# blackle/Megalania

Measured on AMD Instinct MI355X. Metric: SA neighbour-cost evals/s, higher is better.
Workload: dtype u64

## Files before the change

### megalania_amd/csrc/mgl_api.hip

```cpp
#include "mgl_kernels.hip"
#include "mgl_kernels2.hip"
#include "mgl_kernels3.hip"
#include "mgl_kernels4.hip"
#include "mgl_kernels5.hip"
#include "mgl_pbuild.hip"
#include "mgl_index.hip"
#include "mgl_matchfinder.hip"
#include "mgl_optimal.hip"
#include "mgl_adaptive.hip"
#include "mgl_props.hip"
#include "../../include/megalania_hip.h"

#include <math.h>
#include <stdio.h>
#include <stdlib.h>
#include <string.h>
#include <string>
#include <vector>

static const uint16_t k_cost_table[2048] = {
#include "mgl_cost_table.inc"
};

#define MGL_MAX_INPUT 176000000ull
static thread_local std::string g_err;
static int fail(int code, const std::string& msg)
{
	g_err = msg;
	return code;
}
#define HIPCHK(expr)                                                                         \
	do {                                                                                     \
		hipError_t e_ = (expr);                                                              \
		if (e_ != hipSuccess)                                                                \
			return fail(MGL_EDEVICE, std::string(#expr) + ": " + hipGetErrorString(e_));     \
	} while (0)

extern "C" const char* mgl_version(void) { return "megalania-hip 0.1 (gfx950)"; }
extern "C" const char* mgl_last_error(void) { return g_err.c_str(); }
extern "C" int mgl_device_count(void)
{
	int n = 0;
	if (hipGetDeviceCount(&n) != hipSuccess) return 0;
	return n;
}
extern "C" uint32_t mgl_rng_draw_at(uint64_t seed, uint64_t step, uint32_t j, uint32_t n)
{
	return mgl_rng_draw(mgl_rng_key(seed, step, j), n);
}

struct BaseMem {
	BaseView v;
	Control* ctl;
};

struct mgl_sa {
	int device;
	hipStream_t stream;
	hipStream_t stream2;
	hipEvent_t ev_fork, ev_join;
	hipEvent_t ev_tgt = nullptr, ev_tgt_go = nullptr;
	int tgt_ahead = 0;
	hipStream_t stream3 = nullptr;
	hipEvent_t ev_rest[8] = { nullptr, nullptr, nullptr, nullptr, nullptr, nullptr, nullptr, nullptr }, ev_sim = nullptr;
	uint32_t halves;
	uint32_t n;
	mgl_properties props;
	mgl_sa_config cfg;
	uint64_t temperature = 0;
	DevCtx ctx;
	uint8_t* d_data;
	uint32_t* d_bucket_off;
	uint32_t* d_bucket_pos;
	uint16_t* d_bucket_nx;
	uint32_t* d_quad_pos;
	uint16_t* d_quad_nx;
	uint32_t *d_quad_rank = nullptr, *d_quad_run = nullptr;
	uint32_t* d_xpos[6] = { nullptr, nullptr, nullptr, nullptr, nullptr, nullptr };
	uint32_t* d_xrank[6] = { nullptr, nullptr, nullptr, nullptr, nullptr, nullptr };
	uint32_t* d_xrun[6] = { nullptr, nullptr, nullptr, nullptr, nullptr, nullptr };
	uint8_t* d_xnxb[6] = { nullptr, nullptr, nullptr, nullptr, nullptr, nullptr };
	uint32_t *d_oct_pos = nullptr, *d_oct_rank = nullptr, *d_oct_run = nullptr;
	uint32_t *d_hex_pos = nullptr, *d_hex_rank = nullptr, *d_hex_run = nullptr;
	uint64_t *d_oct_nx8 = nullptr, *d_hex_nx8 = nullptr;
	uint16_t* d_cost_tbl;
	BaseMem base, scratch;
	mgl_pk* d_best;
	NbrOut nbr;
	uint32_t* d_aos;
	uint64_t* d_cum;
	uint16_t* d_final_probs;
	mgl_pk* d_topk_pk;
	uint64_t* d_topk_cost;
	uint32_t* d_small;
	uint32_t* d_sub_offs;
	uint32_t* d_sub_lens;
	uint32_t sub_cap;
	uint64_t sqrt_thresh;
	uint32_t per_wave_bytes, waves_per_block, nbr_lds, walk_lds;
	bool incremental;
	Base2 b2;
	unsigned long long* d_prof;
	uint32_t* d_todo;
	uint32_t per_wave2, waves_per_block2, nbr2_lds, build_lds;
	uint32_t chg_cap = MGL_CHG_CAP;
	uint32_t per_wave_pick, per_wave_rest, pick_waves;
	size_t b2_bytes;
	BigScratch big;
	uint32_t* d_todo2;
	uint32_t* d_todo3 = nullptr;
	uint4* d_pickstate;
	uint4* d_pickrec;
	bool split_nbr, adaptive;
	bool form_single = false;
	uint32_t* d_counts;
	ApplyBuf ab;
	uint32_t apply_blocks;
	bool incremental_apply;
	bool snapshots;
	Base2 snap_lit, snap_best;
	SnapMeta* d_snap_meta;
	bool parallel_build;
	PBuild pb;
	hipEvent_t ev_begin, ev_end;
	std::vector<hipEvent_t> ev_pool;
	int accept_mode = MGL_ACCEPT_AUTO;
	uint32_t bulk_threshold = 0;
	bool bulk_now = true;
	uint64_t bulk_hold = 0;
	uint64_t blk_done = 0;
	uint64_t blk_imp0 = 0, blk_acc0 = 0;
	BulkBuf bulk;
	BatchBuf batch;
	bool batch_ok = false;
	uint32_t* d_strat_tgt = nullptr;
	uint32_t* d_strat_pre = nullptr;
	bool select_small = false;
	uint32_t* h_bstat = nullptr;
	hipEvent_t ev_bstat = nullptr;
	uint32_t force_batch_fail = 0;
	uint32_t force_batch_late = 0;
	AcceptLimits lim, lim_max;
	uint64_t batch_early_giveups = 0;
	uint64_t batch_accepts = 0, batch_fallbacks = 0;
	std::vector<uint8_t> mode_log;
	uint32_t force_rollbacks = 0;
	uint64_t bulk_rollbacks = 0;
	bool best_unverified = false;
	uint32_t sim_waves = MGL_SIM_WAVES;
	std::vector<hipEvent_t> ev_sim_pool;
	int64_t time_sim_step = -1;
	bool count_traffic = false;
	unsigned long long* d_traffic = nullptr;
	uint32_t short_looks = 0;
	hipEvent_t ev_val = nullptr;
	int mf_finder = MGL_MF_NEAREST;
	uint32_t mf_depth = MGL_MF_DEF_DEPTH;
	uint32_t mf_built = 0;
	uint32_t* d_mf_off = nullptr;
	uint32_t* d_mf_src = nullptr;
	uint16_t* d_mf_len = nullptr;
	size_t mf_total = 0;
	double mf_ms = 0;
};

static uint64_t ceil_sqrt_u64(uint64_t x)
{
	uint64_t r = (uint64_t)sqrt((double)x);
	while (r * r > x) r--;
	while ((r + 1) * (r + 1) <= x) r++;
	return r * r == x ? r : r + 1;
}

static void dfree(void* p) { if (p) (void)hipFree(p); }
static void free_base(BaseMem& b)
{
	dfree(b.v.slab); dfree(b.v.onwalk); dfree(b.v.ckpt_probs); dfree(b.v.ckpt_hdr); dfree(b.ctl);
	memset(&b, 0, sizeof b);
}
static hipError_t alloc_base(BaseMem& b, uint32_t n, uint32_t ckpt_elems)
{
	memset(&b, 0, sizeof b);
	hipError_t e;
	b.v.nckpt = (n + (1u << MGL_CKPT_SHIFT) - 1u) >> MGL_CKPT_SHIFT;
	b.v.ckpt_elems = ckpt_elems;
	if ((e = hipMalloc(&b.v.slab, sizeof(mgl_pk) * (size_t)n)) != hipSuccess) return e;
	if ((e = hipMalloc(&b.v.onwalk, sizeof(uint64_t) * (((size_t)n + 63) / 64 + 1))) != hipSuccess) return e;
	if ((e = hipMalloc(&b.v.ckpt_probs, sizeof(uint16_t) * (size_t)b.v.nckpt * ckpt_elems)) != hipSuccess) return e;
	if ((e = hipMalloc(&b.v.ckpt_hdr, sizeof(CkptHdr) * (size_t)b.v.nckpt)) != hipSuccess) return e;
	if ((e = hipMalloc(&b.ctl, sizeof(Control))) != hipSuccess) return e;
	if ((e = hipMemset(b.v.onwalk, 0, sizeof(uint64_t) * (((size_t)n + 63) / 64 + 1))) != hipSuccess) return e;
	return hipMemset(b.ctl, 0, sizeof(Control));
}

static size_t b2_pool_entries(const Base2& b) { return (size_t)b.pool_cap + 256; }
static int alloc_b2(Base2& b, size_t n, bool own_slab, bool init, size_t* bytes_out)
{
	size_t bytes = 0;
	if (own_slab) {
		HIPCHK(hipMalloc(&b.slab, sizeof(mgl_pk) * n)); bytes += sizeof(mgl_pk) * n;
		HIPCHK(hipMalloc(&b.onwalk, sizeof(uint64_t) * ((n + 63) / 64 + 1)));
	}
	HIPCHK(hipMalloc(&b.sp0, sizeof(uint64_t) * (b.nw0 + 64))); bytes += sizeof(uint64_t) * (b.nw0 + 64);
	HIPCHK(hipMalloc(&b.sp1, sizeof(uint64_t) * (b.nw1 + 64)));
	HIPCHK(hipMalloc(&b.sp2, sizeof(uint64_t) * (b.nw2 + 64)));
	HIPCHK(hipMalloc(&b.sp_state, sizeof(uint32_t) * 8 * n)); bytes += sizeof(uint32_t) * 8 * n;
	HIPCHK(hipMalloc(&b.ck_probs, sizeof(uint16_t) * (size_t)b.nck * b.ck_elems)); bytes += sizeof(uint16_t) * (size_t)b.nck * b.ck_elems;
	HIPCHK(hipMalloc(&b.ch_off, sizeof(uint32_t) * b.ck_elems));
	HIPCHK(hipMalloc(&b.ch_len, sizeof(uint32_t) * b.ck_elems));
	HIPCHK(hipMalloc(&b.ch_cap, sizeof(uint32_t) * b.ck_elems));
	HIPCHK(hipMalloc(&b.ch_pos, sizeof(uint32_t) * b2_pool_entries(b))); bytes += sizeof(uint32_t) * (size_t)b.pool_cap;
	HIPCHK(hipMalloc(&b.ch_ev, sizeof(uint16_t) * b2_pool_entries(b))); bytes += sizeof(uint16_t) * (size_t)b.pool_cap;
	HIPCHK(hipMalloc(&b.pool_top, sizeof(uint32_t)));
	HIPCHK(hipMalloc(&b.ch_sb, sizeof(uint32_t) * (size_t)b.ck_elems * b.sb_stride)); bytes += sizeof(uint32_t) * (size_t)b.ck_elems * b.sb_stride;
	if (init) {
		HIPCHK(hipMemset(b.ch_sb, 0, sizeof(uint32_t) * (size_t)b.ck_elems * b.sb_stride));
		HIPCHK(hipMemset(b.sp0, 0, sizeof(uint64_t) * (b.nw0 + 64)));
		HIPCHK(hipMemset(b.sp1, 0, sizeof(uint64_t) * (b.nw1 + 64)));
		HIPCHK(hipMemset(b.sp2, 0, sizeof(uint64_t) * (b.nw2 + 64)));
		HIPCHK(hipMemset(b.ch_pos, 0xFF, sizeof(uint32_t) * b2_pool_entries(b)));
		HIPCHK(hipMemset(b.ch_ev, 0, sizeof(uint16_t) * b2_pool_entries(b)));
	}
	if (bytes_out) *bytes_out = bytes;
	return MGL_OK;
}
static void free_b2(Base2& b, bool own_slab)
{
	if (own_slab) { dfree(b.slab); dfree(b.onwalk); }
	dfree(b.sp0); dfree(b.sp1); dfree(b.sp2); dfree(b.sp_state); dfree(b.ck_probs);
	dfree(b.ch_off); dfree(b.ch_len); dfree(b.ch_cap); dfree(b.ch_pos); dfree(b.ch_ev); dfree(b.pool_top); dfree(b.ch_sb);
	memset(&b, 0, sizeof b);
}
static int launch_snapshot(mgl_sa* sa, Base2& snap, uint32_t which, int dir, int cond)
{
	const Base2& from = dir == 0 ? sa->b2 : snap;
	const Base2& to = dir == 0 ? snap : sa->b2;
	const size_t n = sa->n;
	SnapPlan p;
	memset(&p, 0, sizeof p);
	uint32_t k = 0;
	auto seg = [&](const void* s, void* d, size_t bytes, uint32_t pool_elem) {
		p.seg[k].src = s; p.seg[k].dst = d; p.seg[k].bytes = bytes; p.seg[k].pool_elem = pool_elem; k++;
	};
	seg(from.slab, to.slab, sizeof(mgl_pk) * n, 0);
	seg(from.onwalk, to.onwalk, sizeof(uint64_t) * ((n + 63) / 64 + 1), 0);
	seg(from.sp0, to.sp0, sizeof(uint64_t) * (from.nw0 + 64), 0);
	seg(from.sp1, to.sp1, sizeof(uint64_t) * (from.nw1 + 64), 0);
	seg(from.sp2, to.sp2, sizeof(uint64_t) * (from.nw2 + 64), 0);
	seg(from.sp_state, to.sp_state, sizeof(uint32_t) * 8 * n, 0);
	seg(from.ck_probs, to.ck_probs, sizeof(uint16_t) * (size_t)from.nck * from.ck_elems, 0);
	seg(from.ch_off, to.ch_off, sizeof(uint32_t) * from.ck_elems, 0);
	seg(from.ch_len, to.ch_len, sizeof(uint32_t) * from.ck_elems, 0);
	seg(from.ch_cap, to.ch_cap, sizeof(uint32_t) * from.ck_elems, 0);
	seg(from.ch_pos, to.ch_pos, sizeof(uint32_t) * b2_pool_entries(from), 4);
	seg(from.ch_ev, to.ch_ev, sizeof(uint16_t) * b2_pool_entries(from), 2);
	seg(from.pool_top, to.pool_top, sizeof(uint32_t), 0);
	seg(from.ch_sb, to.ch_sb, sizeof(uint32_t) * (size_t)from.ck_elems * from.sb_stride, 0);
	p.nseg = k;
	p.src_pool_top = from.pool_top;
	hipLaunchKernelGGL(k_snapshot, dim3(2048), dim3(256), 0, sa->stream, p, sa->base.ctl, sa->d_snap_meta + which, dir, cond);
	HIPCHK(hipGetLastError());
	return MGL_OK;
}

static int launch_rebuild(mgl_sa* sa, BaseMem& b, int from_dirty, uint64_t* cum, uint16_t* final_probs)
{
	hipLaunchKernelGGL(k_rebuild, dim3(1), dim3(64), sa->walk_lds, sa->stream, sa->ctx, b.v, b.ctl, from_dirty, cum, final_probs);
	HIPCHK(hipGetLastError());
	return MGL_OK;
}
static int launch_pbuild(mgl_sa* sa, bool validate_beside = false)
{
	const DevCtx& c = sa->ctx;
	Base2& b = sa->b2;
	PBuild& pb = sa->pb;
	Control* ctl = sa->base.ctl;
	hipStream_t st = sa->stream;
	const uint32_t total = c.L.total;
	hipLaunchKernelGGL(pb_exits, dim3(pb.nblk), dim3(320), 0, st, c, b, pb);
	hipLaunchKernelGGL(pb_entries_group, dim3(pb.ngrp), dim3(320), MGL_PB_GROUP * MGL_PB_ENTRIES * 2u, st, pb);
	hipLaunchKernelGGL(pb_entries, dim3(1), dim3(64), 0, st, c, pb);
	hipLaunchKernelGGL(pb_entries_fill, dim3(pb.ngrp), dim3(64), 0, st, pb);
	hipLaunchKernelGGL(pb_mark, dim3(pb.nblk), dim3(64), 0, st, c, b, pb, ctl);
	{
		const uint32_t nch = (pb.nblk + MGL_PB_SCAN_CHUNK - 1u) / MGL_PB_SCAN_CHUNK;
		hipLaunchKernelGGL(pb_scan_chunks, dim3((nch + 255u) / 256u), dim3(256), 0, st, pb);
		hipLaunchKernelGGL(pb_scan, dim3(1), dim3(64), 0, st, pb);
		hipLaunchKernelGGL(pb_scan_fill, dim3((nch + 255u) / 256u), dim3(256), 0, st, pb);
	}
	hipLaunchKernelGGL(pb_levels, dim3((b.nw0 + 255) / 256), dim3(256), 0, st, (const uint64_t*)b.sp0, b.sp1, b.nw0, b.nw1);
	hipLaunchKernelGGL(pb_levels, dim3((b.nw1 + 255) / 256), dim3(256), 0, st, (const uint64_t*)b.sp1, b.sp2, b.nw1, b.nw2);
	hipLaunchKernelGGL(pb_walk, dim3(pb.nblk), dim3(64), b.ck_elems * 4u, st, c, b, pb);
	if (validate_beside) {
		HIPCHK(hipEventRecord(sa->ev_fork, st));
		HIPCHK(hipStreamWaitEvent(sa->stream2, sa->ev_fork, 0));
		hipLaunchKernelGGL(k_validate, dim3((sa->ctx.n + 255u) / 256u), dim3(256), 0, sa->stream2, sa->ctx, sa->b2, sa->base.ctl);
		HIPCHK(hipEventRecord(sa->ev_val, sa->stream2));
	}
	{
		const uint32_t og = (pb.nblk + MGL_PB_OFF_ROWS - 1u) / MGL_PB_OFF_ROWS;
		hipLaunchKernelGGL(pb_offsets_sum, dim3((b.ck_elems + 255) / 256, og), dim3(256), 0, st, b, pb);
		hipLaunchKernelGGL(pb_offsets_top, dim3((b.ck_elems + 255) / 256), dim3(256), 0, st, b, pb, total, og);
		hipLaunchKernelGGL(pb_offsets, dim3((b.ck_elems + 255) / 256, og), dim3(256), 0, st, b, pb, total);
		hipLaunchKernelGGL(pb_index, dim3((total + 31u) / 32u, (pb.nblk + 1u + 31u) / 32u), dim3(256), 0, st, b, pb, total);
	}
	hipLaunchKernelGGL(pb_layout, dim3(1), dim3(64), 0, st, b, pb, ctl, total);
	hipLaunchKernelGGL(pb_scatter, dim3(pb.nblk), dim3(256), b.ck_elems * 4u, st, b, pb, total);
	hipLaunchKernelGGL(pb_sim, dim3((pb.seg_cap + 63) / 64), dim3(64), 0, st, c, b, pb);
	hipLaunchKernelGGL(pb_sim_fix, dim3((total + 63) / 64), dim3(64), 0, st, c, b, pb);
	hipLaunchKernelGGL(pb_ckpt, dim3((b.ck_elems + 63) / 64, (b.nck + MGL_PB_CK_ROWS - 1) / MGL_PB_CK_ROWS), dim3(64), 0, st, c, b);
	hipLaunchKernelGGL(pb_finish, dim3(1), dim3(64), 0, st, pb, ctl);
	if (validate_beside) HIPCHK(hipStreamWaitEvent(st, sa->ev_val, 0));
	HIPCHK(hipGetLastError());
	return MGL_OK;
}
static int rebuild_base(mgl_sa* sa, int after_accept)
{
	if (!sa->incremental) return launch_rebuild(sa, sa->base, after_accept, nullptr, nullptr);
	if (sa->parallel_build && !after_accept) return launch_pbuild(sa);
	hipLaunchKernelGGL(k_build, dim3(1), dim3(64), sa->build_lds, sa->stream, sa->ctx, sa->b2, sa->base.ctl, after_accept);
	HIPCHK(hipGetLastError());
	return MGL_OK;
}
static int launch_validate(mgl_sa* sa)
{
	if (!sa->incremental) return MGL_OK;
	hipLaunchKernelGGL(k_validate, dim3((sa->ctx.n + 255u) / 256u), dim3(256), 0, sa->stream, sa->ctx, sa->b2, sa->base.ctl);
	HIPCHK(hipGetLastError());
	return MGL_OK;
}
static Base2 accept_b2(const mgl_sa* sa) { Base2 b = sa->b2; b.pool_cap = sa->lim.v[MGL_LIM_POOL]; return b; }
static ApplyBuf accept_ab(const mgl_sa* sa)
{
	ApplyBuf ab = sa->ab;
	ab.job_cap = sa->lim.v[MGL_LIM_JOBS]; ab.span_cap = sa->lim.v[MGL_LIM_SPAN_AREA]; ab.scratch_cap = sa->lim.v[MGL_LIM_SCRATCH];
	return ab;
}
static BatchBuf accept_bt(const mgl_sa* sa) { BatchBuf bt = sa->batch; bt.runs_cap = sa->lim.v[MGL_LIM_BATCH_RUNS]; return bt; }
static void accept_limits_init(mgl_sa* sa, uint32_t* why)
{
	AcceptLimits& m = sa->lim_max;
	memset(&m, 0, sizeof m);
	m.v[MGL_LIM_APPLY_EVENTS] = MGL_APPLY_CAP; m.v[MGL_LIM_APPLY_GUARD] = 1u << 20; m.v[MGL_LIM_APPLY_SUB] = MGL_SUB_CAP;
	m.v[MGL_LIM_APPLY_SPAN] = MGL_SPAN_CAP; m.v[MGL_LIM_APPLY_PIECES] = MGL_PIECE_CAP; m.v[MGL_LIM_APPLY_SHIFT] = MGL_SUB_CAP;
	m.v[MGL_LIM_POOL] = sa->b2.pool_cap; m.v[MGL_LIM_JOBS] = sa->ab.job_cap; m.v[MGL_LIM_SPAN_AREA] = sa->ab.span_cap;
	m.v[MGL_LIM_SCRATCH] = sa->ab.scratch_cap;
	m.v[MGL_LIM_BATCH_JOURNAL] = MGL_BATCH_JCAP; m.v[MGL_LIM_BATCH_EVENTS] = MGL_BATCH_EVCAP; m.v[MGL_LIM_BATCH_OPS] = MGL_BATCH_OPCAP;
	m.v[MGL_LIM_BATCH_GUARD] = 1u << 18; m.v[MGL_LIM_BATCH_SUB] = MGL_BATCH_SUB; m.v[MGL_LIM_BATCH_SHIFT] = 2047u;
	m.v[MGL_LIM_BATCH_RUNS] = sa->batch.runs_cap; m.v[MGL_LIM_SOFT_REACH] = 1u;
	m.why = why;
	sa->lim = m;
	sa->lim.v[MGL_LIM_SOFT_REACH] = 0u;
}
static int launch_targets_ahead(mgl_sa* sa, uint64_t next_gstep);
static int launch_apply(mgl_sa* sa, uint64_t next_gstep = ~0ull)
{
	if (sa->snapshots) {
		int rc = launch_snapshot(sa, sa->snap_best, 1, 0, 2);
		if (rc) return rc;
	}
	hipLaunchKernelGGL(k_apply_walk, dim3(1), dim3(64), 0, sa->stream, sa->ctx, sa->b2, sa->base.ctl, sa->nbr, sa->ab, sa->lim);
	if (next_gstep != ~0ull) { int rc = launch_targets_ahead(sa, next_gstep); if (rc) return rc; }
	if (!sa->snapshots)
		hipLaunchKernelGGL(k_copy_best, dim3(256), dim3(256), 0, sa->stream, (const Control*)sa->base.ctl,
		                   (const mgl_pk*)sa->base.v.slab, sa->d_best, sa->ctx.n);
	hipLaunchKernelGGL(k_apply_chains, dim3(sa->apply_blocks), dim3(MGL_APPLY_THREADS), 0, sa->stream, sa->ctx, accept_b2(sa), sa->base.ctl, accept_ab(sa), sa->lim);
	hipLaunchKernelGGL(k_apply_jobs, dim3(1024), dim3(256), 0, sa->stream, sa->b2, (const Control*)sa->base.ctl, sa->ab, 0, (const uint32_t*)nullptr);
	hipLaunchKernelGGL(k_apply_jobs, dim3(1024), dim3(256), 0, sa->stream, sa->b2, (const Control*)sa->base.ctl, sa->ab, 1, (const uint32_t*)nullptr);
	hipLaunchKernelGGL(k_build_end, dim3(1), dim3(64), sa->build_lds, sa->stream, sa->ctx, sa->b2, sa->base.ctl, sa->snapshots ? 1 : 0, sa->d_counts, sa->adaptive ? 1 : 0, sa->form_single ? 1 : 0);
	HIPCHK(hipGetLastError());
	return MGL_OK;
}
static const bool g_trace = getenv("MGL_TRACE") != nullptr, g_prof_big = getenv("MGL_PROF_BIG") != nullptr, g_big_inline_sim = getenv("MGL_BIG_INLINE_SIM") != nullptr;
#define NBR_TRACE(name) do { if (g_trace) { fprintf(stderr, "[mgl] %s\n", name); hipError_t e_ = hipDeviceSynchronize(); if (e_ != hipSuccess) fprintf(stderr, "[mgl] %s -> %s\n", name, hipGetErrorString(e_)); } } while (0)
static hipEvent_t sim_event(mgl_sa* sa, size_t i)
{
	while (sa->ev_sim_pool.size() <= i) {
		hipEvent_t e = nullptr;
		if (hipEventCreate(&e) != hipSuccess) return nullptr;
		sa->ev_sim_pool.push_back(e);
	}
	return sa->ev_sim_pool[i];
}
static uint32_t nbr_slices(const mgl_sa* sa)
{
	const uint32_t K = sa->cfg.neighbours_per_step;
	return (sa->halves >= 2 && K >= 1024) ? sa->halves : 1u;
}
static void launch_targets(mgl_sa* sa, hipStream_t st, uint64_t step_override)
{
	const uint32_t K = sa->cfg.neighbours_per_step;
	const uint64_t* onwalk = sa->incremental ? sa->b2.onwalk : sa->base.v.onwalk;
	const uint32_t nw0 = sa->incremental ? sa->b2.nw0 : (sa->ctx.n + 63u) >> 6;
	hipLaunchKernelGGL(k_rank_blocks, dim3(sa->ctx.strat_nblk), dim3(64), 0, st, onwalk, nw0, sa->d_strat_pre, sa->ctx.strat_nblk);
	hipLaunchKernelGGL(k_rank_scan, dim3(1), dim3(1024), 0, st, sa->d_strat_pre, sa->ctx.strat_nblk);
	hipLaunchKernelGGL(k_targets, dim3((K + 3u) / 4u), dim3(256), 0, st, sa->ctx, onwalk, nw0, (const Control*)sa->base.ctl, sa->cfg.seed, step_override, K, sa->d_strat_tgt);
}
static int launch_targets_ahead(mgl_sa* sa, uint64_t next_gstep)
{
	if (!sa->d_strat_pre || !sa->incremental) return MGL_OK;
	HIPCHK(hipEventRecord(sa->ev_tgt_go, sa->stream));
	HIPCHK(hipStreamWaitEvent(sa->stream2, sa->ev_tgt_go, 0));
	launch_targets(sa, sa->stream2, next_gstep);
	HIPCHK(hipEventRecord(sa->ev_tgt, sa->stream2));
	HIPCHK(hipGetLastError());
	sa->tgt_ahead = 1;
	return MGL_OK;
}
static int launch_neighbours(mgl_sa* sa, uint64_t step_override, bool zero_counts = true)
{
	const uint32_t K = sa->cfg.neighbours_per_step;
	if (sa->d_strat_pre) {
		if (sa->tgt_ahead) HIPCHK(hipStreamWaitEvent(sa->stream, sa->ev_tgt, 0));
		if (sa->tgt_ahead != 1) launch_targets(sa, sa->stream, step_override);
		sa->tgt_ahead = 0;
	}
	if (!sa->incremental) {
		const uint32_t blocks = (K + sa->waves_per_block - 1) / sa->waves_per_block;
		hipLaunchKernelGGL(k_neighbours, dim3(blocks), dim3(64 * sa->waves_per_block), sa->nbr_lds, sa->stream, sa->ctx, sa->base.v,
		                   (const Control*)sa->base.ctl, sa->cfg.seed, step_override, K, sa->nbr, sa->per_wave_bytes,
		                   (const uint32_t*)nullptr, (const uint32_t*)nullptr); NBR_TRACE("k_neighbours");
		HIPCHK(hipGetLastError());
		return MGL_OK;
	}
	if (zero_counts) HIPCHK(hipMemsetAsync(sa->d_counts, 0, 8 * sizeof(uint32_t), sa->stream));
	const uint32_t blocks2 = (K + sa->waves_per_block2 - 1) / sa->waves_per_block2;
	const bool split_now = sa->split_nbr && !sa->form_single;
	const uint32_t sim_lds_regular = ((((sa->ctx.L.total + 31u) >> 5) + 3u) & ~3u) * 4u + sa->chg_cap * 16u;
	if (split_now) {
		const uint32_t slices = nbr_slices(sa);
		HIPCHK(hipEventRecord(sa->ev_fork, sa->stream));
		if (slices >= 2) HIPCHK(hipStreamWaitEvent(sa->stream2, sa->ev_fork, 0));
		HIPCHK(hipStreamWaitEvent(sa->stream3, sa->ev_fork, 0));
		for (uint32_t h = 0; h < slices; h++) {
			const uint32_t j0 = (uint32_t)((uint64_t)K * h / slices), j1 = (uint32_t)((uint64_t)K * (h + 1) / slices);
			hipStream_t st = (h & 1u) ? sa->stream2 : sa->stream;
			hipLaunchKernelGGL((k_neighbours2<false, MGL_NBR_PICK>), dim3((j1 - j0 + sa->pick_waves - 1) / sa->pick_waves), dim3(64 * sa->pick_waves),
			                   (MGL_PICK_T_GLOBAL ? 0u : 4096u) + sa->pick_waves * sa->per_wave_pick, st, sa->ctx,
			                   sa->b2, sa->base.ctl, sa->cfg.seed, step_override, K, sa->nbr, sa->per_wave_pick, sa->d_todo, sa->d_counts,
			                   (unsigned long long*)nullptr, sa->big, sa->d_pickrec, j0, j1, sa->d_pickstate); NBR_TRACE("k_neighbours2<false, MGL_NBR_PICK>");
			hipLaunchKernelGGL((k_neighbours2<false, MGL_NBR_REST>), dim3(j1 - j0), dim3(64), sa->per_wave_rest, st, sa->ctx,
			                   sa->b2, sa->base.ctl, sa->cfg.seed, step_override, K, sa->nbr, sa->per_wave_rest, sa->d_todo, sa->d_counts,
			                   g_prof_big ? (unsigned long long*)nullptr : sa->d_prof, sa->big, sa->d_pickrec, j0, j1, sa->d_pickstate); NBR_TRACE("k_neighbours2<false, MGL_NBR_REST>");
			HIPCHK(hipEventRecord(sa->ev_rest[h], st));
		}
		HIPCHK(hipGetLastError());
		for (uint32_t h = 0; h < slices; h++) {
			const uint32_t j0 = (uint32_t)((uint64_t)K * h / slices), j1 = (uint32_t)((uint64_t)K * (h + 1) / slices);
			HIPCHK(hipStreamWaitEvent(sa->stream3, sa->ev_rest[h], 0));
			if (sa->time_sim_step >= 0 && h < 2) HIPCHK(hipEventRecord(sim_event(sa, 6 * (size_t)sa->time_sim_step + 2 * h), sa->stream3));
			if (sa->count_traffic)
				hipLaunchKernelGGL(k_sim<true>, dim3(j1 - j0), dim3(64 * sa->sim_waves), sim_lds_regular, sa->stream3, sa->ctx, sa->b2, sa->base.ctl,
				                   sa->nbr, sa->big, j0, j1, sa->d_todo3, sa->d_counts + 4, (const uint32_t*)nullptr, (const uint32_t*)nullptr, sa->d_traffic);
			else
				hipLaunchKernelGGL(k_sim<false>, dim3(j1 - j0), dim3(64 * sa->sim_waves), sim_lds_regular, sa->stream3, sa->ctx, sa->b2, sa->base.ctl,
				                   sa->nbr, sa->big, j0, j1, sa->d_todo3, sa->d_counts + 4, (const uint32_t*)nullptr, (const uint32_t*)nullptr, (unsigned long long*)nullptr);
			NBR_TRACE("k_sim");
			if (sa->time_sim_step >= 0 && h < 2) HIPCHK(hipEventRecord(sim_event(sa, 6 * (size_t)sa->time_sim_step + 2 * h + 1), sa->stream3));
		}
		HIPCHK(hipEventRecord(sa->ev_sim, sa->stream3));
		for (uint32_t h = 1; h < slices; h += 2) HIPCHK(hipStreamWaitEvent(sa->stream, sa->ev_rest[h], 0));
	}
	if (!sa->split_nbr || sa->form_single) {
		hipLaunchKernelGGL((k_neighbours2<false, MGL_NBR_FULL>), dim3(blocks2), dim3(64 * sa->waves_per_block2), sa->nbr2_lds, sa->stream, sa->ctx,
		                   sa->b2, sa->base.ctl, sa->cfg.seed, step_override, K, sa->nbr, sa->per_wave2, sa->d_todo, sa->d_counts,
		                   sa->d_prof, sa->big, sa->d_pickrec, 0u, K, sa->d_pickstate); NBR_TRACE("k_neighbours2<false, MGL_NBR_FULL>");
	}
	const uint32_t bigneed = (sa->big.slots + sa->waves_per_block2 - 1) / sa->waves_per_block2;
	const uint32_t bigblocks = bigneed < 1024u ? bigneed : 1024u;
	BigScratch big_now = sa->big;
	big_now.lds_cache = 1u;
	const uint32_t big_lds = sa->nbr2_lds + 12u * MGL_BIG_CAP;
	if (!split_now || g_big_inline_sim) big_now.sim_hdr2 = nullptr;
	hipLaunchKernelGGL((k_neighbours2<true, MGL_NBR_FULL>), dim3(bigblocks), dim3(64 * sa->waves_per_block2), big_lds, sa->stream, sa->ctx,
	                   sa->b2, sa->base.ctl, sa->cfg.seed, step_override, K, sa->nbr, sa->per_wave2, sa->d_todo2, sa->d_counts + 1,
	                   g_prof_big ? sa->d_prof : (unsigned long long*)nullptr, big_now, (sa->split_nbr && !sa->form_single) ? sa->d_pickrec : (uint4*)nullptr, 0u, K, sa->d_pickstate); NBR_TRACE("k_neighbours2<true, MGL_NBR_FULL>");
	if (split_now) {
		const uint32_t sim_lds = ((((sa->ctx.L.total + 31u) >> 5) + 3u) & ~3u) * 4u + MGL_SIM2_CAP * 16u;
		if (sa->time_sim_step >= 0) HIPCHK(hipEventRecord(sim_event(sa, 6 * (size_t)sa->time_sim_step + 4), sa->stream));
		if (sa->count_traffic)
			hipLaunchKernelGGL(k_sim<true>, dim3(256), dim3(64 * MGL_SIM_WAVES_LIST), sim_lds, sa->stream, sa->ctx, sa->b2, sa->base.ctl, sa->nbr, big_now, 0u, K,
			                   sa->d_todo3, sa->d_counts + 4, (const uint32_t*)sa->d_todo, (const uint32_t*)sa->d_counts, sa->d_traffic);
		else
			hipLaunchKernelGGL(k_sim<false>, dim3(256), dim3(64 * MGL_SIM_WAVES_LIST), sim_lds, sa->stream, sa->ctx, sa->b2, sa->base.ctl, sa->nbr, big_now, 0u, K,
			                   sa->d_todo3, sa->d_counts + 4, (const uint32_t*)sa->d_todo, (const uint32_t*)sa->d_counts, (unsigned long long*)nullptr);
		NBR_TRACE("k_sim");
		if (sa->time_sim_step >= 0) HIPCHK(hipEventRecord(sim_event(sa, 6 * (size_t)sa->time_sim_step + 5), sa->stream));
		HIPCHK(hipStreamWaitEvent(sa->stream, sa->ev_sim, 0));
		BigScratch late = sa->big;
		late.todo_in = sa->d_todo3; late.todo_in_count = sa->d_counts + 4; late.sim_hdr2 = nullptr; late.lds_cache = 1u;
		late.cont = nullptr;
		hipLaunchKernelGGL((k_neighbours2<true, MGL_NBR_FULL>), dim3(bigblocks < 64u ? bigblocks : 64u), dim3(64 * sa->waves_per_block2), big_lds, sa->stream, sa->ctx,
		                   sa->b2, sa->base.ctl, sa->cfg.seed, step_override, K, sa->nbr, sa->per_wave2, sa->d_todo2, sa->d_counts + 1,
		                   (unsigned long long*)nullptr, late, sa->d_pickrec, 0u, K, sa->d_pickstate); NBR_TRACE("k_neighbours2<true, MGL_NBR_FULL>");
	}
	const uint32_t blocks = (K + sa->waves_per_block - 1) / sa->waves_per_block;
	hipLaunchKernelGGL(k_neighbours, dim3(blocks < 256u ? blocks : 256u), dim3(64 * sa->waves_per_block), sa->nbr_lds, sa->stream, sa->ctx, sa->base.v,
	                   (const Control*)sa->base.ctl, sa->cfg.seed, step_override, K, sa->nbr, sa->per_wave_bytes,
	                   (const uint32_t*)sa->d_todo2, (const uint32_t*)(sa->d_counts + 1)); NBR_TRACE("k_neighbours");
	HIPCHK(hipGetLastError());
	return MGL_OK;
}

static int import_slab(mgl_sa* sa, const mgl_packet* packets, mgl_pk* d_slab)
{
	HIPCHK(hipMemcpyAsync(sa->d_aos, packets, sizeof(mgl_packet) * (size_t)sa->n, hipMemcpyHostToDevice, sa->stream));
	hipLaunchKernelGGL(k_import, dim3(1024), dim3(256), 0, sa->stream, (const uint32_t*)sa->d_aos, d_slab, sa->n);
	HIPCHK(hipGetLastError());
	return MGL_OK;
}
static int export_slab(mgl_sa* sa, const mgl_pk* d_slab, mgl_packet* packets)
{
	hipLaunchKernelGGL(k_export, dim3(1024), dim3(256), 0, sa->stream, d_slab, sa->d_aos, sa->n);
	HIPCHK(hipGetLastError());
	HIPCHK(hipMemcpyAsync(packets, sa->d_aos, sizeof(mgl_packet) * (size_t)sa->n, hipMemcpyDeviceToHost, sa->stream));
	HIPCHK(hipStreamSynchronize(sa->stream));
	return MGL_OK;
}

extern "C" void mgl_sa_destroy(mgl_sa* sa)
{
	if (!sa) return;
	(void)hipSetDevice(sa->device);
	if (sa->stream) (void)hipStreamSynchronize(sa->stream);
	dfree(sa->d_data); dfree(sa->d_bucket_off); dfree(sa->d_bucket_pos); dfree(sa->d_bucket_nx); dfree(sa->d_quad_pos); dfree(sa->d_quad_nx); dfree(sa->d_cost_tbl);
	dfree(sa->d_quad_rank); dfree(sa->d_quad_run); dfree(sa->d_oct_pos);
	for (int i = 0; i < 6; i++) { if (i != 0 && i != 2) { dfree(sa->d_xpos[i]); dfree(sa->d_xrank[i]); dfree(sa->d_xrun[i]); } dfree(sa->d_xnxb[i]); } dfree(sa->d_oct_rank); dfree(sa->d_oct_run);
	dfree(sa->d_hex_pos); dfree(sa->d_hex_rank); dfree(sa->d_hex_run); dfree(sa->d_oct_nx8); dfree(sa->d_hex_nx8);
	free_base(sa->base); free_base(sa->scratch);
	if (!sa->snapshots) dfree(sa->d_best);
	dfree(sa->nbr.cost); dfree(sa->nbr.ndiffs); dfree(sa->nbr.walked); dfree(sa->nbr.win); dfree(sa->nbr.win2); dfree(sa->nbr.dpos);
	dfree(sa->bulk.ckey); dfree(sa->bulk.cwin); dfree(sa->bulk.taken); dfree(sa->bulk.cstate); dfree(sa->bulk.cflags); dfree(sa->bulk.hdr);
	dfree(sa->nbr.dold); dfree(sa->nbr.dnew);
	dfree(sa->d_aos); dfree(sa->d_cum); dfree(sa->d_final_probs);
	free_b2(sa->b2, false);
	free_b2(sa->snap_lit, true); free_b2(sa->snap_best, true); dfree(sa->d_snap_meta);
	dfree(sa->pb.exits); dfree(sa->pb.entry); dfree(sa->pb.gexits); dfree(sa->pb.gentry); dfree(sa->pb.gsum); dfree(sa->pb.ch_map); dfree(sa->pb.ch_vs); dfree(sa->pb.ch_pk); dfree(sa->pb.ch_state); dfree(sa->pb.tf_ctx); dfree(sa->pb.tf_dist); dfree(sa->pb.tf_pk);
	dfree(sa->pb.st_in); dfree(sa->pb.hist); dfree(sa->pb.stage); dfree(sa->pb.stage_n); dfree(sa->pb.stage_over); dfree(sa->pb.acc); dfree(sa->pb.seg_off); dfree(sa->pb.unres);
	dfree(sa->d_todo); dfree(sa->d_prof);
	dfree(sa->big.sim_hdr); dfree(sa->big.sim_keys); dfree(sa->big.sim_pos);
	dfree(sa->big.ins_key); dfree(sa->big.rem_key); dfree(sa->big.ins_pos); dfree(sa->big.rem_pos); dfree(sa->big.uctx);
	if (sa->h_bstat) (void)hipHostFree(sa->h_bstat);
	if (sa->ev_bstat) (void)hipEventDestroy(sa->ev_bstat);
	dfree(sa->big.cont); dfree(sa->d_traffic); dfree(sa->d_strat_pre); dfree(sa->d_strat_tgt);
	{
		BatchBuf& bt = sa->batch;
		dfree(bt.hdr); dfree(bt.cl); dfree(bt.jpos); dfree(bt.jnew); dfree(bt.jold); dfree(bt.st_ikey); dfree(bt.st_rkey); dfree(bt.st_ipos);
		dfree(bt.st_rpos); dfree(bt.ops); dfree(bt.ins_cl); dfree(bt.rem_cl); dfree(bt.acc); dfree(bt.runs);
		dfree(bt.cnt_i); dfree(bt.cnt_r); dfree(bt.off_i); dfree(bt.off_r); dfree(bt.cur_i); dfree(bt.cur_r); dfree(bt.touched);
		dfree(bt.bk_ipos); dfree(bt.bk_rpos); dfree(bt.bk_ibit); dfree(bt.bk_icl); dfree(bt.bk_rcl);
	}
	for (hipEvent_t e : sa->ev_sim_pool) if (e) (void)hipEventDestroy(e);
	dfree(sa->d_todo2); dfree(sa->d_todo3); dfree(sa->d_counts); dfree(sa->big.sim_hdr2); dfree(sa->big.sim_slot2); dfree(sa->d_pickrec); dfree(sa->d_pickstate);
	dfree(sa->lim.why); dfree(sa->ab.hdr); dfree(sa->ab.ins_key); dfree(sa->ab.rem_key); dfree(sa->ab.ins_pos); dfree(sa->ab.rem_pos);
	dfree(sa->ab.tctx); dfree(sa->ab.scratch_pos); dfree(sa->ab.scratch_ev);
	dfree(sa->ab.span_pos); dfree(sa->ab.span_ev); dfree(sa->ab.jobs_b); dfree(sa->ab.jobs_c);
	dfree(sa->d_mf_off); dfree(sa->d_mf_src); dfree(sa->d_mf_len);
	dfree(sa->d_topk_pk); dfree(sa->d_topk_cost); dfree(sa->d_small); dfree(sa->d_sub_offs); dfree(sa->d_sub_lens);
	for (hipEvent_t e : sa->ev_pool) (void)hipEventDestroy(e);
	if (sa->ev_begin) (void)hipEventDestroy(sa->ev_begin);
	if (sa->ev_end) (void)hipEventDestroy(sa->ev_end);
	if (sa->stream2) (void)hipStreamDestroy(sa->stream2);
	if (sa->stream3) (void)hipStreamDestroy(sa->stream3);
	for (auto& e : sa->ev_rest) if (e) (void)hipEventDestroy(e);
	if (sa->ev_sim) (void)hipEventDestroy(sa->ev_sim);
	if (sa->ev_val) (void)hipEventDestroy(sa->ev_val);
	if (sa->ev_fork) (void)hipEventDestroy(sa->ev_fork);
	if (sa->ev_tgt) (void)hipEventDestroy(sa->ev_tgt);
	if (sa->ev_tgt_go) (void)hipEventDestroy(sa->ev_tgt_go);
	if (sa->ev_join) (void)hipEventDestroy(sa->ev_join);
	if (sa->stream) (void)hipStreamDestroy(sa->stream);
	delete sa;
}

static int create_impl(mgl_sa* sa, const uint8_t* data, size_t n)
{
	HIPCHK(hipSetDevice(sa->device));
	HIPCHK(hipStreamCreate(&sa->stream));
	HIPCHK(hipStreamCreate(&sa->stream2));
	HIPCHK(hipEventCreateWithFlags(&sa->ev_fork, hipEventDisableTiming));
	HIPCHK(hipEventCreateWithFlags(&sa->ev_join, hipEventDisableTiming));
	HIPCHK(hipEventCreateWithFlags(&sa->ev_tgt, hipEventDisableTiming));
	HIPCHK(hipEventCreateWithFlags(&sa->ev_tgt_go, hipEventDisableTiming));
	HIPCHK(hipStreamCreate(&sa->stream3));
	for (auto& e : sa->ev_rest) HIPCHK(hipEventCreateWithFlags(&e, hipEventDisableTiming));
	HIPCHK(hipEventCreateWithFlags(&sa->ev_sim, hipEventDisableTiming));
	HIPCHK(hipEventCreateWithFlags(&sa->ev_val, hipEventDisableTiming));
	sa->halves = getenv("MGL_HALVES") ? (uint32_t)atoi(getenv("MGL_HALVES")) : (n > (1u << 20) ? 2u : 1u);
	if (sa->halves < 1 || sa->halves > 8) sa->halves = 1;
	HIPCHK(hipEventCreate(&sa->ev_begin));
	HIPCHK(hipEventCreate(&sa->ev_end));
	const mgl_layout L = mgl_make_layout(sa->props.lc, sa->props.lp, sa->props.pb);
	const uint32_t ckpt_elems = (L.total + 7u) & ~7u;

	HIPCHK(hipMalloc(&sa->d_data, n + 128));
	HIPCHK(hipMemset(sa->d_data, 0, n + 128));
	HIPCHK(hipMemcpy(sa->d_data, data, n, hipMemcpyHostToDevice));

	{
		const uint32_t m = (uint32_t)(n - 1);
		HIPCHK(hipMalloc(&sa->d_bucket_off, sizeof(uint32_t) * 65537));
		HIPCHK(hipMalloc(&sa->d_bucket_pos, sizeof(uint32_t) * (n ? n : 1)));
		HIPCHK(hipMalloc(&sa->d_bucket_nx, sizeof(uint16_t) * (n ? n : 1)));
		HIPCHK(hipMalloc(&sa->d_quad_pos, sizeof(uint32_t) * (n ? n : 1)));
		HIPCHK(hipMalloc(&sa->d_quad_nx, sizeof(uint16_t) * (n ? n : 1)));
		for (int i = 0; i < 6; i++) {
			HIPCHK(hipMalloc(&sa->d_xnxb[i], n + 1));
			HIPCHK(hipMemset(sa->d_xnxb[i], 0, n + 1));
			if (i == 0 || i == 2) continue;
			for (uint32_t** a : { &sa->d_xpos[i], &sa->d_xrank[i], &sa->d_xrun[i] }) {
				HIPCHK(hipMalloc(a, sizeof(uint32_t) * (n + 1)));
				HIPCHK(hipMemset(*a, 0, sizeof(uint32_t) * (n + 1)));
			}
		}
		for (uint32_t** a : { &sa->d_quad_rank, &sa->d_quad_run, &sa->d_oct_pos, &sa->d_oct_rank, &sa->d_oct_run, &sa->d_hex_pos, &sa->d_hex_rank, &sa->d_hex_run }) {
			HIPCHK(hipMalloc(a, sizeof(uint32_t) * (n + 1)));
			HIPCHK(hipMemset(*a, 0, sizeof(uint32_t) * (n + 1)));
		}
		HIPCHK(hipMalloc(&sa->d_oct_nx8, sizeof(uint64_t) * (n + 1)));
		HIPCHK(hipMalloc(&sa->d_hex_nx8, sizeof(uint64_t) * (n + 1)));
		if (m == 0) HIPCHK(hipMemset(sa->d_bucket_off, 0, sizeof(uint32_t) * 65537));
		else {
			const uint32_t nblk = (m + MGL_IX_ITEMS - 1) / MGL_IX_ITEMS;
			uint32_t *tmp = nullptr, *matrix = nullptr;
			HIPCHK(hipMalloc(&tmp, sizeof(uint32_t) * m));
			HIPCHK(hipMalloc(&matrix, sizeof(uint32_t) * 256 * (size_t)nblk));
			for (int pass = 1; pass >= 0; pass--) {
				const uint32_t* in = pass == 1 ? nullptr : tmp;
				uint32_t* out = pass == 1 ? tmp : sa->d_bucket_pos;
				hipLaunchKernelGGL(ix_count, dim3(nblk), dim3(64), 0, sa->stream, (const uint8_t*)sa->d_data, in, m, pass, matrix, nblk);
				hipLaunchKernelGGL(ix_scan, dim3(1), dim3(1024), 0, sa->stream, matrix, 256u * nblk);
				hipLaunchKernelGGL(ix_scatter, dim3(nblk), dim3(64), 0, sa->stream, (const uint8_t*)sa->d_data, in, out, m, pass,
				                   (const uint32_t*)matrix, nblk);
			}
			hipLaunchKernelGGL(ix_offsets, dim3(m / 256 + 1), dim3(256), 0, sa->stream, (const uint8_t*)sa->d_data,
			                   (const uint32_t*)sa->d_bucket_pos, m, sa->d_bucket_off);
			hipLaunchKernelGGL(ix_next2, dim3(m / 256 + 1), dim3(256), 0, sa->stream, (const uint8_t*)sa->d_data,
			                   (const uint32_t*)sa->d_bucket_pos, m, sa->d_bucket_nx, 0);
			for (int pass = 3; pass >= 0; pass--) {
				const uint32_t* in = pass == 3 ? nullptr : ((pass & 1) ? (const uint32_t*)sa->d_quad_pos : (const uint32_t*)tmp);
				uint32_t* out = (pass & 1) ? tmp : sa->d_quad_pos;
				hipLaunchKernelGGL(ix_count, dim3(nblk), dim3(64), 0, sa->stream, (const uint8_t*)sa->d_data, in, m, pass, matrix, nblk);
				hipLaunchKernelGGL(ix_scan, dim3(1), dim3(1024), 0, sa->stream, matrix, 256u * nblk);
				hipLaunchKernelGGL(ix_scatter, dim3(nblk), dim3(64), 0, sa->stream, (const uint8_t*)sa->d_data, in, out, m, pass,
				                   (const uint32_t*)matrix, nblk);
			}
			hipLaunchKernelGGL(ix_next2, dim3(m / 256 + 1), dim3(256), 0, sa->stream, (const uint8_t*)sa->d_data,
			                   (const uint32_t*)sa->d_quad_pos, m, sa->d_quad_nx, 1);
			sa->d_xpos[0] = sa->d_bucket_pos; sa->d_xpos[2] = sa->d_quad_pos;
			sa->d_xrank[2] = sa->d_quad_rank; sa->d_xrun[2] = sa->d_quad_run;
			for (uint32_t D : { 3u, 5u, 6u, 7u, 8u, 16u }) {
				uint32_t* dst = D == 8 ? sa->d_oct_pos : D == 16 ? sa->d_hex_pos : sa->d_xpos[D - 2];
				for (int pass = (int)D - 1; pass >= 0; pass--) {
					const uint32_t* in = pass == (int)D - 1 ? nullptr : ((pass & 1) ? (const uint32_t*)dst : (const uint32_t*)tmp);
					uint32_t* out = (pass & 1) ? tmp : dst;
					hipLaunchKernelGGL(ix_count, dim3(nblk), dim3(64), 0, sa->stream, (const uint8_t*)sa->d_data, in, m, pass, matrix, nblk);
					hipLaunchKernelGGL(ix_scan, dim3(1), dim3(1024), 0, sa->stream, matrix, 256u * nblk);
					hipLaunchKernelGGL(ix_scatter, dim3(nblk), dim3(64), 0, sa->stream, (const uint8_t*)sa->d_data, in, out, m, pass,
					                   (const uint32_t*)matrix, nblk);
				}
			}
			struct { const uint32_t* pos; uint32_t* rank; uint32_t* run; void* nx; uint32_t D, nxbytes; } lv[7] = {
				{ sa->d_xpos[1], sa->d_xrank[1], sa->d_xrun[1], sa->d_xnxb[1], 3u, 1u },
				{ sa->d_quad_pos, sa->d_quad_rank, sa->d_quad_run, sa->d_xnxb[2], 4u, 1u },
				{ sa->d_xpos[3], sa->d_xrank[3], sa->d_xrun[3], sa->d_xnxb[3], 5u, 1u },
				{ sa->d_xpos[4], sa->d_xrank[4], sa->d_xrun[4], sa->d_xnxb[4], 6u, 1u },
				{ sa->d_xpos[5], sa->d_xrank[5], sa->d_xrun[5], sa->d_xnxb[5], 7u, 1u },
				{ sa->d_oct_pos, sa->d_oct_rank, sa->d_oct_run, sa->d_oct_nx8, 8u, 8u },
				{ sa->d_hex_pos, sa->d_hex_rank, sa->d_hex_run, sa->d_hex_nx8, 16u, 8u } };
			hipLaunchKernelGGL(ix_next_byte, dim3(m / 256 + 1), dim3(256), 0, sa->stream, (const uint8_t*)sa->d_data, (const uint32_t*)sa->d_bucket_pos, m, sa->d_xnxb[0], 2u);
			for (auto& l : lv) {
				hipLaunchKernelGGL(ix_rank, dim3(m / 256 + 1), dim3(256), 0, sa->stream, l.pos, m, l.rank);
				if (l.nxbytes == 1) hipLaunchKernelGGL(ix_next_byte, dim3(m / 256 + 1), dim3(256), 0, sa->stream, (const uint8_t*)sa->d_data, l.pos, m, (uint8_t*)l.nx, l.D);
				else hipLaunchKernelGGL(ix_next_bytes, dim3(m / 256 + 1), dim3(256), 0, sa->stream, (const uint8_t*)sa->d_data, l.pos, m, l.nx, l.D, l.nxbytes);
				hipLaunchKernelGGL(ix_heads, dim3(m / 256 + 1), dim3(256), 0, sa->stream, (const uint8_t*)sa->d_data, l.pos, m, l.D, l.run);
				hipLaunchKernelGGL(ix_maxscan, dim3(1), dim3(1024), 0, sa->stream, l.run, m);
			}
			hipError_t e1 = hipGetLastError(), e2 = hipStreamSynchronize(sa->stream);
			(void)hipFree(tmp); (void)hipFree(matrix);
			HIPCHK(e1); HIPCHK(e2);
		}
	}
	HIPCHK(hipMalloc(&sa->d_cost_tbl, sizeof(k_cost_table)));
	HIPCHK(hipMemcpy(sa->d_cost_tbl, k_cost_table, sizeof(k_cost_table), hipMemcpyHostToDevice));

	sa->ctx.data = sa->d_data; sa->ctx.n = (uint32_t)n;
	sa->ctx.bucket_off = sa->d_bucket_off; sa->ctx.bucket_pos = sa->d_bucket_pos; sa->ctx.bucket_nx = sa->d_bucket_nx; sa->ctx.quad_pos = sa->d_quad_pos; sa->ctx.quad_nx = sa->d_quad_nx;
	for (int i = 0; i < 6; i++) { sa->ctx.xpos[i] = sa->d_xpos[i]; sa->ctx.xrank[i] = sa->d_xrank[i]; sa->ctx.xrun[i] = sa->d_xrun[i]; sa->ctx.xnxb[i] = sa->d_xnxb[i]; }
	sa->ctx.oct_pos = sa->d_oct_pos; sa->ctx.oct_rank = sa->d_oct_rank; sa->ctx.oct_run = sa->d_oct_run; sa->ctx.oct_nx8 = sa->d_oct_nx8;
	sa->ctx.hex_pos = sa->d_hex_pos; sa->ctx.hex_rank = sa->d_hex_rank; sa->ctx.hex_run = sa->d_hex_run; sa->ctx.hex_nx8 = sa->d_hex_nx8;
	sa->ctx.cost_tbl = sa->d_cost_tbl; sa->ctx.L = L;
	sa->ctx.dict_limit = sa->cfg.dict_limit; sa->ctx.max_scan = sa->cfg.max_bucket_scan; sa->ctx.top_k = sa->cfg.top_k;

	HIPCHK(alloc_base(sa->base, (uint32_t)n, ckpt_elems));
	HIPCHK(alloc_base(sa->scratch, (uint32_t)n, ckpt_elems));

	const size_t K = sa->cfg.neighbours_per_step;
	HIPCHK(hipMalloc(&sa->nbr.cost, sizeof(uint64_t) * K));
	HIPCHK(hipMalloc(&sa->nbr.ndiffs, sizeof(uint32_t) * K));
	HIPCHK(hipMalloc(&sa->nbr.walked, sizeof(uint32_t) * K));
	HIPCHK(hipMalloc(&sa->nbr.win, sizeof(uint32_t) * 2 * K));
	HIPCHK(hipMemset(sa->nbr.win, 0xFF, sizeof(uint32_t) * 2 * K));
	HIPCHK(hipMalloc(&sa->nbr.win2, sizeof(uint32_t) * K));
	HIPCHK(hipMemset(sa->nbr.win2, 0xFF, sizeof(uint32_t) * K));
	memset(&sa->bulk, 0, sizeof sa->bulk);
	HIPCHK(hipMalloc(&sa->bulk.ckey, sizeof(uint64_t) * K));
// ... 56 lines not shown
			pb.shift = b.sb_shift;
			pb.nblk = (uint32_t)((n + (1u << pb.shift) - 1) >> pb.shift);
			HIPCHK(hipMalloc(&pb.exits, sizeof(uint16_t) * (size_t)pb.nblk * MGL_PB_ENTRIES));
			HIPCHK(hipMalloc(&pb.entry, sizeof(uint32_t) * ((size_t)pb.nblk + 1)));
			pb.ngrp = (pb.nblk + MGL_PB_GROUP - 1u) / MGL_PB_GROUP;
			HIPCHK(hipMalloc(&pb.gexits, sizeof(uint16_t) * (size_t)pb.ngrp * MGL_PB_ENTRIES));
			HIPCHK(hipMalloc(&pb.gentry, sizeof(uint16_t) * (size_t)pb.ngrp));
			{
				const size_t nch = ((size_t)pb.nblk + MGL_PB_SCAN_CHUNK - 1u) / MGL_PB_SCAN_CHUNK;
				HIPCHK(hipMalloc(&pb.ch_map, sizeof(uint64_t) * nch));
				HIPCHK(hipMalloc(&pb.ch_vs, sizeof(uint32_t) * 8 * nch));
				HIPCHK(hipMalloc(&pb.ch_pk, sizeof(uint32_t) * nch));
				HIPCHK(hipMalloc(&pb.ch_state, sizeof(uint32_t) * 8 * nch));
			}
			HIPCHK(hipMalloc(&pb.gsum, sizeof(uint32_t) * (size_t)((pb.nblk + MGL_PB_OFF_ROWS - 1u) / MGL_PB_OFF_ROWS) * ckpt_elems));
			HIPCHK(hipMalloc(&pb.tf_ctx, sizeof(uint64_t) * pb.nblk));
			HIPCHK(hipMalloc(&pb.tf_dist, sizeof(uint32_t) * 8 * (size_t)pb.nblk));
			HIPCHK(hipMalloc(&pb.tf_pk, sizeof(uint32_t) * pb.nblk));
			HIPCHK(hipMalloc(&pb.st_in, sizeof(uint32_t) * 8 * (size_t)pb.nblk));
			HIPCHK(hipMalloc(&pb.hist, sizeof(uint32_t) * (size_t)pb.nblk * ckpt_elems));
			HIPCHK(hipMalloc(&pb.stage, sizeof(uint64_t) * (size_t)pb.nblk * ((MGL_PB_STAGE_PER_POS << pb.shift) + 32u)));
			HIPCHK(hipMalloc(&pb.stage_n, sizeof(uint32_t) * (size_t)pb.nblk));
			HIPCHK(hipMalloc(&pb.stage_over, sizeof(uint32_t)));
			HIPCHK(hipMemset(pb.stage_over, 0, sizeof(uint32_t)));
			HIPCHK(hipMalloc(&pb.acc, sizeof(unsigned long long) * 16));
			HIPCHK(hipMemset(pb.acc, 0, sizeof(unsigned long long) * 16));
			pb.seg_cap = b.pool_cap / MGL_PB_SEG + ckpt_elems + 64u;
			HIPCHK(hipMalloc(&pb.seg_off, sizeof(uint32_t) * (ckpt_elems + 1)));
			HIPCHK(hipMalloc(&pb.unres, pb.seg_cap));
		}
		sa->snapshots = !(sa->cfg.flags & MGL_F_NO_SNAPSHOTS);
		if (sa->snapshots) {
			for (Base2* s : { &sa->snap_lit, &sa->snap_best }) {
				*s = b;
				s->slab = nullptr; s->onwalk = nullptr; s->sp0 = s->sp1 = s->sp2 = nullptr; s->sp_state = nullptr;
				s->ck_probs = nullptr; s->ch_off = s->ch_len = s->ch_cap = s->ch_pos = nullptr; s->ch_ev = nullptr;
				s->pool_top = nullptr;
				int rc = alloc_b2(*s, n, true, false, nullptr);
				if (rc) return rc;
			}
			HIPCHK(hipMalloc(&sa->d_snap_meta, sizeof(SnapMeta) * 2));
			HIPCHK(hipMemset(sa->d_snap_meta, 0, sizeof(SnapMeta) * 2));
			sa->d_best = sa->snap_best.slab;
		}
		if (sa->cfg.flags & MGL_F_PROFILE) {
			HIPCHK(hipMalloc(&sa->d_prof, sizeof(unsigned long long) * (32 + K)));
			HIPCHK(hipMemset(sa->d_prof, 0, sizeof(unsigned long long) * (32 + K)));
		}
		HIPCHK(hipMalloc(&sa->d_todo, sizeof(uint32_t) * (K + 1)));
		HIPCHK(hipMemset(sa->d_todo, 0, sizeof(uint32_t) * (K + 1)));
		sa->b2_bytes = bytes;
		sa->incremental_apply = getenv("MGL_NO_INCREMENTAL_APPLY") == nullptr;
		{
			ApplyBuf& ab = sa->ab;
			memset(&ab, 0, sizeof ab);
			sa->apply_blocks = 256;
			ab.scratch_cap = b.pool_cap + 256u;
			ab.span_cap = 1u << 22;
			ab.job_cap = 1u << 20;
			HIPCHK(hipMalloc(&ab.hdr, sizeof(uint32_t) * 16));
			HIPCHK(hipMemset(ab.hdr, 0, sizeof(uint32_t) * 16));
			HIPCHK(hipMalloc(&ab.ins_key, sizeof(uint16_t) * MGL_BATCH_ALLOC));
			HIPCHK(hipMalloc(&ab.rem_key, sizeof(uint16_t) * MGL_BATCH_ALLOC));
			HIPCHK(hipMalloc(&ab.ins_pos, sizeof(uint32_t) * MGL_BATCH_ALLOC));
			HIPCHK(hipMalloc(&ab.rem_pos, sizeof(uint32_t) * MGL_BATCH_ALLOC));
			HIPCHK(hipMalloc(&ab.tctx, sizeof(uint16_t) * 16384));
			HIPCHK(hipMalloc(&ab.scratch_pos, sizeof(uint32_t) * (size_t)ab.scratch_cap));
			HIPCHK(hipMalloc(&ab.scratch_ev, sizeof(uint16_t) * (size_t)ab.scratch_cap));
			HIPCHK(hipMalloc(&ab.span_pos, sizeof(uint32_t) * (size_t)ab.span_cap));
			HIPCHK(hipMalloc(&ab.span_ev, sizeof(uint16_t) * (size_t)ab.span_cap));
			HIPCHK(hipMalloc(&ab.jobs_b, sizeof(uint4) * (size_t)ab.job_cap));
			HIPCHK(hipMalloc(&ab.jobs_c, sizeof(uint4) * (size_t)ab.job_cap));
			BatchBuf& bt = sa->batch;
			memset(&bt, 0, sizeof bt);
			HIPCHK(hipMalloc(&bt.hdr, sizeof(uint32_t) * 16));
			HIPCHK(hipMemset(bt.hdr, 0, sizeof(uint32_t) * 16));
			HIPCHK(hipMalloc(&bt.cl, sizeof(uint32_t) * 8 * MGL_BATCH_MAX));
			HIPCHK(hipMalloc(&bt.jpos, sizeof(uint32_t) * MGL_BATCH_MAX * MGL_MAX_DIFFS));
			HIPCHK(hipMalloc(&bt.jnew, sizeof(mgl_pk) * MGL_BATCH_MAX * MGL_MAX_DIFFS));
			HIPCHK(hipMalloc(&bt.jold, sizeof(mgl_pk) * MGL_BATCH_MAX * MGL_MAX_DIFFS));
			HIPCHK(hipMalloc(&bt.st_ikey, sizeof(uint16_t) * MGL_BATCH_ALLOC));
			HIPCHK(hipMalloc(&bt.st_rkey, sizeof(uint16_t) * MGL_BATCH_ALLOC));
			HIPCHK(hipMalloc(&bt.st_ipos, sizeof(uint32_t) * MGL_BATCH_ALLOC));
			HIPCHK(hipMalloc(&bt.st_rpos, sizeof(uint32_t) * MGL_BATCH_ALLOC));
			HIPCHK(hipMalloc(&bt.ops, sizeof(uint4) * 2 * (size_t)MGL_BATCH_MAX * MGL_BATCH_OPCAP));
			HIPCHK(hipMalloc(&bt.ins_cl, MGL_BATCH_ALLOC));
			HIPCHK(hipMalloc(&bt.rem_cl, MGL_BATCH_ALLOC));
			bt.nctx = L.total;
			bt.runs_cap = 1u << 17;
			HIPCHK(hipMalloc(&bt.runs, sizeof(uint4) * 2 * (size_t)bt.runs_cap));
			for (uint32_t** p : { &bt.cnt_i, &bt.cnt_r, &bt.off_i, &bt.off_r, &bt.cur_i, &bt.cur_r, &bt.touched }) {
				HIPCHK(hipMalloc(p, sizeof(uint32_t) * (bt.nctx + 64u)));
				HIPCHK(hipMemset(*p, 0, sizeof(uint32_t) * (bt.nctx + 64u)));
			}
			HIPCHK(hipMalloc(&bt.bk_ipos, sizeof(uint32_t) * MGL_BATCH_ALLOC));
			HIPCHK(hipMalloc(&bt.bk_rpos, sizeof(uint32_t) * MGL_BATCH_ALLOC));
			HIPCHK(hipMalloc(&bt.bk_ibit, sizeof(uint16_t) * MGL_BATCH_ALLOC));
			HIPCHK(hipMalloc(&bt.bk_icl, MGL_BATCH_ALLOC));
			HIPCHK(hipMalloc(&bt.bk_rcl, MGL_BATCH_ALLOC));
			HIPCHK(hipMalloc(&bt.acc, sizeof(long long) * 4));
			HIPCHK(hipMemset(bt.acc, 0, sizeof(long long) * 4));
			HIPCHK(hipHostMalloc((void**)&sa->h_bstat, sizeof(uint32_t) * 16, hipHostMallocDefault));
			HIPCHK(hipEventCreateWithFlags(&sa->ev_bstat, hipEventDisableTiming));
			sa->batch_ok = sa->incremental_apply && getenv("MGL_NO_BATCH") == nullptr;
			uint32_t* why = nullptr;
			HIPCHK(hipMalloc(&why, sizeof(uint32_t)));
			HIPCHK(hipMemset(why, 0, sizeof(uint32_t)));
			accept_limits_init(sa, why);

		}
		{
			const uint32_t fixed = MGL_MAX_DIFFS * (8u + 8u + 4u) + (((((L.total + 31u) >> 5) + 3u) & ~3u) * 4u) ;
			const uint32_t model = ckpt_elems * 2u + MGL_PRICE_WORDS * 4u;
			sa->chg_cap = K <= 1024u ? 4u * MGL_CHG_CAP : (K <= 2048u ? 2u * MGL_CHG_CAP : MGL_CHG_CAP);
			const uint32_t lists = sa->chg_cap * (4u + 4u + 2u + 2u) + 2u * sa->chg_cap * 2u;
			sa->per_wave2 = (fixed + (model > lists ? model : lists) + 15u) & ~15u;
			sa->per_wave_pick = (model + 15u) & ~15u;
			sa->per_wave_rest = (fixed + lists + 15u) & ~15u;
		}
		{
			BigScratch& g = sa->big;
			memset(&g, 0, sizeof g);
			g.chg_cap = sa->chg_cap;
			g.cap = MGL_BIG_CAP; g.uctx_cap = ckpt_elems; g.slots = (uint32_t)(K > 512 ? K : 512);
			HIPCHK(hipMalloc(&g.ins_key, sizeof(uint16_t) * (size_t)g.cap * g.slots));
			HIPCHK(hipMalloc(&g.rem_key, sizeof(uint16_t) * (size_t)g.cap * g.slots));
			HIPCHK(hipMalloc(&g.ins_pos, sizeof(uint32_t) * (size_t)g.cap * g.slots));
			HIPCHK(hipMalloc(&g.rem_pos, sizeof(uint32_t) * (size_t)g.cap * g.slots));
			HIPCHK(hipMalloc(&g.uctx, sizeof(uint16_t) * (size_t)g.uctx_cap * g.slots));
			HIPCHK(hipMalloc(&sa->d_todo2, sizeof(uint32_t) * (K + 1)));
			HIPCHK(hipMemset(sa->d_todo2, 0, sizeof(uint32_t) * (K + 1)));
		}
		{
			uint32_t best_w = 1, best_total = 0;
			for (uint32_t w = 1; w <= 8; w++) {
				const uint32_t bytes = 4096u + w * sa->per_wave2;
				if (bytes > 160u * 1024u) break;
				const uint32_t tot = (160u * 1024u / bytes) * w;
				if (tot > best_total) { best_total = tot; best_w = w; }
			}
			(void)best_w;
			sa->waves_per_block2 = 1;
		}
		sa->nbr2_lds = 4096u + sa->waves_per_block2 * sa->per_wave2;
		sa->build_lds = 4096u + ckpt_elems * 2u + ckpt_elems * 8u;
		HIPCHK(hipMalloc(&sa->d_counts, sizeof(uint32_t) * 16));
		HIPCHK(hipMemset(sa->d_counts, 0, sizeof(uint32_t) * 16));
		HIPCHK(hipMalloc(&sa->d_todo3, sizeof(uint32_t) * (K + 1)));
		HIPCHK(hipMemset(sa->d_todo3, 0, sizeof(uint32_t) * (K + 1)));
		sa->big.todo_in = sa->d_todo; sa->big.todo_in_count = sa->d_counts; sa->big.spill_ctr = sa->d_counts + 2;
		HIPCHK(hipFuncSetAttribute((const void*)k_neighbours2<false, MGL_NBR_FULL>, hipFuncAttributeMaxDynamicSharedMemorySize, (int)sa->nbr2_lds));
		HIPCHK(hipFuncSetAttribute((const void*)k_neighbours2<false, MGL_NBR_PICK>, hipFuncAttributeMaxDynamicSharedMemorySize, 160 * 1024));
		HIPCHK(hipFuncSetAttribute((const void*)k_neighbours2<false, MGL_NBR_REST>, hipFuncAttributeMaxDynamicSharedMemorySize, (int)sa->nbr2_lds));
		HIPCHK(hipFuncSetAttribute((const void*)k_neighbours2<true, MGL_NBR_FULL>, hipFuncAttributeMaxDynamicSharedMemorySize, (int)(sa->nbr2_lds + 12u * MGL_BIG_CAP)));
		HIPCHK(hipMalloc(&sa->d_pickrec, sizeof(uint4) * K));
		HIPCHK(hipMalloc(&sa->d_pickstate, sizeof(uint4) * 2 * K));
		sa->split_nbr = getenv("MGL_NO_SPLIT") == nullptr;
		if (sa->split_nbr) {
			BigScratch& g = sa->big;
			HIPCHK(hipMalloc(&g.sim_hdr, sizeof(uint4) * (size_t)K));
			HIPCHK(hipMalloc(&g.sim_keys, sizeof(uint16_t) * 2u * sa->chg_cap * (size_t)K));
			HIPCHK(hipMalloc(&g.sim_pos, sizeof(uint32_t) * 2u * sa->chg_cap * (size_t)K));
			HIPCHK(hipMemset(g.sim_hdr, 0xFF, sizeof(uint4) * (size_t)K));
			HIPCHK(hipMalloc(&g.sim_hdr2, sizeof(uint4) * (size_t)K));
			HIPCHK(hipMalloc(&g.sim_slot2, sizeof(uint32_t) * (size_t)K));
			HIPCHK(hipMemset(g.sim_hdr2, 0xFF, sizeof(uint4) * (size_t)K));
			if (getenv("MGL_NO_CONT") == nullptr) {
				HIPCHK(hipMalloc(&g.cont, sizeof(uint32_t) * MGL_CONT_WORDS * (size_t)g.slots));
				HIPCHK(hipMemset(g.cont, 0, sizeof(uint32_t) * MGL_CONT_WORDS * (size_t)g.slots));
			}
		}
		if (getenv("MGL_SIMW")) { const int w = atoi(getenv("MGL_SIMW")); if (w == 1 || w == 2 || w == 4 || w == 8) sa->sim_waves = (uint32_t)w; }
		sa->adaptive = sa->split_nbr && getenv("MGL_NO_ADAPT") == nullptr;
		sa->form_single = !sa->split_nbr;
		sa->pick_waves = getenv("MGL_PICK_WAVES") ? (uint32_t)atoi(getenv("MGL_PICK_WAVES")) : 0u;
		if (sa->pick_waves != 1 && sa->pick_waves != 2 && sa->pick_waves != 4 && sa->pick_waves != 8) sa->pick_waves = 0;
		{
			uint32_t best_w = 1, best_resident = 0;
			for (uint32_t w = 1; w <= 8; w *= 2) {
				const uint32_t bytes = (MGL_PICK_T_GLOBAL ? 0u : 4096u) + w * sa->per_wave_pick;
				if (bytes > 160u * 1024u) break;
				const uint32_t resident = (160u * 1024u / ((bytes + 1279u) / 1280u * 1280u)) * w;
				if (resident > best_resident) { best_resident = resident; best_w = w; }
			}
			if (n > (1u << 20)) best_w = 1;
			if (sa->pick_waves == 0 || (MGL_PICK_T_GLOBAL ? 0u : 4096u) + sa->pick_waves * sa->per_wave_pick > 160u * 1024u) sa->pick_waves = best_w;
		}
		HIPCHK(hipFuncSetAttribute((const void*)k_sim<false>, hipFuncAttributeMaxDynamicSharedMemorySize, 96 * 1024));
		HIPCHK(hipFuncSetAttribute((const void*)k_sim<true>, hipFuncAttributeMaxDynamicSharedMemorySize, 96 * 1024));
		HIPCHK(hipMalloc(&sa->d_traffic, sizeof(unsigned long long) * 2));
		HIPCHK(hipMemset(sa->d_traffic, 0, sizeof(unsigned long long) * 2));
		HIPCHK(hipFuncSetAttribute((const void*)k_build, hipFuncAttributeMaxDynamicSharedMemorySize, (int)sa->build_lds));
		HIPCHK(hipFuncSetAttribute((const void*)k_build_end, hipFuncAttributeMaxDynamicSharedMemorySize, (int)sa->build_lds));
	}

	if (!(sa->cfg.flags & MGL_F_POSITION_TARGETS)) {
		sa->ctx.strat_nblk = (uint32_t)((n + 4095u) / 4096u);
		HIPCHK(hipMalloc(&sa->d_strat_pre, sizeof(uint32_t) * (sa->ctx.strat_nblk + 2u)));
		HIPCHK(hipMemset(sa->d_strat_pre, 0, sizeof(uint32_t) * (sa->ctx.strat_nblk + 2u)));
		sa->ctx.strat_pre = sa->d_strat_pre;
		HIPCHK(hipMalloc(&sa->d_strat_tgt, sizeof(uint32_t) * sa->cfg.neighbours_per_step));
		sa->ctx.strat_tgt = sa->d_strat_tgt;
	}
	sa->sqrt_thresh = ceil_sqrt_u64(sa->cfg.iters_per_epoch);
	sa->bulk_threshold = getenv("MGL_BULK_THRESHOLD") ? (uint32_t)atoi(getenv("MGL_BULK_THRESHOLD"))
	                     : sa->batch_ok ? 2u : (n <= (1u << 20) ? 16u : n <= (1u << 24) ? 32u : 128u);
	if (sa->bulk_threshold == 0) sa->bulk_threshold = 1;

	hipLaunchKernelGGL(k_fill_literal, dim3(1024), dim3(256), 0, sa->stream, sa->base.v.slab, sa->ctx.n);
	if (!sa->d_best) HIPCHK(hipMalloc(&sa->d_best, sizeof(mgl_pk) * n));
	hipLaunchKernelGGL(k_fill_literal, dim3(1024), dim3(256), 0, sa->stream, sa->d_best, sa->ctx.n);
	HIPCHK(hipGetLastError());
	int rc = rebuild_base(sa, 0);
	if (rc) return rc;
	if (sa->incremental && sa->snapshots && (rc = launch_snapshot(sa, sa->snap_lit, 0, 0, 0))) return rc;
	HIPCHK(hipStreamSynchronize(sa->stream));
	{
		Control c0;
		HIPCHK(hipMemcpy(&c0, sa->base.ctl, sizeof c0, hipMemcpyDeviceToHost));
		if (c0.error_flags) return fail(MGL_EDEVICE, "mgl_sa_create: building the base structures of the all-literal slab failed");
	}
	return MGL_OK;
}

extern "C" mgl_sa* mgl_sa_create(const uint8_t* data, size_t n, mgl_properties props, const mgl_sa_config* cfg)
{
	if (!data || n == 0 || !cfg) { fail(MGL_EINVAL, "mgl_sa_create: bad data/size/config"); return nullptr; }
	if (n > MGL_MAX_INPUT) { fail(MGL_EINVAL, "mgl_sa_create: input larger than 176 000 000 bytes is not supported"); return nullptr; }
	if (props.lc + props.lp > 4 || props.pb > 4 || props.lc > 8) { fail(MGL_EINVAL, "mgl_sa_create: unsupported lc/lp/pb"); return nullptr; }
	mgl_sa* sa = new (std::nothrow) mgl_sa();
	if (!sa) { fail(MGL_ENOMEM, "mgl_sa_create: out of host memory"); return nullptr; }
	sa->cfg = *cfg;
	sa->props = props;
	sa->n = (uint32_t)n;
	sa->device = cfg->device;
	if (sa->cfg.neighbours_per_step == 0) sa->cfg.neighbours_per_step = 1;
	if (sa->cfg.neighbours_per_step > (1u << 20)) { delete sa; fail(MGL_EINVAL, "neighbours_per_step > 2^20"); return nullptr; }
	if (sa->cfg.top_k == 0) sa->cfg.top_k = 20;
	if (sa->cfg.top_k > MGL_MAX_TOPK) { delete sa; fail(MGL_EINVAL, "top_k > 32"); return nullptr; }
	if (sa->cfg.dict_limit == 0) sa->cfg.dict_limit = 0x400000u;
	if (sa->cfg.iters_per_epoch == 0) sa->cfg.iters_per_epoch = n;
	int rc = create_impl(sa, data, n);
	if (rc != MGL_OK) {
		std::string keep = g_err;
		mgl_sa_destroy(sa);
		g_err = keep;
		return nullptr;
	}
	return sa;
}

static int read_ctl(mgl_sa* sa, BaseMem& b, Control* out)
{
	HIPCHK(hipMemcpyAsync(out, b.ctl, sizeof(Control), hipMemcpyDeviceToHost, sa->stream));
	HIPCHK(hipStreamSynchronize(sa->stream));
	return MGL_OK;
}
static int write_ctl(mgl_sa* sa, BaseMem& b, const Control* in)
{
	HIPCHK(hipMemcpyAsync(b.ctl, in, sizeof(Control), hipMemcpyHostToDevice, sa->stream));
	HIPCHK(hipStreamSynchronize(sa->stream));
	return MGL_OK;
}

static int keep_best_before_overwrite(mgl_sa* sa, Control& c)
{
	if (!(sa->incremental && sa->snapshots) || !c.best_is_current) return MGL_OK;
	int rc = launch_snapshot(sa, sa->snap_best, 1, 0, 0);
	if (rc) return rc;
	c.best_is_current = 0;
	return MGL_OK;
}

extern "C" int mgl_sa_begin_epoch(mgl_sa* sa, unsigned phase, int from_best)
{
	if (!sa) return fail(MGL_EINVAL, "null handle");
	HIPCHK(hipSetDevice(sa->device));
	Control c;
	int rc = read_ctl(sa, sa->base, &c);
	if (rc) return rc;
	if (from_best && c.best_cost == 0) from_best = 0;
	const bool snaps = sa->incremental && sa->snapshots;
	const bool base_is_best = snaps && c.best_is_current;
	if (!from_best && (rc = keep_best_before_overwrite(sa, c))) return rc;
	c.iter = 0; c.cur_cost = 0; c.phase = phase; c.accepted_flag = 0; c.copy_best_flag = 0;
	if ((rc = write_ctl(sa, sa->base, &c))) return rc;
	sa->bulk_now = !from_best; sa->bulk_hold = 0; sa->blk_done = 0; sa->select_small = false;
	if (from_best && base_is_best) return MGL_OK;
	if (snaps) {
		SnapMeta meta[2];
		HIPCHK(hipMemcpyAsync(meta, sa->d_snap_meta, sizeof meta, hipMemcpyDeviceToHost, sa->stream));
		HIPCHK(hipStreamSynchronize(sa->stream));
		const uint32_t which = from_best ? 1u : 0u;
		if (meta[which].valid) {
			if ((rc = launch_snapshot(sa, which ? sa->snap_best : sa->snap_lit, which, 1, 0))) return rc;
			HIPCHK(hipStreamSynchronize(sa->stream));
			return MGL_OK;
		}
	}
	if (from_best) HIPCHK(hipMemcpyAsync(sa->base.v.slab, sa->d_best, sizeof(mgl_pk) * (size_t)sa->n, hipMemcpyDeviceToDevice, sa->stream));
	else {
		hipLaunchKernelGGL(k_fill_literal, dim3(1024), dim3(256), 0, sa->stream, sa->base.v.slab, sa->ctx.n);
		HIPCHK(hipGetLastError());
	}
	if ((rc = rebuild_base(sa, 0))) return rc;
	if (from_best && sa->best_unverified) {
		if ((rc = launch_validate(sa))) return rc;
		Control v;
		if ((rc = read_ctl(sa, sa->base, &v))) return rc;
		if (v.error_flags || v.rebuild_cost != v.best_cost) {
			v.error_flags = 0;
			(void)write_ctl(sa, sa->base, &v);
			return fail(MGL_EINVAL, "mgl_sa_begin_epoch: the adopted best slab is not a valid parse of the input at the cost it came with");
		}
		sa->best_unverified = false;
	}
	if (snaps && (rc = launch_snapshot(sa, from_best ? sa->snap_best : sa->snap_lit, from_best ? 1u : 0u, 0, 0))) return rc;
	HIPCHK(hipStreamSynchronize(sa->stream));
	return MGL_OK;
// ... 739 lines not shown
		hipLaunchKernelGGL(k_batch_chains, dim3(MGL_BATCH_GRID), dim3(MGL_BATCH_THREADS), 0, sa->stream, sa->ctx, accept_b2(sa), sa->base.ctl, bt, ab, sa->lim);
		hipLaunchKernelGGL(k_batch_ckpt, dim3(1024, 8), dim3(256), 0, sa->stream, b, (const Control*)sa->base.ctl, bt, ab);
		hipLaunchKernelGGL(k_apply_jobs, dim3(1024), dim3(256), 0, sa->stream, b, (const Control*)sa->base.ctl, sa->ab, 0, (const uint32_t*)sa->batch.hdr);
		hipLaunchKernelGGL(k_apply_jobs, dim3(1024), dim3(256), 0, sa->stream, b, (const Control*)sa->base.ctl, sa->ab, 1, (const uint32_t*)sa->batch.hdr);
		hipLaunchKernelGGL(k_batch_end, dim3(1), dim3(64), 0, sa->stream, sa->base.ctl, sa->batch);
		HIPCHK(hipGetLastError());
		HIPCHK(hipMemcpyAsync(sa->h_bstat, sa->batch.hdr, sizeof bstat, hipMemcpyDeviceToHost, sa->stream));
		HIPCHK(hipEventRecord(sa->ev_bstat, sa->stream));
		launch_bulk_close(sa, (const uint32_t*)sa->batch.hdr);
		HIPCHK(hipGetLastError());
		HIPCHK(hipEventSynchronize(sa->ev_bstat));
		memcpy(bstat, sa->h_bstat, sizeof bstat);
		closed = bstat[0] == 3u || bstat[0] == 0u;
		if (!closed && sa->tgt_ahead) sa->tgt_ahead = 2;
		if (sa->force_batch_fail) {
			const uint32_t zero = 0u;
			HIPCHK(hipMemcpy(sa->batch.hdr + 9, &zero, sizeof zero, hipMemcpyHostToDevice));
			HIPCHK(hipMemcpy(sa->batch.hdr + 13, &zero, sizeof zero, hipMemcpyHostToDevice));
			if ((bstat[0] == 1u || bstat[0] == 3u) && --sa->force_batch_fail == 0) sa->force_batch_late = 0;
		}
	}
	if (sa->batch_ok) sa->select_small = bstat[7] <= 512u;
	if (bstat[0] == 3u) sa->batch_accepts++;
	else if (bstat[0] != 0u) {
		if (sa->batch_ok && bstat[0] == 1u) sa->batch_fallbacks++;
		if (sa->batch_ok && bstat[0] == 2u && bstat[4]) sa->batch_early_giveups++;
		if (bstat[0] != 1u)
			hipLaunchKernelGGL(k_bulk_write, dim3(64), dim3(256), 0, sa->stream, sa->base.ctl, sa->nbr, sa->bulk, sa->base.v.slab);
		HIPCHK(hipGetLastError());
		Control now;
		if (sa->batch_ok && bstat[0] == 1u) {
			if ((rc = read_ctl(sa, sa->base, &now))) return rc;
			now.apply_failed = 0;
			if ((rc = write_ctl(sa, sa->base, &now))) return rc;
		}
		if ((rc = launch_pbuild(sa, sa->incremental))) return rc;
		if ((rc = read_ctl(sa, sa->base, &now))) return rc;
		if (sa->force_rollbacks && now.taken) { sa->force_rollbacks--; now.error_flags |= MGL_ERR_BAD_PACKET; }
		if (now.error_flags & MGL_ERR_BAD_PACKET) {
			hipLaunchKernelGGL(k_bulk_rollback, dim3(64), dim3(256), 0, sa->stream, sa->nbr, sa->bulk, sa->base.v.slab);
			HIPCHK(hipGetLastError());
			now.error_flags &= ~MGL_ERR_BAD_PACKET;
			now.accepted -= now.taken;
			now.taken = 0;
			sa->bulk_rollbacks++;
			if ((rc = write_ctl(sa, sa->base, &now))) return rc;
			if ((rc = launch_pbuild(sa))) return rc;
		}
	}
	if (!closed) launch_bulk_close(sa, nullptr);
	HIPCHK(hipGetLastError());
	return MGL_OK;
}

extern "C" int mgl_sa_run(mgl_sa* sa, uint64_t steps, mgl_sa_stats* stats)
{
	if (!sa) return fail(MGL_EINVAL, "null handle");
	HIPCHK(hipSetDevice(sa->device));
	Control before, after;
	int rc = read_ctl(sa, sa->base, &before);
	if (rc) return rc;
	const bool timing = (sa->cfg.flags & MGL_F_TIMING) != 0;
	const uint64_t t_stride = steps > 16 ? 4u : 1u;
	const uint64_t timed_steps = timing ? ((steps + t_stride - 1) / t_stride < 512 ? (steps + t_stride - 1) / t_stride : 512) : 0;
	const bool inc_apply = sa->incremental && sa->incremental_apply;
	const DecideArgs dargs = decide_args(sa);
	const int mode = (sa->incremental && sa->parallel_build) ? sa->accept_mode : MGL_ACCEPT_SINGLE;
	sa->mode_log.clear();
	if (sa->tgt_ahead) sa->tgt_ahead = 2;
	const uint64_t rollbacks_before = sa->bulk_rollbacks;
	std::vector<uint8_t> sim_timed;
	unsigned long long traffic_before[2] = { 0, 0 };
	if (sa->count_traffic) HIPCHK(hipMemcpy(traffic_before, sa->d_traffic, sizeof traffic_before, hipMemcpyDeviceToHost));
	if (sa->blk_done == 0) { sa->blk_imp0 = before.imp_cands; sa->blk_acc0 = before.accepted; }
	HIPCHK(hipEventRecord(sa->ev_begin, sa->stream));
	for (uint64_t s = 0; s < steps;) {
		const bool bulk = mode == MGL_ACCEPT_BULK || (mode == MGL_ACCEPT_AUTO && sa->bulk_now);
		const uint64_t full = mode == MGL_ACCEPT_AUTO ? (bulk ? 4u : 16u) : 64u;
		uint64_t block = mode == MGL_ACCEPT_AUTO ? full - sa->blk_done : full;
		if (sa->short_looks && block > 4u) block = 4u;
		if (block > steps - s) block = steps - s;
		for (uint64_t e = s + block; s < e; s++) {
			const bool t = s % t_stride == 0 && s / t_stride < timed_steps;
			const uint64_t ti = s / t_stride;
			if (sa->mode_log.size() < (1u << 20)) sa->mode_log.push_back(bulk ? 1 : 0);
			if (t) HIPCHK(hipEventRecord(pool_event(sa, 4 * ti + 0), sa->stream));
			sa->time_sim_step = (t && sa->split_nbr && !sa->form_single) ? (int64_t)ti : -1;
			if (t) sim_timed.push_back(sa->time_sim_step >= 0 ? (nbr_slices(sa) < 2u ? 1 : 2) : 0);
			rc = launch_neighbours(sa, ~0ull, s == 0 || !inc_apply);
			sa->time_sim_step = -1;
			if (rc) return rc;
			if (t) HIPCHK(hipEventRecord(pool_event(sa, 4 * ti + 1), sa->stream));
			if (bulk) {
				if (t) HIPCHK(hipEventRecord(pool_event(sa, 4 * ti + 2), sa->stream));
				if ((rc = launch_bulk_tail(sa, s + 1 < steps ? before.gstep + s + 1 : ~0ull))) return rc;
				if (t) HIPCHK(hipEventRecord(pool_event(sa, 4 * ti + 3), sa->stream));
				continue;
			}
			hipLaunchKernelGGL(k_decide, dim3(1), dim3(1024), 0, sa->stream, sa->ctx, sa->base.v, sa->base.ctl, sa->nbr, dargs, inc_apply ? 0 : 1);
			HIPCHK(hipGetLastError());
			if (t) HIPCHK(hipEventRecord(pool_event(sa, 4 * ti + 2), sa->stream));
			if (inc_apply) {
				if ((rc = launch_apply(sa, s + 1 < steps ? before.gstep + s + 1 : ~0ull))) return rc;
			} else {
				hipLaunchKernelGGL(k_copy_best, dim3(256), dim3(256), 0, sa->stream, (const Control*)sa->base.ctl,
				                   (const mgl_pk*)sa->base.v.slab, sa->d_best, sa->ctx.n);
				HIPCHK(hipGetLastError());
				if ((rc = rebuild_base(sa, 1))) return rc;
				if (sa->incremental && sa->snapshots && (rc = launch_snapshot(sa, sa->snap_best, 1, 0, 1))) return rc;
			}
			if (t) HIPCHK(hipEventRecord(pool_event(sa, 4 * ti + 3), sa->stream));
		}
		if (mode == MGL_ACCEPT_AUTO) sa->blk_done += block;
		const bool block_over = mode == MGL_ACCEPT_AUTO && sa->blk_done == full;
		if (block_over || (s < steps && sa->adaptive)) {
			Control now;
			if ((rc = read_ctl(sa, sa->base, &now))) return rc;
			if (now.error_flags) break;
			if (sa->short_looks) sa->short_looks--;
			if (sa->adaptive && sa->form_single != (now.nbr_single != 0)) { sa->form_single = now.nbr_single != 0; sa->short_looks = 3; }
			if (block_over) {
				auto_decide(sa, bulk, full, now.imp_cands - sa->blk_imp0, now.accepted - sa->blk_acc0);
				sa->blk_done = 0; sa->blk_imp0 = now.imp_cands; sa->blk_acc0 = now.accepted;
			}
		}
	}
	HIPCHK(hipEventRecord(sa->ev_end, sa->stream));
	HIPCHK(hipStreamSynchronize(sa->stream));
	if ((rc = read_ctl(sa, sa->base, &after))) return rc;
	if (sa->adaptive && sa->form_single != (after.nbr_single != 0)) { sa->form_single = after.nbr_single != 0; sa->short_looks = 3; }
	if (stats) {
		memset(stats, 0, sizeof *stats);
		stats->steps = after.gstep - before.gstep;
		stats->evaluations = after.evals - before.evals;
		stats->failed = after.failed - before.failed;
		stats->accepted = after.accepted - before.accepted;
		stats->improved = after.improved - before.improved;
		stats->packets_evaluated = after.packets_eval - before.packets_eval;
		stats->current_cost = after.cur_cost;
		stats->best_cost = after.best_cost;
		stats->packets = after.packets;
		float ms = 0;
		HIPCHK(hipEventElapsedTime(&ms, sa->ev_begin, sa->ev_end));
		stats->gpu_ms_total = ms;
		for (uint64_t s = 0; s < timed_steps; s++) {
			HIPCHK(hipEventElapsedTime(&ms, sa->ev_pool[4 * s + 0], sa->ev_pool[4 * s + 1]));
			stats->gpu_ms_neighbours += ms;
			HIPCHK(hipEventElapsedTime(&ms, sa->ev_pool[4 * s + 2], sa->ev_pool[4 * s + 3]));
			stats->gpu_ms_rebuild += ms;
		}
		stats->neighbour_launches = timed_steps;
		for (uint64_t s = 0; s < timed_steps && s < sim_timed.size(); s++) {
			if (!sim_timed[s]) continue;
			for (uint32_t h = 0; h < 3; h++) {
				if (h < 2 && h >= sim_timed[s]) continue;
				HIPCHK(hipEventElapsedTime(&ms, sa->ev_sim_pool[6 * s + 2 * h], sa->ev_sim_pool[6 * s + 2 * h + 1]));
				stats->gpu_ms_sim += ms;
				stats->sim_launches++;
			}
		}
		if (sa->count_traffic) {
			unsigned long long now[2] = { 0, 0 };
			HIPCHK(hipMemcpy(now, sa->d_traffic, sizeof now, hipMemcpyDeviceToHost));
			stats->sim_bytes_counted = now[0] - traffic_before[0];
		}
		stats->full_rebuilds = after.full_rebuilds - before.full_rebuilds;
		stats->fallback_neighbours = after.fallback_nbrs - before.fallback_nbrs;
		stats->second_pass_neighbours = after.big_nbrs - before.big_nbrs;
		stats->bulk_steps = after.bulk_steps - before.bulk_steps;
		stats->dropped_neighbours = after.dropped - before.dropped;
		stats->improving_neighbours = after.imp_cands - before.imp_cands;
		stats->bulk_rollbacks = sa->bulk_rollbacks - rollbacks_before;
		stats->bulk_double_writes = after.bulk_overlaps - before.bulk_overlaps;
	}
	if (after.error_flags) {
		char buf[96];
		snprintf(buf, sizeof buf, "mgl_sa_run: device consistency check failed (flags 0x%x)", after.error_flags);
		return fail(MGL_EDEVICE, buf);
	}
	return MGL_OK;
}

extern "C" int mgl_sa_current(mgl_sa* sa, mgl_packet* packets_out, uint64_t* perplexity_out)
{
	if (!sa) return fail(MGL_EINVAL, "null handle");
	HIPCHK(hipSetDevice(sa->device));
	Control c;
	int rc = read_ctl(sa, sa->base, &c);
	if (rc) return rc;
	if (perplexity_out) *perplexity_out = c.rebuild_cost;
	if (packets_out) return export_slab(sa, sa->base.v.slab, packets_out);
	return MGL_OK;
}
extern "C" int mgl_sa_best(mgl_sa* sa, mgl_packet* packets_out, uint64_t* perplexity_out)
{
	if (!sa) return fail(MGL_EINVAL, "null handle");
	HIPCHK(hipSetDevice(sa->device));
	Control c;
	int rc = read_ctl(sa, sa->base, &c);
	if (rc) return rc;
	if (perplexity_out) *perplexity_out = c.best_cost;
	if (packets_out) return export_slab(sa, (sa->incremental && sa->snapshots && c.best_is_current) ? sa->base.v.slab : sa->d_best, packets_out);
	return MGL_OK;
}

static int scratch_walk(mgl_sa* sa, const mgl_packet* packets, bool want_cum, bool want_probs, Control* out)
{
	int rc = import_slab(sa, packets, sa->scratch.v.slab);
	if (rc) return rc;
	HIPCHK(hipMemsetAsync(sa->scratch.ctl, 0, sizeof(Control), sa->stream));
	if ((rc = launch_rebuild(sa, sa->scratch, 0, want_cum ? sa->d_cum : nullptr, want_probs ? sa->d_final_probs : nullptr))) return rc;
	if ((rc = read_ctl(sa, sa->scratch, out))) return rc;
	if (out->error_flags) return fail(MGL_EINVAL, "slab is not a valid parse of the input");
	return MGL_OK;
}

extern "C" int mgl_sa_set_best(mgl_sa* sa, const mgl_packet* packets, uint64_t perplexity)
{
	if (!sa || !packets) return fail(MGL_EINVAL, "null argument");
	HIPCHK(hipSetDevice(sa->device));
	Control c;
	int rc = scratch_walk(sa, packets, false, false, &c);
	if (rc) return rc;
	if (c.rebuild_cost != perplexity) return fail(MGL_EINVAL, "mgl_sa_set_best: perplexity does not match the slab");
	HIPCHK(hipMemcpyAsync(sa->d_best, sa->scratch.v.slab, sizeof(mgl_pk) * (size_t)sa->n, hipMemcpyDeviceToDevice, sa->stream));
	if (sa->d_snap_meta) HIPCHK(hipMemsetAsync(sa->d_snap_meta + 1, 0, sizeof(SnapMeta), sa->stream));
	if ((rc = read_ctl(sa, sa->base, &c))) return rc;
	c.best_cost = perplexity;
	c.best_is_current = 0;
	return write_ctl(sa, sa->base, &c);
}

extern "C" int mgl_cost_slab(mgl_sa* sa, const mgl_packet* packets, uint64_t* total, uint64_t* per_packet_cumulative,
                             size_t* npackets)
{
	if (!sa || !packets) return fail(MGL_EINVAL, "null argument");
	HIPCHK(hipSetDevice(sa->device));
	Control c;
	int rc = scratch_walk(sa, packets, per_packet_cumulative != nullptr, false, &c);
	if (rc) return rc;
	if (total) *total = c.rebuild_cost;
	if (npackets) *npackets = (size_t)c.packets;
	if (per_packet_cumulative)
		HIPCHK(hipMemcpy(per_packet_cumulative, sa->d_cum, sizeof(uint64_t) * (size_t)c.packets, hipMemcpyDeviceToHost));
	return MGL_OK;
}

extern "C" int mgl_props_sweep(mgl_sa* sa, const mgl_packet* packets, mgl_props_cost* out, size_t cap, size_t* count, double* gpu_ms)
{
	static_assert(MGL_PROPS_TRIPLES == MGL_PROPS_NTRIPLES, "header and kernel disagree on the number of triples");
	if (!sa || !out) return fail(MGL_EINVAL, "null argument");
	if (count) *count = MGL_PROPS_TRIPLES;
	if (cap < MGL_PROPS_TRIPLES) return fail(MGL_ERANGE, "mgl_props_sweep: out holds fewer than 75 entries");
	HIPCHK(hipSetDevice(sa->device));
	const mgl_pk* slab = sa->base.v.slab;
	if (packets) {
		Control c;
		int rc = scratch_walk(sa, packets, false, false, &c);
		if (rc) return rc;
		slab = sa->scratch.v.slab;
	}
	struct Tmp {
		uint64_t* d = nullptr;
		hipEvent_t t0 = nullptr, t1 = nullptr;
		~Tmp() { dfree(d); if (t0) (void)hipEventDestroy(t0); if (t1) (void)hipEventDestroy(t1); }
	} tmp;
	HIPCHK(hipMalloc(&tmp.d, sizeof(uint64_t) * MGL_PROPS_TRIPLES));
	HIPCHK(hipEventCreate(&tmp.t0));
	HIPCHK(hipEventCreate(&tmp.t1));
	HIPCHK(hipEventRecord(tmp.t0, sa->stream));
	hipLaunchKernelGGL(k_props_sweep, dim3(MGL_PROPS_TRIPLES), dim3(64), 0, sa->stream, sa->ctx, slab, tmp.d);
	HIPCHK(hipGetLastError());
	HIPCHK(hipEventRecord(tmp.t1, sa->stream));
	uint64_t costs[MGL_PROPS_TRIPLES];
	HIPCHK(hipMemcpyAsync(costs, tmp.d, sizeof costs, hipMemcpyDeviceToHost, sa->stream));
	HIPCHK(hipStreamSynchronize(sa->stream));
	float ms = 0;
	HIPCHK(hipEventElapsedTime(&ms, tmp.t0, tmp.t1));
	if (gpu_ms) *gpu_ms = ms;
	for (uint32_t t = 0; t < MGL_PROPS_TRIPLES; t++) {
		const mgl_layout L = mgl_props_triple(t);
		out[t].props.lc = (uint8_t)L.lc; out[t].props.lp = (uint8_t)L.lp; out[t].props.pb = (uint8_t)L.pb;
		out[t].cost = costs[t];
	}
	return MGL_OK;
}

extern "C" int mgl_final_state(mgl_sa* sa, const mgl_packet* packets, uint16_t* probs_out, size_t probs_cap,
                               uint8_t* ctx_state_out, uint32_t dists_out[4])
{
	if (!sa || !packets) return fail(MGL_EINVAL, "null argument");
	HIPCHK(hipSetDevice(sa->device));
	Control c;
	int rc = scratch_walk(sa, packets, false, true, &c);
	if (rc) return rc;
	if (ctx_state_out) *ctx_state_out = (uint8_t)c.final_ctx_state;
	if (dists_out) memcpy(dists_out, c.final_dists, sizeof c.final_dists);
	if (probs_out) {
		const uint32_t total = sa->ctx.L.total, lit = total - MGL_OFF_LIT;
		if (probs_cap < total) return fail(MGL_ERANGE, "probs_out too small");
		std::vector<uint16_t> mine(total);
		HIPCHK(hipMemcpy(mine.data(), sa->d_final_probs, sizeof(uint16_t) * total, hipMemcpyDeviceToHost));
		uint16_t* o = probs_out;
		memcpy(o, &mine[MGL_OFF_LIT], 2 * lit); o += lit;
		memcpy(o, &mine[MGL_OFF_LEN], 2 * 514); o += 514;
		memcpy(o, &mine[MGL_OFF_REP_LEN], 2 * 514); o += 514;
		memcpy(o, &mine[MGL_OFF_DIST], 2 * 387); o += 387;
		memcpy(o, &mine[0], 2 * 432);
	}
// ... 33 lines not shown
	if (pos >= sa->n) return fail(MGL_ERANGE, "position outside the input");
	HIPCHK(hipSetDevice(sa->device));
	const uint32_t dcap = cap < sa->sub_cap ? (uint32_t)cap : sa->sub_cap;
	DevCtx c = sa->ctx;
	c.dict_limit = 0xFFFFFFFFu;
	hipLaunchKernelGGL(k_substrings, dim3(1), dim3(1), 0, sa->stream, c, (uint32_t)pos, (uint32_t)max_len, sa->d_sub_offs,
	                   sa->d_sub_lens, dcap, sa->d_small);
	HIPCHK(hipGetLastError());
	uint32_t cnt = 0;
	HIPCHK(hipMemcpyAsync(&cnt, sa->d_small, sizeof cnt, hipMemcpyDeviceToHost, sa->stream));
	HIPCHK(hipStreamSynchronize(sa->stream));
	const uint32_t take = cnt < dcap ? cnt : dcap;
	if (offsets && take) HIPCHK(hipMemcpy(offsets, sa->d_sub_offs, sizeof(uint32_t) * take, hipMemcpyDeviceToHost));
	if (lengths && take) HIPCHK(hipMemcpy(lengths, sa->d_sub_lens, sizeof(uint32_t) * take, hipMemcpyDeviceToHost));
	*count = cnt;
	return MGL_OK;
}

extern "C" int mgl_neighbours(mgl_sa* sa, uint64_t global_step, uint64_t* costs, mgl_diff* diffs, uint32_t* ndiffs, size_t diff_cap)
{
	if (!sa || !costs) return fail(MGL_EINVAL, "null argument");
	HIPCHK(hipSetDevice(sa->device));
	int rc = launch_neighbours(sa, global_step);
	if (rc == MGL_OK && sa->d_counts) HIPCHK(hipMemcpyAsync(sa->d_counts + 8, sa->d_counts, sizeof(uint32_t) * 8, hipMemcpyDeviceToDevice, sa->stream));
	if (rc) return rc;
	const size_t K = sa->cfg.neighbours_per_step;
	HIPCHK(hipMemcpyAsync(costs, sa->nbr.cost, sizeof(uint64_t) * K, hipMemcpyDeviceToHost, sa->stream));
	std::vector<uint32_t> nd(K), dpos;
	std::vector<mgl_pk> dold, dnew;
	HIPCHK(hipMemcpyAsync(nd.data(), sa->nbr.ndiffs, sizeof(uint32_t) * K, hipMemcpyDeviceToHost, sa->stream));
	if (diffs) {
		dpos.resize(K * MGL_MAX_DIFFS); dold.resize(K * MGL_MAX_DIFFS); dnew.resize(K * MGL_MAX_DIFFS);
		HIPCHK(hipMemcpyAsync(dpos.data(), sa->nbr.dpos, sizeof(uint32_t) * dpos.size(), hipMemcpyDeviceToHost, sa->stream));
		HIPCHK(hipMemcpyAsync(dold.data(), sa->nbr.dold, sizeof(mgl_pk) * dold.size(), hipMemcpyDeviceToHost, sa->stream));
		HIPCHK(hipMemcpyAsync(dnew.data(), sa->nbr.dnew, sizeof(mgl_pk) * dnew.size(), hipMemcpyDeviceToHost, sa->stream));
	}
	HIPCHK(hipStreamSynchronize(sa->stream));
	for (size_t j = 0; j < K; j++) {
		if (ndiffs) ndiffs[j] = nd[j];
		if (!diffs) continue;
		for (size_t e = 0; e < nd[j] && e < diff_cap; e++) {
			mgl_diff* d = &diffs[j * diff_cap + e];
			const mgl_pk o = dold[j * MGL_MAX_DIFFS + e], w = dnew[j * MGL_MAX_DIFFS + e];
			d->position = dpos[j * MGL_MAX_DIFFS + e];
			d->old_packet.type = (uint8_t)mgl_pk_type(o); d->old_packet.dist = mgl_pk_dist(o); d->old_packet.len = (uint16_t)mgl_pk_len(o);
			d->new_packet.type = (uint8_t)mgl_pk_type(w); d->new_packet.dist = mgl_pk_dist(w); d->new_packet.len = (uint16_t)mgl_pk_len(w);
		}
	}
	return MGL_OK;
}

extern "C" int mgl_debug_dump(mgl_sa* sa, uint32_t what, void* out, size_t cap_bytes, size_t* bytes)
{
	if (!sa || !out || !bytes) return fail(MGL_EINVAL, "null argument");
	if (!sa->incremental && what != 21 && what != 22) return fail(MGL_EINVAL, "mgl_debug_dump: handle runs the full-walk engine");
	HIPCHK(hipSetDevice(sa->device));
	HIPCHK(hipStreamSynchronize(sa->stream));
	const Base2& b = sa->b2;
	const void* src = nullptr;
	size_t sz = 0;
	uint32_t top = 0;
	if (sa->incremental) HIPCHK(hipMemcpy(&top, b.pool_top, sizeof top, hipMemcpyDeviceToHost));
	switch (what) {
	case 0: src = b.ch_off; sz = sizeof(uint32_t) * sa->ctx.L.total; break;
	case 1: src = b.ch_len; sz = sizeof(uint32_t) * sa->ctx.L.total; break;
	case 2: src = b.ch_pos; sz = sizeof(uint32_t) * (size_t)top; break;
	case 3: src = b.ch_ev; sz = sizeof(uint16_t) * (size_t)top; break;
	case 4: src = b.onwalk; sz = sizeof(uint64_t) * b.nw0; break;
	case 5: src = b.sp0; sz = sizeof(uint64_t) * b.nw0; break;
	case 6: src = b.sp_state; sz = sizeof(uint32_t) * 8 * (size_t)sa->n; break;
	case 7: src = b.ck_probs; sz = sizeof(uint16_t) * (size_t)b.nck * b.ck_elems; break;
	case 8: src = b.ch_cap; sz = sizeof(uint32_t) * sa->ctx.L.total; break;
	case 9: src = sa->d_prof; sz = sa->d_prof ? sizeof(unsigned long long) * (32 + sa->cfg.neighbours_per_step) : 0; break;
	case 80: {
		const uint64_t v[3] = { sa->batch_accepts, sa->batch_fallbacks, sa->batch_early_giveups };
		*bytes = sizeof v;
		if (cap_bytes >= sizeof v) memcpy(out, v, sizeof v);
		return MGL_OK;
	}
	case 84: src = sa->lim.why; sz = sizeof(uint32_t); break;
	case 85: src = b.pool_top; sz = sizeof(uint32_t); break;
	case 83: src = b.ch_sb; sz = sizeof(uint32_t) * (size_t)b.ck_elems * b.sb_stride; break;
	case 81: src = sa->batch.hdr; sz = sizeof(uint32_t) * 16; break;
	case 82: src = sa->batch.acc; sz = sizeof(long long) * 4; break;
	case 10: src = sa->d_counts + 8; sz = sizeof(uint32_t) * 4; break;
	case 14: src = sa->ab.hdr; sz = sa->ab.hdr ? sizeof(uint32_t) * 16 : 0; break;
	case 16: src = sa->base.ctl; sz = sizeof(Control); break;
	case 15: src = sa->d_pickrec; sz = sa->d_pickrec ? sizeof(uint4) * sa->cfg.neighbours_per_step : 0; break;
	case 18: src = sa->d_quad_pos; sz = sizeof(uint32_t) * (sa->n - 1); break;
	case 19: src = sa->d_quad_nx; sz = sizeof(uint16_t) * (sa->n - 1); break;
	case 12: src = sa->d_bucket_off; sz = sizeof(uint32_t) * 65537; break;
	case 13: src = sa->d_bucket_pos; sz = sizeof(uint32_t) * (sa->n - 1); break;
	case 30: case 31: case 32: case 33: case 34: case 35: src = sa->d_xpos[what - 30]; sz = sizeof(uint32_t) * (sa->n - 1); break;
	case 40: case 41: case 42: case 43: case 44: case 45: src = sa->d_xrank[what - 40]; sz = src ? sizeof(uint32_t) * (sa->n - 1) : 0; break;
	case 50: case 51: case 52: case 53: case 54: case 55: src = sa->d_xrun[what - 50]; sz = src ? sizeof(uint32_t) * (sa->n - 1) : 0; break;
	case 60: case 61: case 62: case 63: case 64: case 65: src = sa->d_xnxb[what - 60]; sz = sa->n - 1; break;
	case 70: src = sa->d_oct_pos; sz = sizeof(uint32_t) * (sa->n - 1); break;
	case 71: src = sa->d_oct_rank; sz = sizeof(uint32_t) * (sa->n - 1); break;
	case 72: src = sa->d_oct_run; sz = sizeof(uint32_t) * (sa->n - 1); break;
	case 73: src = sa->d_oct_nx8; sz = sizeof(uint64_t) * (sa->n - 1); break;
	case 74: src = sa->d_hex_pos; sz = sizeof(uint32_t) * (sa->n - 1); break;
	case 75: src = sa->d_hex_rank; sz = sizeof(uint32_t) * (sa->n - 1); break;
	case 76: src = sa->d_hex_run; sz = sizeof(uint32_t) * (sa->n - 1); break;
	case 77: src = sa->d_hex_nx8; sz = sizeof(uint64_t) * (sa->n - 1); break;
	case 22: src = sa->nbr.win2; sz = sizeof(uint32_t) * sa->cfg.neighbours_per_step; break;
	case 21: src = sa->nbr.win; sz = sizeof(uint32_t) * 2 * sa->cfg.neighbours_per_step; break;
	case 11: src = sa->pb.acc; sz = sa->pb.acc ? sizeof(unsigned long long) * 8 : 0; break;
	default: return fail(MGL_EINVAL, "mgl_debug_dump: unknown selector");
	}
	*bytes = sz;
	if (sz > cap_bytes) return fail(MGL_ERANGE, "mgl_debug_dump: buffer too small");
	HIPCHK(hipMemcpy(out, src, sz, hipMemcpyDeviceToHost));
	if (what == 84) HIPCHK(hipMemset(sa->lim.why, 0, sizeof(uint32_t)));
	return MGL_OK;
}

extern "C" int mgl_debug_set(mgl_sa* sa, uint32_t key, uint64_t value)
{
	if (sa && key == 5) {
		sa->force_batch_late = (uint32_t)(value >> 32);
		sa->force_batch_fail = (uint32_t)value;
		if (sa->force_batch_late && !sa->force_batch_fail) sa->force_batch_fail = 1;
		return MGL_OK;
	}
	if (sa && key == 6) {
		const uint32_t id = (uint32_t)(value & 0xFFu);
		const uint64_t v = value >> 8;
		if (!sa->incremental || !sa->lim.why) return fail(MGL_EINVAL, "mgl_debug_set: no in-place accept on this handle");
		HIPCHK(hipSetDevice(sa->device));
		HIPCHK(hipStreamSynchronize(sa->stream));
		if (id == 0) {
			if (v) return fail(MGL_EINVAL, "mgl_debug_set: limit id 0 takes value 0 (restore the defaults)");
			for (uint32_t i = 1; i < MGL_LIM_COUNT; i++) sa->lim.v[i] = i == MGL_LIM_SOFT_REACH ? 0u : sa->lim_max.v[i];
		} else {
			if (id >= MGL_LIM_COUNT || v > sa->lim_max.v[id]) return fail(MGL_EINVAL, "mgl_debug_set: unknown limit, or a value above the compiled / allocated one");
			sa->lim.v[id] = (uint32_t)v;
		}
		HIPCHK(hipMemset(sa->lim.why, 0, sizeof(uint32_t)));
		return MGL_OK;
	}
	if (sa && key == 4) {
		if (!sa->d_traffic) return fail(MGL_EINVAL, "mgl_debug_set: no split neighbour evaluation on this handle");
		sa->count_traffic = value != 0;
		return MGL_OK;
	}
	if (!sa) return fail(MGL_EINVAL, "null handle");
	if (key == 0) { sa->ctx.diag_stop = (uint32_t)value; return MGL_OK; }
	if (key == 1) { sa->pb.force_fix = (uint32_t)value; return MGL_OK; }
	if (key == 2) {
		if (value < 8 || value > sa->chg_cap || (value & 7u)) return fail(MGL_EINVAL, "mgl_debug_set: list capacity must be a multiple of 8 within the allocated one");
		sa->big.chg_cap = (uint32_t)value;
		return MGL_OK;
	}
	if (key == 3) { sa->force_rollbacks = (uint32_t)value; return MGL_OK; }
	return fail(MGL_EINVAL, "mgl_debug_set: unknown key");
}

#include "mgl_exchange.inc"
```

### megalania_amd/csrc/mgl_kernels2.hip

```cpp
#include "mgl_base2.h"


struct BitAcc {
	uint32_t word;
	uint64_t bits;
};
__device__ __forceinline__ void bitacc_move(BitAcc& a, uint64_t* arr, uint32_t new_word, uint32_t lane)
{
	if (new_word == a.word) return;
	if (lane == 0) arr[a.word] = a.bits;
	for (uint32_t z = a.word + 1 + lane; z < new_word; z += 64) arr[z] = 0;
	a.word = new_word; a.bits = 0;
}

__device__ void build_body(const DevCtx& c, const Base2& b, Control* ctl, int check_cost)
{
	extern __shared__ __attribute__((aligned(16))) unsigned char smem[];
	uint16_t* T = (uint16_t*)smem;
	uint16_t* probs = (uint16_t*)(smem + 4096);
	uint32_t* cnt = (uint32_t*)(smem + 4096 + (size_t)b.ck_elems * 2);
	uint32_t* off = cnt + b.ck_elems;
	const uint32_t lane = threadIdx.x;
	const uint32_t total = c.L.total;
	if (check_cost && !ctl->accepted_flag) return;
// ... 417 lines not shown
	if (!p.acc) return;
	const unsigned long long now = __builtin_readcyclecounter();
	if (lane == 0) { atomicAdd(&p.acc[phase], now - p.t); atomicAdd(&p.acc[8 + phase], 1ull); atomicMax(&p.acc[16 + phase], now - p.t); }
	p.t = __builtin_readcyclecounter();
}

struct Win {
	uint32_t base;
	mgl_pk pk;
	uint32_t byte;
};
__device__ __forceinline__ void win_cover(Win& w, const DevCtx& c, const mgl_pk* slab, uint32_t pos, uint32_t lane)
{
	const uint32_t base = pos & ~63u;
	if (base != w.base) {
		const uint32_t p = base + lane;
		w.pk = p < c.n ? slab[p] : 0;
		w.byte = c.data[p < c.n ? p : c.n];
		w.base = base;
	}
}
__device__ __forceinline__ mgl_pk win_pk(const Win& w, uint32_t pos) { return rdlane64(w.pk, pos - w.base); }
__device__ __forceinline__ uint32_t win_byte(const Win& w, uint32_t pos) { return rdlane(w.byte, pos - w.base); }

__device__ __forceinline__ void plan_at(const DevCtx& c, const mgl_wstate& st, uint32_t type, uint32_t dist, uint32_t len,
                                        uint32_t byte, mgl_plan& pl)
{
	uint32_t match_byte = 0, prev_byte = 0;
	if (type == MGL_LITERAL) {
		if (st.ctx_state >= 7 && st.dists[0] < st.pos) match_byte = c.data[st.pos - st.dists[0] - 1];
		if (c.L.lc > 0 && st.pos > 0) prev_byte = c.data[st.pos - 1];
	}
	mgl_plan_packet(&c.L, &st, type, dist, len, byte, match_byte, prev_byte, &pl);
}

template <bool INS>
__device__ __forceinline__ uint32_t literal_run_events(const DevCtx& c, Changes& ch, const Win& win, mgl_wstate& st, uint32_t limit, uint32_t lane)
{
	if (st.ctx_state >= 7u) return 0;
	const uint32_t o = st.pos - win.base;
	const unsigned long long lit = __ballot(mgl_pk_type(win.pk) == MGL_LITERAL) >> o;
	uint32_t run = (uint32_t)__ffsll((long long)~lit) - 1u;
	if (~lit == 0ull) run = 64u;
	run = run < 64u - o ? run : 64u - o;
	run = run < limit ? run : limit;
	if (run < 2u) return 0;
	const uint32_t take = run < 7u ? run : 7u;
	uint32_t& n = INS ? ch.n_ins : ch.n_rem;
	if (n + 9u * take > ch.cap) { ch.overflow = true; ch.list_full = true; return take; }
	const uint32_t i = lane / 9u, slot = lane - i * 9u;
	const uint32_t p = st.pos + i;
	const bool active = i < take;
	const uint32_t byte = (uint32_t)__shfl((int)win.byte, (int)((p - win.base) & 63u), 64);
	uint32_t prev_byte = 0;
	if (c.L.lc > 0) {
		const uint32_t wprev = (uint32_t)__shfl((int)win.byte, (int)((p - 1u - win.base) & 63u), 64);
		prev_byte = p == 0 ? 0u : (p - 1u >= win.base ? wprev : (uint32_t)c.data[p - 1u]);
	}
	mgl_wstate sv = st;
	sv.pos = p;
	sv.ctx_state = lit_steps(st.ctx_state, i);
	mgl_plan pl;
	mgl_plan_packet(&c.L, &sv, MGL_LITERAL, 0, 1, byte, 0, prev_byte, &pl);
	if (__ballot(active && pl.nev != 9u)) return 0;
	if (active) {
		uint32_t ctx, bit;
		mgl_plan_event(&pl, slot, &ctx, &bit);
		const uint32_t at = n + i * 9u + slot;
		if (INS) { ch.ins_key[at] = (uint16_t)(ctx | (bit << 15)); ch.ins_pos[at] = p; }
		else { ch.rem_key[at] = (uint16_t)ctx; ch.rem_pos[at] = p; }
	}
	n += 9u * take;
	st.pos += take;
	st.ctx_state = lit_steps(st.ctx_state, take);
	return take;
}

__device__ void model_load(const DevCtx& c, const Base2& b, uint16_t* probs, const uint16_t* T, uint32_t y, uint32_t lane)
{
	const uint32_t ck = y >> MGL_CK2_SHIFT;
	const uint4* src = (const uint4*)(b.ck_probs + (size_t)ck * b.ck_elems);
	uint4* dst = (uint4*)probs;
	const uint32_t n16 = b.ck_elems / 8u;
	for (uint32_t base = 0; base < n16; base += 256u) {
		uint4 r[4];
#pragma unroll
		for (uint32_t u = 0; u < 4; u++) { const uint32_t i = base + u * 64u + lane; if (i < n16) r[u] = src[i]; }
#pragma unroll
		for (uint32_t u = 0; u < 4; u++) { const uint32_t i = base + u * 64u + lane; if (i < n16) dst[i] = r[u]; }
	}
	const uint32_t first = ck << MGL_CK2_SHIFT;
	const uint64_t bits = b.onwalk[first >> 6] & ((y & 63u) ? ((1ull << (y & 63u)) - 1ull) : 0ull) & (~0ull << (first & 63u));
	wave_sync();
	if (bits) {
		const uint32_t start = uni(((first >> 6) << 6) + ctz64(bits));
		Walk w;
		walk_reset(w);
		w.st = uni_state(base_state_at(b, start));
		while (w.st.pos < y) {
			walk_window(w, c, b.slab, lane);
			if (w.st.ctx_state < 7u) {
				const uint32_t o = w.st.pos - w.wbase;
				const unsigned long long lit = __ballot(mgl_pk_type(w.wpk) == MGL_LITERAL) >> o;
				uint32_t run = ~lit == 0ull ? 64u : (uint32_t)__ffsll((long long)~lit) - 1u;
				run = run < 64u - o ? run : 64u - o;
				run = run < y - w.st.pos ? run : y - w.st.pos;
				if (run >= 2u) {
					const uint32_t take = run < 7u ? run : 7u;
					const uint32_t i = lane / 9u, slot = lane - i * 9u, p = w.st.pos + i;
					const bool active = i < take;
					const uint32_t byte = (uint32_t)__shfl((int)w.wbyte, (int)((p - w.wbase) & 63u), 64);
					uint32_t prev_byte = 0;
					if (c.L.lc > 0) {
						const uint32_t wprev = (uint32_t)__shfl((int)w.wbyte, (int)((p - 1u - w.wbase) & 63u), 64);
						prev_byte = p == 0 ? 0u : (p - 1u >= w.wbase ? wprev : (uint32_t)c.data[p - 1u]);
					}
					mgl_wstate sv = w.st;
					sv.pos = p; sv.ctx_state = lit_steps(w.st.ctx_state, i);
					mgl_plan pl;
					mgl_plan_packet(&c.L, &sv, MGL_LITERAL, 0, 1, byte, 0, prev_byte, &pl);
					if (!__ballot(active && pl.nev != 9u)) {
						uint32_t ctx = 0, bit = 0;
						if (active) mgl_plan_event(&pl, slot, &ctx, &bit);
						for (uint32_t r = 0; r < take; r++) {
							if (active && i == r) probs[ctx] = (uint16_t)mgl_prob_update(probs[ctx], bit);
							wave_sync();
						}
						w.st.pos += take; w.st.ctx_state = lit_steps(w.st.ctx_state, take);
						w.packets += take;
						continue;
					}
				}
			}
			const mgl_pk pk = walk_slab_at(w, w.st.pos);
			walk_packet<true>(w, c, probs, T, mgl_pk_type(pk), mgl_pk_dist(pk), mgl_pk_len(pk), lane);
		}
		wave_sync();
	}
}

__device__ __forceinline__ void walk_from_state(Walk& w, const mgl_wstate& st)
{
	walk_reset(w);
	w.st = st;
}

struct BigScratch {
	uint16_t* ins_key; uint32_t* ins_pos; uint16_t* rem_key; uint32_t* rem_pos; uint16_t* uctx;
	uint32_t cap, uctx_cap, slots;
	const uint32_t* todo_in; const uint32_t* todo_in_count;
	uint32_t* spill_ctr;
	uint32_t chg_cap;
	uint4* sim_hdr;
	uint4* sim_hdr2;
	uint32_t* sim_slot2;
	uint32_t lds_cache;
	uint16_t* sim_keys;
	uint32_t* sim_pos;
	uint32_t* cont;
};
#define MGL_CONT_WORDS 368u
#define MGL_CONT_MAGIC 0x434F4E54u
#ifndef MGL_PICK_T_GLOBAL
#define MGL_PICK_T_GLOBAL 1
#endif
#ifndef MGL_REST_WAVES_PER_SIMD
#define MGL_REST_WAVES_PER_SIMD 4
#endif
#define MGL_SIM2_CAP 4096u
#define MGL_NBR_FULL 0
#define MGL_NBR_PICK 1
#define MGL_NBR_REST 2
template <bool BIG, int MODE>
__device__ __forceinline__ void nbr2_one(const DevCtx& c, const Base2& b, Control* ctl, uint64_t seed,
                                         uint64_t step_override, uint32_t K, const NbrOut& out, uint32_t per_wave_bytes,
                                         uint32_t* todo, uint32_t* todo_count, unsigned long long* prof_acc,
                                         const BigScratch& big, uint4* pickrec, uint32_t j_base, uint32_t j_end, uint4* pickstate,
                                         unsigned char* smem, const uint16_t* T, uint32_t unit, uint32_t lane, uint32_t wid)
{
	uint32_t j = j_base + unit;
	uint32_t slot = 0;
	const unsigned long long t_begin = prof_acc ? __builtin_readcyclecounter() : 0ull;
	if (BIG) {
		slot = unit;
		const uint32_t nflag = *big.todo_in_count;
		if (slot >= nflag) return;
		j = uni(big.todo_in[slot]);
		if (lane == 0) atomicAdd((unsigned long long*)&ctl->big_nbrs, 1ull);
	}
	if (j >= K || (!BIG && j >= j_end)) return;
	unsigned char* mine = smem + ((MODE == MGL_NBR_REST || (MODE == MGL_NBR_PICK && MGL_PICK_T_GLOBAL)) ? 0u : 4096u) + (size_t)wid * per_wave_bytes;
	Journal jn;
	jn.old = (mgl_pk*)mine;
	jn.neu = jn.old + MGL_MAX_DIFFS;
	jn.pos = (uint32_t*)(jn.neu + MGL_MAX_DIFFS);
	jn.count = 0; jn.overflow = false;
	Changes ch;
	ch.nbitwords = (c.L.total + 31u) >> 5;
	ch.ctxbits = jn.pos + MGL_MAX_DIFFS;
	unsigned char* uni_base = MODE == MGL_NBR_PICK ? mine : (unsigned char*)(ch.ctxbits + ((ch.nbitwords + 3u) & ~3u));
	uint16_t* probs = (uint16_t*)uni_base;
	uint32_t* lencost = (uint32_t*)(uni_base + (size_t)b.ck_elems * 2);
	ch.ins_pos = (uint32_t*)uni_base;
	ch.rem_pos = ch.ins_pos + big.chg_cap;
	ch.ins_key = (uint16_t*)(ch.rem_pos + big.chg_cap);
	ch.rem_key = ch.ins_key + big.chg_cap;
	ch.uctx = ch.rem_key + big.chg_cap;
	ch.cap = big.chg_cap; ch.uctx_cap = 2 * big.chg_cap;
	if (BIG) {
		if (slot >= big.slots) {
			if (lane == 0) { const uint32_t s2 = atomicAdd(todo_count, 1u); todo[s2] = j; }
			return;
		}
		ch.ins_key = big.ins_key + (size_t)slot * big.cap; ch.ins_pos = big.ins_pos + (size_t)slot * big.cap;
		ch.rem_key = big.rem_key + (size_t)slot * big.cap; ch.rem_pos = big.rem_pos + (size_t)slot * big.cap;
		ch.uctx = big.uctx + (size_t)slot * big.uctx_cap;
		ch.cap = big.cap; ch.uctx_cap = big.uctx_cap;
	}
	ch.n_ins = ch.n_rem = 0; ch.direct = 0; ch.overflow = false; ch.list_full = false;
	bool too_many = false;
	bool spilled = BIG;
	const bool spilled_lds = false;

	const uint64_t gstep = step_override != ~0ull ? step_override : ctl->gstep;
	NbrRng rng; rng.key = mgl_rng_key(seed, gstep, j); rng.n = 0;
	uint32_t* const crec = (BIG && big.cont != nullptr) ? big.cont + (size_t)slot * MGL_CONT_WORDS : nullptr;
	bool resumed = false;
	if (BIG && crec != nullptr) resumed = uni(crec[0]) == MGL_CONT_MAGIC && uni(crec[1]) == j;

	uint32_t target;
	mgl_wstate nb;
	if (MODE == MGL_NBR_REST && lane == 0) big.sim_hdr[j] = make_uint4(0xFFFFFFFFu, 0u, 0u, 0u);
	if (BIG && big.sim_hdr2 != nullptr && lane == 0) big.sim_hdr2[j] = make_uint4(0xFFFFFFFFu, 0u, 0u, 0u);
	if (MODE == MGL_NBR_REST) {
		const uint4 s0 = pickstate[2u * j], s1 = pickstate[2u * j + 1u];
		target = s0.x; rng.n = s0.y;
		nb.pos = target; nb.ctx_state = s0.z;
		nb.dists[0] = s0.w; nb.dists[1] = s1.x; nb.dists[2] = s1.y; nb.dists[3] = s1.z;
	} else if (BIG && resumed) {
		target = uni(crec[2]);
		nb.pos = uni(crec[3]); nb.ctx_state = uni(crec[4]);
		nb.dists[0] = uni(crec[5]); nb.dists[1] = uni(crec[6]); nb.dists[2] = uni(crec[7]); nb.dists[3] = uni(crec[8]);
	} else if (c.strat_pre != nullptr) {
		target = uni(c.strat_tgt[j]);
		rng.n = 1;
		nb = uni_state(base_state_at(b, target));
		if (MODE == MGL_NBR_PICK && lane == 0) {
			pickstate[2u * j] = make_uint4(target, rng.n, nb.ctx_state, nb.dists[0]);
			pickstate[2u * j + 1u] = make_uint4(nb.dists[1], nb.dists[2], nb.dists[3], 0u);
		}
	} else {
		uint32_t mydraw = lane < 32 ? mgl_rng_draw(rng.key, lane) % c.n : 0;
		bool on = lane < 32 && ((b.onwalk[mydraw >> 6] >> (mydraw & 63u)) & 1ull);
		unsigned long long m = __ballot(on);
		if (m) {
			int f = __ffsll((long long)m) - 1;
			target = rdlane(mydraw, (uint32_t)f);
			rng.n = (uint32_t)f + 1;
		} else {
			rng.n = 32;
			uint32_t p = rdlane(mydraw, 31);
			uint32_t wd = p >> 6;
			uint64_t bits = b.onwalk[wd] & (~0ull << (p & 63u));
			while (!bits && ++wd < b.nw0) bits = b.onwalk[wd];
			target = uni(bits ? (wd << 6) + ctz64(bits) : 0u);
		}
		nb = uni_state(base_state_at(b, target));
		if (MODE == MGL_NBR_PICK && lane == 0) {
			pickstate[2u * j] = make_uint4(target, rng.n, nb.ctx_state, nb.dists[0]);
			pickstate[2u * j + 1u] = make_uint4(nb.dists[1], nb.dists[2], nb.dists[3], 0u);
		}
	}
	Prof prof;
	prof_start(prof, prof_acc);
	ch.dbg = prof_acc;
	ch.diag = c.diag_stop;
	const uint32_t pos = target;
	mgl_wstate bs = nb;
	Win win; win.base = 0xFFFFFFFFu; win.pk = 0; win.byte = 0;
	Walk tw;

	win_cover(win, c, b.slab, pos, lane);
	const mgl_pk first = win_pk(win, pos);
	mgl_pk m_first = first, m_second = 0;
	bool second_set = false, mutated = false;
	prof_mark(prof, 0, lane);
	if (c.diag_stop == 1) { if (lane == 0) { out.cost[j] = MGL_INVALID_COST; out.ndiffs[j] = 0; out.walked[j] = first; } return; }
	if (!(BIG && resumed) && pos + 1 < c.n && (nbr_draw(rng) % 2u) == 0) {
		const mgl_pk second = uni64(b.slab[pos + 1]);
		const uint32_t ft = mgl_pk_type(first), flen = mgl_pk_len(first);
		const uint32_t st = mgl_pk_type(second), slen = mgl_pk_len(second), sdist = mgl_pk_dist(second);
		if ((ft == MGL_LONG_REP || ft == MGL_MATCH) && flen > 2) {
			m_second = mgl_pack(ft, mgl_pk_dist(first), flen - 1);
			m_first = MGL_PK_LITERAL;
			if (MODE != MGL_NBR_PICK) { journal_set(jn, pos, first, m_first, lane); journal_set(jn, pos + 1, second, m_second, lane); }
			second_set = true; mutated = true;
		} else if ((ft == MGL_LITERAL || ft == MGL_SHORT_REP) && (st == MGL_MATCH || st == MGL_LONG_REP)) {
			uint32_t rep_start = pos - (st == MGL_LONG_REP ? mgl_dist_at(&nb, sdist) : sdist);
			if (slen < MGL_MAX_MATCH && rep_start > 0 && rep_start <= pos && win_byte(win, pos) == c.data[rep_start - 1]) {
				m_first = mgl_pack(st, sdist, slen + 1);
				if (MODE != MGL_NBR_PICK) journal_set(jn, pos, first, m_first, lane);
				mutated = true;
			}
		}
	}
	enum { P_MODEL, P_SIM, P_TOPK, P_WALK, P_OUT };
	uint32_t phase = mutated ? P_WALK : P_MODEL;
	if (MODE == MGL_NBR_PICK && mutated) return;
	if (MODE == MGL_NBR_REST && c.diag_stop != 0 && c.diag_stop != 4 && c.diag_stop < 40) return;
	bool pick_is_mutation = !mutated;
	uint32_t pick_pos = pos;
	mgl_pk pick_inc = first;
	bool pick_best = false;
	bool have_pick = false;
	mgl_pk picked_pk = 0, resume_old = 0;
	uint32_t sim_limit = MGL_POS_INF;
	bool sim_overlay = false;
	int64_t delta = 0;
	bool generate_failed = false, sim_deferred = false, walk_long = false;
	uint32_t npicks = 0;
	uint32_t count = 0;
	uint32_t walked = 0;
	uint32_t wend = 0;
	uint32_t wsoft = 0xFFFFFFFFu, taint = 0xFu, dep = 0u;
	bool first_packet = true;
	uint32_t guard = 0;
	if (BIG && resumed) {
		bs.pos = uni(crec[9]); bs.ctx_state = uni(crec[10]);
		bs.dists[0] = uni(crec[11]); bs.dists[1] = uni(crec[12]); bs.dists[2] = uni(crec[13]); bs.dists[3] = uni(crec[14]);
		count = uni(crec[15]); walked = uni(crec[16]); npicks = uni(crec[17]); wsoft = uni(crec[18]); taint = uni(crec[19]); dep = uni(crec[20]);
		rng.n = uni(crec[21]); guard = uni(crec[22]); jn.count = uni(crec[23]); ch.n_ins = uni(crec[24]); ch.n_rem = uni(crec[25]);
		const uint32_t fl = uni(crec[26]);
		pick_best = (fl & 1u) != 0; second_set = (fl & 2u) != 0;
		pick_inc = (mgl_pk)uni(crec[28]) | ((mgl_pk)uni(crec[29]) << 32);
		resume_old = (mgl_pk)uni(crec[30]) | ((mgl_pk)uni(crec[31]) << 32);
		m_second = (mgl_pk)uni(crec[32]) | ((mgl_pk)uni(crec[33]) << 32);
		ch.direct = (int64_t)((uint64_t)uni(crec[34]) | ((uint64_t)uni(crec[35]) << 32));
		if (lane < jn.count) {
			jn.pos[lane] = crec[48u + lane];
			jn.old[lane] = reinterpret_cast<const mgl_pk*>(crec + 112u)[lane];
			jn.neu[lane] = reinterpret_cast<const mgl_pk*>(crec + 240u)[lane];
		}
		wave_sync();
		if (lane == 0) crec[0] = 0u;
		pick_pos = nb.pos;
		mutated = true; pick_is_mutation = false; first_packet = false;
		phase = P_MODEL;
	}
	if ((MODE == MGL_NBR_REST || (BIG && pickrec != nullptr)) && !mutated) {
		const uint4 rec = pickrec[j];
		if (!(rec.w & 1u)) { generate_failed = true; phase = P_OUT; }
		else {
			m_first = (mgl_pk)rec.x | ((mgl_pk)rec.y << 32);
			journal_set(jn, pos, first, m_first, lane);
			rng.n = rec.z;
			pick_is_mutation = false;
			phase = P_WALK;
		}
	}

	for (;;) {
		if (MODE == MGL_NBR_REST && (phase == P_MODEL || phase == P_TOPK)) { ch.overflow = true; phase = P_OUT; continue; }
		if (MODE != MGL_NBR_REST && phase == P_MODEL) {
			if ((ch.n_ins + ch.n_rem) != 0 && !spilled) {
				uint32_t sl = 0;
				if (lane == 0) sl = atomicAdd(big.spill_ctr, 1u);
				sl = uni(sl);
				if (sl >= big.slots) { ch.overflow = true; phase = P_OUT; continue; }
				uint16_t* gik = big.ins_key + (size_t)sl * big.cap; uint32_t* gip = big.ins_pos + (size_t)sl * big.cap;
				uint16_t* grk = big.rem_key + (size_t)sl * big.cap; uint32_t* grp = big.rem_pos + (size_t)sl * big.cap;
				for (uint32_t i = lane; i < ch.n_ins; i += 64) { gik[i] = ch.ins_key[i]; gip[i] = ch.ins_pos[i]; }
				for (uint32_t i = lane; i < ch.n_rem; i += 64) { grk[i] = ch.rem_key[i]; grp[i] = ch.rem_pos[i]; }
				__threadfence_block();
				wave_sync();
				ch.ins_key = gik; ch.ins_pos = gip; ch.rem_key = grk; ch.rem_pos = grp;
				ch.uctx = big.uctx + (size_t)sl * big.uctx_cap;
				ch.cap = big.cap; ch.uctx_cap = big.uctx_cap;
				spilled = true;
			}
			model_load(c, b, probs, T, pick_pos, lane);
			if (!pick_is_mutation) prof_mark(prof, 5, lane);
			if (pick_is_mutation) {
				prof_mark(prof, 1, lane);
				if (c.diag_stop == 2) { if (lane == 0) { out.cost[j] = MGL_INVALID_COST; out.ndiffs[j] = 0; out.walked[j] = probs[lane]; } return; }
			}
			if ((ch.n_ins + ch.n_rem) != 0) { sim_limit = pick_pos; sim_overlay = true; phase = P_SIM; }
			else phase = P_TOPK;
		}
		if (BIG && big.sim_hdr2 != nullptr && !sim_overlay && !spilled_lds && ch.n_ins <= MGL_SIM2_CAP && ch.n_rem <= MGL_SIM2_CAP && phase == P_SIM) {
			if (lane == 0) {
				big.sim_slot2[j] = slot;
				big.sim_hdr2[j] = make_uint4(ch.n_ins, ch.n_rem, (uint32_t)(uint64_t)ch.direct, (uint32_t)((uint64_t)ch.direct >> 32));
			}
			sim_deferred = true;
			phase = P_OUT;
			continue;
		}
		if (MODE == MGL_NBR_REST && phase == P_SIM) {
			uint16_t* gk = big.sim_keys + (size_t)j * (2u * big.chg_cap);
			uint32_t* gp = big.sim_pos + (size_t)j * (2u * big.chg_cap);
			for (uint32_t e = lane; e < ch.n_ins; e += 64) { gk[e] = ch.ins_key[e]; gp[e] = ch.ins_pos[e]; }
			for (uint32_t e = lane; e < ch.n_rem; e += 64) { gk[big.chg_cap + e] = ch.rem_key[e]; gp[big.chg_cap + e] = ch.rem_pos[e]; }
			if (lane == 0) big.sim_hdr[j] = make_uint4(ch.n_ins, ch.n_rem, (uint32_t)(uint64_t)ch.direct, (uint32_t)((uint64_t)ch.direct >> 32));
			sim_deferred = true;
			phase = P_OUT;
			continue;
		}
		if (MODE == MGL_NBR_FULL && phase == P_SIM) {
			int64_t r;
			if (BIG && big.lds_cache && ch.n_ins <= MGL_BIG_CAP && ch.n_rem <= MGL_BIG_CAP) {
				uint32_t* cp = (uint32_t*)(mine + per_wave_bytes);
				Changes cl = ch;
				cl.ins_pos = cp; cl.rem_pos = cp + MGL_BIG_CAP;
				cl.ins_key = (uint16_t*)(cp + 2u * MGL_BIG_CAP); cl.rem_key = cl.ins_key + MGL_BIG_CAP;
				for (uint32_t e = lane; e < ch.n_ins; e += 64) { cl.ins_pos[e] = ch.ins_pos[e]; cl.ins_key[e] = ch.ins_key[e]; }
				for (uint32_t e = lane; e < ch.n_rem; e += 64) { cl.rem_pos[e] = ch.rem_pos[e]; cl.rem_key[e] = ch.rem_key[e]; }
				wave_sync();
				r = chain_sim(b, cl, T, sim_limit, sim_overlay ? probs : nullptr, lane, &too_many);
			} else {
				r = chain_sim(b, ch, T, sim_limit, (MODE != MGL_NBR_REST && sim_overlay) ? probs : nullptr, lane, &too_many);
			}
			wave_sync();
			if (too_many) { phase = P_OUT; continue; }
			if (sim_overlay) { prof_mark(prof, 6, lane); phase = P_TOPK; }
			else { delta = r; prof_mark(prof, 4, lane); phase = P_OUT; }
		}
		if (MODE != MGL_NBR_REST && phase == P_TOPK) {
			walk_from_state(tw, nb);
			walk_window(tw, c, b.slab, lane);
			mgl_pk picked;
			const bool ok = pick_from_top_k<(MODE == MGL_NBR_PICK ? 4 : 1)>(c, tw, probs, T, lencost, pick_inc, pick_best, rng, lane, &picked);
			if (MODE == MGL_NBR_PICK) {
				if (lane == 0) pickrec[j] = make_uint4((uint32_t)picked, (uint32_t)(picked >> 32), rng.n, ok ? 1u : 0u);
				return;
			}
			if (pick_is_mutation) {
				if (!ok) { generate_failed = true; phase = P_OUT; continue; }
				m_first = picked;
				journal_set(jn, pos, first, m_first, lane);
				pick_is_mutation = false;
				prof_mark(prof, 2, lane);
				if (c.diag_stop == 3 || (c.diag_stop >= 31 && c.diag_stop <= 39)) { if (lane == 0) { out.cost[j] = MGL_INVALID_COST; out.ndiffs[j] = 0; out.walked[j] = (uint32_t)m_first; } return; }
			} else {
				picked_pk = ok ? picked : pick_inc;
				have_pick = true;
				prof_mark(prof, 7, lane);
			}
			win.base = 0xFFFFFFFFu;
			phase = P_WALK;
		}
		if (MODE != MGL_NBR_PICK && phase == P_WALK) {
			bool request_pick = false;
			while (nb.pos < c.n || bs.pos < c.n) {
				if (ch.overflow || jn.overflow || too_many || ++guard > (BIG ? (1u << 20) : 4096u)) { ch.overflow = true; break; }
				if (!first_packet && !have_pick && nb.pos == bs.pos && count >= 3) {
					const bool same_ctx = nb.ctx_state == bs.ctx_state;
					const bool same_d = nb.dists[0] == bs.dists[0] && nb.dists[1] == bs.dists[1] && nb.dists[2] == bs.dists[2] &&
					                    nb.dists[3] == bs.dists[3];
					if (same_ctx && wsoft == 0xFFFFFFFFu) wsoft = nb.pos;
					if (same_ctx && same_d) break;
					if (same_ctx && nb.ctx_state < 7) {
						uint32_t sx = uni(sp_find_next(b, nb.pos));
						if (sx == MGL_POS_INF || sx > c.n) sx = c.n;
						if (sx > nb.pos) {
							const uint32_t cs = lit_steps(nb.ctx_state, sx - nb.pos);
							nb.pos = bs.pos = sx; nb.ctx_state = bs.ctx_state = cs;
							count = 8;
							continue;
						}
					}
				}
				if (walked > MGL_MAX_WALK && !have_pick) { walk_long = true; break; }
				if ((have_pick || nb.pos <= bs.pos) && nb.pos < c.n) {
					const uint32_t p = nb.pos;
					win_cover(win, c, b.slab, p, lane);
					mgl_pk pk, old = 0;
					if (have_pick) {
						pk = picked_pk; old = resume_old; have_pick = false;
					} else if (first_packet) {
						pk = m_first;
					} else {
						if (count < 8) count++;
						old = (second_set && p == pos + 1) ? m_second : win_pk(win, p);
						pk = old;
						uint32_t type = mgl_pk_type(pk);
						if (type == MGL_SHORT_REP || (type == MGL_LITERAL && count < 4)) {
							const bool same = nb.dists[0] < p && win_byte(win, p) == c.data[p - nb.dists[0] - 1];
							if (same) { if (count < 4) pk = MGL_PK_SHORT_REP; }
							else pk = MGL_PK_LITERAL;
						}
						type = mgl_pk_type(pk);
						if (type == MGL_LONG_REP) {
							const uint32_t len = mgl_pk_len(pk);
							uint32_t idx = mgl_pk_dist(pk);
							walk_from_state(tw, nb);
							bool ok = long_rep_ok(c, tw, idx, len, lane);
							for (uint32_t i = 0; i < 4 && !ok; i++) { idx = i; ok = long_rep_ok(c, tw, idx, len, lane); }
							pk = mgl_pack(MGL_LONG_REP, idx, len);
							if (!ok) {
								if (++npicks > MGL_MAX_REPAIR_PICKS) { walk_long = true; break; }
								pick_best = (nbr_draw(rng) % 4u) == 0;
								while (bs.pos < p && !ch.overflow) {
									win_cover(win, c, b.slab, bs.pos, lane);
									const mgl_pk bpk = win_pk(win, bs.pos);
									mgl_plan bpl;
									plan_at(c, bs, mgl_pk_type(bpk), mgl_pk_dist(bpk), mgl_pk_len(bpk), win_byte(win, bs.pos), bpl);
									changes_add<false>(ch, bpl, bs.pos, lane);
									mgl_advance(&bs, mgl_pk_type(bpk), mgl_pk_dist(bpk), mgl_pk_len(bpk));
								}
								if (ch.overflow) break;
								if (MODE == MGL_NBR_REST && big.cont != nullptr) {
									uint32_t slot2 = 0;
									if (lane == 0) {
										atomicAdd(big.spill_ctr + 1, 1u);
										slot2 = atomicAdd(todo_count, 1u);
										todo[slot2] = j;
										out.cost[j] = MGL_INVALID_COST; out.ndiffs[j] = 0; out.walked[j] = 0; out.win[2u * j] = pos; out.win[2u * j + 1u] = MGL_WIN_NONE;
									}
									slot2 = uni(slot2);
									if (slot2 < big.slots) {
										uint16_t* gik = big.ins_key + (size_t)slot2 * big.cap; uint32_t* gip = big.ins_pos + (size_t)slot2 * big.cap;
										uint16_t* grk = big.rem_key + (size_t)slot2 * big.cap; uint32_t* grp = big.rem_pos + (size_t)slot2 * big.cap;
										for (uint32_t i = lane; i < ch.n_ins; i += 64) { gik[i] = ch.ins_key[i]; gip[i] = ch.ins_pos[i]; }
										for (uint32_t i = lane; i < ch.n_rem; i += 64) { grk[i] = ch.rem_key[i]; grp[i] = ch.rem_pos[i]; }
										uint32_t* rec = big.cont + (size_t)slot2 * MGL_CONT_WORDS;
										if (lane < jn.count) {
											rec[48u + lane] = jn.pos[lane];
											reinterpret_cast<mgl_pk*>(rec + 112u)[lane] = jn.old[lane];
											reinterpret_cast<mgl_pk*>(rec + 240u)[lane] = jn.neu[lane];
										}
										if (lane == 0) {
											rec[1] = j; rec[2] = pos;
											rec[3] = nb.pos; rec[4] = nb.ctx_state; rec[5] = nb.dists[0]; rec[6] = nb.dists[1]; rec[7] = nb.dists[2]; rec[8] = nb.dists[3];
											rec[9] = bs.pos; rec[10] = bs.ctx_state; rec[11] = bs.dists[0]; rec[12] = bs.dists[1]; rec[13] = bs.dists[2]; rec[14] = bs.dists[3];
											rec[15] = count; rec[16] = walked; rec[17] = npicks; rec[18] = wsoft; rec[19] = taint; rec[20] = dep;
											rec[21] = rng.n; rec[22] = guard; rec[23] = jn.count; rec[24] = ch.n_ins; rec[25] = ch.n_rem;
											rec[26] = (pick_best ? 1u : 0u) | (second_set ? 2u : 0u);
											rec[28] = (uint32_t)pk; rec[29] = (uint32_t)(pk >> 32);
											rec[30] = (uint32_t)old; rec[31] = (uint32_t)(old >> 32);
											rec[32] = (uint32_t)m_second; rec[33] = (uint32_t)(m_second >> 32);
											rec[34] = (uint32_t)(uint64_t)ch.direct; rec[35] = (uint32_t)((uint64_t)ch.direct >> 32);
											rec[0] = MGL_CONT_MAGIC;
										}
									}
									return;
								}
								resume_old = old; pick_pos = p; pick_inc = pk;
								request_pick = true;
								if (!BIG && lane == 0) atomicAdd(big.spill_ctr + 1, 1u);
								break;
							}
						}
					}
					if (!first_packet && pk != old) {
						const mgl_pk base_old = (second_set && p == pos + 1) ? uni64(b.slab[p]) : old;
						journal_set(jn, p, base_old, pk, lane);
						wsoft = 0xFFFFFFFFu;
					}
					first_packet = false;
					walked++;
					const uint32_t ntype = mgl_pk_type(pk), ndist = mgl_pk_dist(pk), nlen = mgl_pk_len(pk);
					if (ntype == MGL_SHORT_REP || ntype == MGL_LONG_REP) {
						const uint32_t slot = ntype == MGL_SHORT_REP ? 0u : ndist;
						const bool same_read = bs.pos == p && win_pk(win, p) == pk && mgl_dist_at(&nb, slot) == mgl_dist_at(&bs, slot);
						if (!same_read) wsoft = 0xFFFFFFFFu;
						dep |= ntype == MGL_SHORT_REP ? (taint & 1u) : ((taint >> ndist) & 1u);
					}
					if (ntype == MGL_MATCH) taint = (taint << 1) & 0xFu;
					else if (ntype == MGL_LONG_REP) taint = (taint & ~((2u << ndist) - 1u)) | ((taint & ((1u << ndist) - 1u)) << 1) | ((taint >> ndist) & 1u);
					bool cancelled = false;
					if (bs.pos == p && win_pk(win, p) == pk && nb.ctx_state == bs.ctx_state) {
						cancelled = true;
						if (ntype == MGL_LITERAL && nb.ctx_state >= 7) {
							const uint32_t mn = nb.dists[0] < p ? c.data[p - nb.dists[0] - 1] : 0u;
							const uint32_t mb = bs.dists[0] < p ? c.data[p - bs.dists[0] - 1] : 0u;
							cancelled = mn == mb;
						}
					}
					if (cancelled) {
						mgl_advance(&bs, ntype, ndist, nlen);
					} else {
						if (bs.pos == p) {
							const mgl_pk bpk = win_pk(win, p);
							const uint32_t btype = mgl_pk_type(bpk), bdist = mgl_pk_dist(bpk), blen = mgl_pk_len(bpk);
							mgl_plan bpl;
							plan_at(c, bs, btype, bdist, blen, win_byte(win, p), bpl);
							changes_add<false>(ch, bpl, p, lane);
							mgl_advance(&bs, btype, bdist, blen);
						}
						mgl_plan npl;
						plan_at(c, nb, ntype, ndist, nlen, win_byte(win, p), npl);
						changes_add<true>(ch, npl, p, lane);
					}
					mgl_advance(&nb, ntype, ndist, nlen);
				} else {
					win_cover(win, c, b.slab, bs.pos, lane);
					if (literal_run_events<false>(c, ch, win, bs, (nb.pos < c.n ? nb.pos : c.n) - bs.pos, lane)) continue;
					const mgl_pk bpk = win_pk(win, bs.pos);
					mgl_plan bpl;
					plan_at(c, bs, mgl_pk_type(bpk), mgl_pk_dist(bpk), mgl_pk_len(bpk), win_byte(win, bs.pos), bpl);
					changes_add<false>(ch, bpl, bs.pos, lane);
					mgl_advance(&bs, mgl_pk_type(bpk), mgl_pk_dist(bpk), mgl_pk_len(bpk));
				}
			}
			if (walk_long) { phase = P_OUT; continue; }
			if (request_pick) { prof_mark(prof, 3, lane); phase = P_MODEL; continue; }
			prof_mark(prof, 3, lane);
			if (c.diag_stop == 4) { if (lane == 0) { out.cost[j] = MGL_INVALID_COST; out.ndiffs[j] = 0; out.walked[j] = ch.n_ins + ch.n_rem; } return; }
			if (ch.overflow || jn.overflow || too_many) { phase = P_OUT; continue; }
			wend = nb.pos;
			sim_limit = MGL_POS_INF; sim_overlay = false; phase = P_SIM;
			continue;
		}
		if (phase == P_OUT) break;
	}

	if (generate_failed) {
		if (lane == 0) { out.cost[j] = MGL_INVALID_COST; out.ndiffs[j] = 0; out.walked[j] = 0; out.win[2u * j] = pos; out.win[2u * j + 1u] = MGL_WIN_NONE; }
		return;
	}
	if (jn.overflow) {
		if (lane == 0) { out.cost[j] = MGL_INVALID_COST; out.ndiffs[j] = 0; out.walked[j] = walked; out.win[2u * j] = pos; out.win[2u * j + 1u] = MGL_WIN_DROPPED; }
		return;
	}
	if (walk_long || (ch.list_full && ch.cap == big.cap && !jn.overflow)) {
		if (lane == 0) { out.cost[j] = MGL_INVALID_COST; out.ndiffs[j] = 0; out.walked[j] = walked; out.win[2u * j] = pos; out.win[2u * j + 1u] = MGL_WIN_DROPPED; }
		return;
	}
	if (ch.overflow || too_many) {
		if (lane == 0) {
			const uint32_t slot2 = atomicAdd(todo_count, 1u);
			todo[slot2] = j;
			if (BIG) atomicAdd((unsigned long long*)&ctl->fallback_nbrs, 1ull);
			out.cost[j] = MGL_INVALID_COST; out.ndiffs[j] = 0; out.walked[j] = 0; out.win[2u * j] = pos; out.win[2u * j + 1u] = MGL_WIN_NONE;
		}
		return;
	}
	const uint64_t total = (uint64_t)((int64_t)ctl->rebuild_cost + delta + ch.direct);
	uint32_t nd = 0;
	for (uint32_t i = 0; i < jn.count; i++) {
		if (jn.old[i] == jn.neu[i]) continue;
		if (lane == 0) {
			out.dpos[(size_t)j * MGL_MAX_DIFFS + nd] = jn.pos[i];
			out.dold[(size_t)j * MGL_MAX_DIFFS + nd] = jn.old[i];
			out.dnew[(size_t)j * MGL_MAX_DIFFS + nd] = jn.neu[i];
		}
		nd++;
	}
	if (lane == 0) { if (!sim_deferred) out.cost[j] = total; out.ndiffs[j] = nd; out.walked[j] = walked; out.win[2u * j] = pos; out.win[2u * j + 1u] = wend; out.win2[j] = (wsoft < wend ? wsoft : wend) | (dep << 31); }
	if (prof_acc && lane == 0)
		prof_acc[32 + j] = ((__builtin_readcyclecounter() - t_begin) & 0xFFFFFFFFFFull) |
		                   ((unsigned long long)((ch.n_ins + ch.n_rem) & 0xFFFu) << 40) | ((unsigned long long)(walked & 0xFFFu) << 52);
}

template <bool BIG, int MODE>
__global__ void __launch_bounds__((MODE == MGL_NBR_PICK ? 512 : 64), (MODE == MGL_NBR_FULL ? (BIG ? 1 : MGL_NBR_WAVES_PER_SIMD) : (MODE == MGL_NBR_REST ? MGL_REST_WAVES_PER_SIMD : 4))) k_neighbours2(DevCtx c, Base2 b, Control* ctl, uint64_t seed,
                                                     uint64_t step_override, uint32_t K, NbrOut out, uint32_t per_wave_bytes,
                                                     uint32_t* todo, uint32_t* todo_count, unsigned long long* prof_acc,
                                                     BigScratch big, uint4* pickrec, uint32_t j_base, uint32_t j_end, uint4* pickstate)
{
	const uint32_t waves = blockDim.x >> 6;
	if (BIG && blockIdx.x * waves >= *big.todo_in_count) return;
	extern __shared__ __attribute__((aligned(16))) unsigned char smem[];
	uint16_t* T = (uint16_t*)smem;
	if (MODE == MGL_NBR_PICK && MGL_PICK_T_GLOBAL) {
		T = const_cast<uint16_t*>(c.cost_tbl);
	} else if (MODE != MGL_NBR_REST) {
		for (uint32_t i = threadIdx.x; i < 256; i += blockDim.x) reinterpret_cast<uint4*>(T)[i] = reinterpret_cast<const uint4*>(c.cost_tbl)[i];
		__syncthreads();
	}
	const uint32_t lane = threadIdx.x & 63u, wid = threadIdx.x >> 6;
	if (BIG) {
		const uint32_t n = *big.todo_in_count;
		for (uint32_t unit = blockIdx.x * waves + wid; unit < n; unit += gridDim.x * waves)
			nbr2_one<BIG, MODE>(c, b, ctl, seed, step_override, K, out, per_wave_bytes, todo, todo_count, prof_acc, big, pickrec, j_base, j_end, pickstate, smem, T, unit, lane, wid);
	} else {
		nbr2_one<BIG, MODE>(c, b, ctl, seed, step_override, K, out, per_wave_bytes, todo, todo_count, prof_acc, big, pickrec, j_base, j_end, pickstate, smem, T,
		                    blockIdx.x * waves + wid, lane, wid);
	}
}


#ifndef MGL_SIM_WAVES
#define MGL_SIM_WAVES 2u
#endif
#ifndef MGL_SIM_WAVES_LIST
#define MGL_SIM_WAVES_LIST 8u
#endif
#define MGL_SIM_WAVES_MAX 8u
struct SimShared {
	uint16_t* T;
	uint32_t* dyn;
	unsigned long long* sum;
	uint32_t* nu_many;
};
template <bool FROM_BIG, bool COUNT>
__device__ __forceinline__ void sim_one(const DevCtx& c, const Base2& b, Control* ctl, const NbrOut& out, const BigScratch& big, const uint4* hdrs,
                                        uint32_t j, uint32_t* todo, uint32_t* todo_count, const SimShared& sh, unsigned long long* traffic_ctr)
{
	const uint4 hdr = hdrs[j];
	if (hdr.x == 0xFFFFFFFFu) return;
	const uint32_t cap = FROM_BIG ? MGL_SIM2_CAP : big.chg_cap;
	const uint32_t slot = FROM_BIG ? big.sim_slot2[j] : 0u;
	uint32_t* s_bits = sh.dyn;
	uint32_t* s_pos = sh.dyn + ((((c.L.total + 31u) >> 5) + 3u) & ~3u);
	uint16_t* s_key = (uint16_t*)(s_pos + 2u * cap);
	uint16_t* s_uctx = s_key + 2u * cap;
	const uint32_t lane = threadIdx.x & 63u, wid = threadIdx.x >> 6;
	Changes ch;
	ch.n_ins = hdr.x; ch.n_rem = hdr.y;
	ch.ins_pos = s_pos; ch.rem_pos = s_pos + cap;
	ch.ins_key = s_key; ch.rem_key = s_key + cap;
	ch.uctx = s_uctx; ch.ctxbits = s_bits;
	ch.cap = cap; ch.uctx_cap = 2 * cap;
	ch.nbitwords = (c.L.total + 31u) >> 5;
	ch.direct = 0; ch.dbg = nullptr; ch.diag = c.diag_stop; ch.overflow = false; ch.list_full = false;
	__syncthreads();
	if (FROM_BIG) {
		const uint16_t* ik = big.ins_key + (size_t)slot * big.cap; const uint32_t* ip = big.ins_pos + (size_t)slot * big.cap;
		const uint16_t* rk = big.rem_key + (size_t)slot * big.cap; const uint32_t* rp = big.rem_pos + (size_t)slot * big.cap;
		for (uint32_t e = threadIdx.x; e < ch.n_ins; e += blockDim.x) { s_key[e] = ik[e]; s_pos[e] = ip[e]; }
		for (uint32_t e = threadIdx.x; e < ch.n_rem; e += blockDim.x) { s_key[cap + e] = rk[e]; s_pos[cap + e] = rp[e]; }
	} else {
		const uint16_t* gk = big.sim_keys + (size_t)j * (2u * cap);
		const uint32_t* gp = big.sim_pos + (size_t)j * (2u * cap);
		for (uint32_t e = threadIdx.x; e < ch.n_ins; e += blockDim.x) { s_key[e] = gk[e]; s_pos[e] = gp[e]; }
		for (uint32_t e = threadIdx.x; e < ch.n_rem; e += blockDim.x) { s_key[cap + e] = gk[cap + e]; s_pos[cap + e] = gp[cap + e]; }
	}
	__syncthreads();
	if (wid == 0) {
		bool too_many = false;
		const uint32_t nu = chain_list(ch, lane, &too_many);
		if (lane == 0) { sh.nu_many[0] = nu; sh.nu_many[1] = too_many ? 1u : 0u; }
	}
	__syncthreads();
	if (sh.nu_many[1]) {
		if (threadIdx.x == 0) {
			const uint32_t slot2 = atomicAdd(todo_count, 1u);
			todo[slot2] = j;
			out.cost[j] = MGL_INVALID_COST; out.ndiffs[j] = 0; out.walked[j] = 0; out.win[2u * j + 1u] = MGL_WIN_NONE;
		}
		return;
	}
	if (c.diag_stop == 41) { if (threadIdx.x == 0) out.cost[j] = sh.nu_many[0]; return; }
	uint32_t traffic = 0;
	const int64_t mine = chain_sim_contexts(b, ch, sh.T, MGL_POS_INF, nullptr, lane, wid * 64u, blockDim.x, sh.nu_many[0], COUNT ? &traffic : nullptr);
	const uint64_t u = wave_sum64((uint64_t)mine);
	if (lane == 0) sh.sum[wid] = u;
	if (COUNT) {
		const uint64_t tb = wave_sum64((uint64_t)traffic) + (wid == 0 ? 6ull * (ch.n_ins + ch.n_rem) + 16ull : 0ull);
		if (lane == 0) atomicAdd(traffic_ctr, (unsigned long long)tb);
	}
	__syncthreads();
	if (threadIdx.x == 0) {
		uint64_t d = 0;
		for (uint32_t w = 0; w < (blockDim.x >> 6); w++) d += sh.sum[w];
		const int64_t direct = (int64_t)((uint64_t)hdr.z | ((uint64_t)hdr.w << 32));
		out.cost[j] = (uint64_t)((int64_t)ctl->rebuild_cost + (int64_t)d + direct);
	}
}
template <bool COUNT>
__global__ void __launch_bounds__(64 * MGL_SIM_WAVES_MAX, 8) k_sim(DevCtx c, Base2 b, Control* ctl, NbrOut out, BigScratch big, uint32_t j_base, uint32_t j_end,
                                                           uint32_t* todo, uint32_t* todo_count, const uint32_t* list, const uint32_t* list_count,
                                                           unsigned long long* traffic_ctr)
{
	if (list ? blockIdx.x >= *list_count : j_base + blockIdx.x >= j_end) return;
	__shared__ __attribute__((aligned(16))) uint16_t T[2048];
	extern __shared__ __attribute__((aligned(16))) uint32_t s_dyn[];
	__shared__ unsigned long long s_sum[MGL_SIM_WAVES_MAX];
	__shared__ uint32_t s_nm[2];
	if (!list && big.sim_hdr[j_base + blockIdx.x].x == 0xFFFFFFFFu) return;
	for (uint32_t i = threadIdx.x; i < 256; i += blockDim.x) reinterpret_cast<uint4*>(T)[i] = reinterpret_cast<const uint4*>(c.cost_tbl)[i];
	SimShared sh;
	sh.T = T; sh.dyn = s_dyn; sh.sum = s_sum; sh.nu_many = s_nm;
	if (list) {
		const uint32_t n = *list_count;
		for (uint32_t i = blockIdx.x; i < n; i += gridDim.x)
			sim_one<true, COUNT>(c, b, ctl, out, big, big.sim_hdr2, list[i], todo, todo_count, sh, traffic_ctr);
	} else {
		sim_one<false, COUNT>(c, b, ctl, out, big, big.sim_hdr, j_base + blockIdx.x, todo, todo_count, sh, traffic_ctr);
	}
}


__global__ void __launch_bounds__(64) k_rank_blocks(const uint64_t* onwalk, uint32_t nw0, uint32_t* pre, uint32_t nblk)
{
	const uint32_t blk = blockIdx.x, lane = threadIdx.x;
	if (blk >= nblk) return;
	const uint32_t w = blk * 64u + lane;
	unsigned long long v = w < nw0 ? (unsigned long long)__popcll(onwalk[w]) : 0ull;
	v = wave_sum64(v);
	if (lane == 0) pre[blk + 1u] = (uint32_t)v;
}
__global__ void __launch_bounds__(1024) k_rank_scan(uint32_t* pre, uint32_t nblk)
{
	__shared__ uint32_t s_w[16], s_base;
	const uint32_t tid = threadIdx.x, lane = tid & 63u, wid = tid >> 6;
	if (tid == 0) { s_base = 0; pre[0] = 0; }
	__syncthreads();
	for (uint32_t base = 0; base < nblk; base += blockDim.x) {
		const uint32_t i = base + tid;
		const uint32_t v = i < nblk ? pre[i + 1u] : 0u;
		uint32_t incl = v;
		for (int o = 1; o < 64; o <<= 1) { const uint32_t t = (uint32_t)__shfl_up((int)incl, o, 64); if ((int)lane >= o) incl += t; }
		if (lane == 63) s_w[wid] = incl;
		__syncthreads();
		uint32_t bsum = s_base;
		for (uint32_t q = 0; q < wid; q++) bsum += s_w[q];
		if (i < nblk) pre[i + 1u] = bsum + incl;
		__syncthreads();
		if (tid == blockDim.x - 1u) s_base = bsum + incl;
		__syncthreads();
	}
}

__global__ void __launch_bounds__(256) k_targets(DevCtx c, const uint64_t* onwalk, uint32_t nw0, const Control* ctl, uint64_t seed, uint64_t step_override,
                                                 uint32_t K, uint32_t* tgt)
{
	const uint32_t j = blockIdx.x * (blockDim.x >> 6) + (threadIdx.x >> 6), lane = threadIdx.x & 63u;
	if (j >= K) return;
	const uint64_t gstep = step_override != ~0ull ? step_override : ctl->gstep;
	const uint32_t t = stratified_target(onwalk, nw0, c.strat_pre, c.strat_nblk, c.strat_pre[c.strat_nblk], K, j, mgl_rng_draw(mgl_rng_key(seed, gstep, j), 0), lane);
	if (lane == 0) tgt[j] = t;
}
```

Measured before the change: 13.78 million.

## Replace deferred big-neighbour sim kernel with in-block cooperative multi-wave simulation

Big neighbours no longer defer their chain simulation to a separate list-driven k_sim launch through sim_hdr2/sim_slot2 staging. Each big block now has one leader wave walking neighbours while helper waves wait on an LDS command record; when a sim is needed, all waves stage the change lists into LDS and split the context simulation, with the per-wave sums reduced through the shared command. This drops one kernel launch, the global header and slot arrays, and the global-to-LDS reload, but the helper waves sit idle during the non-sim phases and only one neighbour is processed per block.

```diff
diff --git a/megalania_amd/csrc/mgl_api.hip b/megalania_amd/csrc/mgl_api.hip
--- a/megalania_amd/csrc/mgl_api.hip
+++ b/megalania_amd/csrc/mgl_api.hip
@@ -103,6 +103,7 @@
 	unsigned long long* d_prof;
 	uint32_t* d_todo;
 	uint32_t per_wave2, waves_per_block2, nbr2_lds, build_lds;
+	uint32_t big_waves = MGL_BIG_WAVES;
 	uint32_t chg_cap = MGL_CHG_CAP;
 	uint32_t per_wave_pick, per_wave_rest, pick_waves;
 	size_t b2_bytes;
@@ -371,7 +372,7 @@
 	HIPCHK(hipGetLastError());
 	return MGL_OK;
 }
-static const bool g_trace = getenv("MGL_TRACE") != nullptr, g_prof_big = getenv("MGL_PROF_BIG") != nullptr, g_big_inline_sim = getenv("MGL_BIG_INLINE_SIM") != nullptr;
+static const bool g_trace = getenv("MGL_TRACE") != nullptr, g_prof_big = getenv("MGL_PROF_BIG") != nullptr;
 #define NBR_TRACE(name) do { if (g_trace) { fprintf(stderr, "[mgl] %s\n", name); hipError_t e_ = hipDeviceSynchronize(); if (e_ != hipSuccess) fprintf(stderr, "[mgl] %s -> %s\n", name, hipGetErrorString(e_)); } } while (0)
 static hipEvent_t sim_event(mgl_sa* sa, size_t i)
 {
@@ -448,15 +449,15 @@
 		for (uint32_t h = 0; h < slices; h++) {
 			const uint32_t j0 = (uint32_t)((uint64_t)K * h / slices), j1 = (uint32_t)((uint64_t)K * (h + 1) / slices);
 			HIPCHK(hipStreamWaitEvent(sa->stream3, sa->ev_rest[h], 0));
-			if (sa->time_sim_step >= 0 && h < 2) HIPCHK(hipEventRecord(sim_event(sa, 6 * (size_t)sa->time_sim_step + 2 * h), sa->stream3));
+			if (sa->time_sim_step >= 0 && h < 2) HIPCHK(hipEventRecord(sim_event(sa, 4 * (size_t)sa->time_sim_step + 2 * h), sa->stream3));
 			if (sa->count_traffic)
 				hipLaunchKernelGGL(k_sim<true>, dim3(j1 - j0), dim3(64 * sa->sim_waves), sim_lds_regular, sa->stream3, sa->ctx, sa->b2, sa->base.ctl,
-				                   sa->nbr, sa->big, j0, j1, sa->d_todo3, sa->d_counts + 4, (const uint32_t*)nullptr, (const uint32_t*)nullptr, sa->d_traffic);
+				                   sa->nbr, sa->big, j0, j1, sa->d_todo3, sa->d_counts + 4, sa->d_traffic);
 			else
 				hipLaunchKernelGGL(k_sim<false>, dim3(j1 - j0), dim3(64 * sa->sim_waves), sim_lds_regular, sa->stream3, sa->ctx, sa->b2, sa->base.ctl,
-				                   sa->nbr, sa->big, j0, j1, sa->d_todo3, sa->d_counts + 4, (const uint32_t*)nullptr, (const uint32_t*)nullptr, (unsigned long long*)nullptr);
+				                   sa->nbr, sa->big, j0, j1, sa->d_todo3, sa->d_counts + 4, (unsigned long long*)nullptr);
 			NBR_TRACE("k_sim");
-			if (sa->time_sim_step >= 0 && h < 2) HIPCHK(hipEventRecord(sim_event(sa, 6 * (size_t)sa->time_sim_step + 2 * h + 1), sa->stream3));
+			if (sa->time_sim_step >= 0 && h < 2) HIPCHK(hipEventRecord(sim_event(sa, 4 * (size_t)sa->time_sim_step + 2 * h + 1), sa->stream3));
 		}
 		HIPCHK(hipEventRecord(sa->ev_sim, sa->stream3));
 		for (uint32_t h = 1; h < slices; h += 2) HIPCHK(hipStreamWaitEvent(sa->stream, sa->ev_rest[h], 0));
@@ -466,31 +467,17 @@
 		                   sa->b2, sa->base.ctl, sa->cfg.seed, step_override, K, sa->nbr, sa->per_wave2, sa->d_todo, sa->d_counts,
 		                   sa->d_prof, sa->big, sa->d_pickrec, 0u, K, sa->d_pickstate); NBR_TRACE("k_neighbours2<false, MGL_NBR_FULL>");
 	}
-	const uint32_t bigneed = (sa->big.slots + sa->waves_per_block2 - 1) / sa->waves_per_block2;
-	const uint32_t bigblocks = bigneed < 1024u ? bigneed : 1024u;
-	BigScratch big_now = sa->big;
-	big_now.lds_cache = 1u;
-	const uint32_t big_lds = sa->nbr2_lds + 12u * MGL_BIG_CAP;
-	if (!split_now || g_big_inline_sim) big_now.sim_hdr2 = nullptr;
-	hipLaunchKernelGGL((k_neighbours2<true, MGL_NBR_FULL>), dim3(bigblocks), dim3(64 * sa->waves_per_block2), big_lds, sa->stream, sa->ctx,
+	const uint32_t bigblocks = sa->big.slots < 1024u ? sa->big.slots : 1024u;
+	const uint32_t big_lds = 4096u + sa->per_wave2 + 12u * MGL_BIG_CAP + MGL_COOP_BYTES;
+	hipLaunchKernelGGL((k_neighbours2<true, MGL_NBR_FULL>), dim3(bigblocks), dim3(64 * sa->big_waves), big_lds, sa->stream, sa->ctx,
 	                   sa->b2, sa->base.ctl, sa->cfg.seed, step_override, K, sa->nbr, sa->per_wave2, sa->d_todo2, sa->d_counts + 1,
-	                   g_prof_big ? sa->d_prof : (unsigned long long*)nullptr, big_now, (sa->split_nbr && !sa->form_single) ? sa->d_pickrec : (uint4*)nullptr, 0u, K, sa->d_pickstate); NBR_TRACE("k_neighbours2<true, MGL_NBR_FULL>");
+	                   g_prof_big ? sa->d_prof : (unsigned long long*)nullptr, sa->big, split_now ? sa->d_pickrec : (uint4*)nullptr, 0u, K, sa->d_pickstate); NBR_TRACE("k_neighbours2<true, MGL_NBR_FULL>");
 	if (split_now) {
-		const uint32_t sim_lds = ((((sa->ctx.L.total + 31u) >> 5) + 3u) & ~3u) * 4u + MGL_SIM2_CAP * 16u;
-		if (sa->time_sim_step >= 0) HIPCHK(hipEventRecord(sim_event(sa, 6 * (size_t)sa->time_sim_step + 4), sa->stream));
-		if (sa->count_traffic)
-			hipLaunchKernelGGL(k_sim<true>, dim3(256), dim3(64 * MGL_SIM_WAVES_LIST), sim_lds, sa->stream, sa->ctx, sa->b2, sa->base.ctl, sa->nbr, big_now, 0u, K,
-			                   sa->d_todo3, sa->d_counts + 4, (const uint32_t*)sa->d_todo, (const uint32_t*)sa->d_counts, sa->d_traffic);
-		else
-			hipLaunchKernelGGL(k_sim<false>, dim3(256), dim3(64 * MGL_SIM_WAVES_LIST), sim_lds, sa->stream, sa->ctx, sa->b2, sa->base.ctl, sa->nbr, big_now, 0u, K,
-			                   sa->d_todo3, sa->d_counts + 4, (const uint32_t*)sa->d_todo, (const uint32_t*)sa->d_counts, (unsigned long long*)nullptr);
-		NBR_TRACE("k_sim");
-		if (sa->time_sim_step >= 0) HIPCHK(hipEventRecord(sim_event(sa, 6 * (size_t)sa->time_sim_step + 5), sa->stream));
 		HIPCHK(hipStreamWaitEvent(sa->stream, sa->ev_sim, 0));
 		BigScratch late = sa->big;
-		late.todo_in = sa->d_todo3; late.todo_in_count = sa->d_counts + 4; late.sim_hdr2 = nullptr; late.lds_cache = 1u;
+		late.todo_in = sa->d_todo3; late.todo_in_count = sa->d_counts + 4;
 		late.cont = nullptr;
-		hipLaunchKernelGGL((k_neighbours2<true, MGL_NBR_FULL>), dim3(bigblocks < 64u ? bigblocks : 64u), dim3(64 * sa->waves_per_block2), big_lds, sa->stream, sa->ctx,
+		hipLaunchKernelGGL((k_neighbours2<true, MGL_NBR_FULL>), dim3(bigblocks < 64u ? bigblocks : 64u), dim3(64 * sa->big_waves), big_lds, sa->stream, sa->ctx,
 		                   sa->b2, sa->base.ctl, sa->cfg.seed, step_override, K, sa->nbr, sa->per_wave2, sa->d_todo2, sa->d_counts + 1,
 		                   (unsigned long long*)nullptr, late, sa->d_pickrec, 0u, K, sa->d_pickstate); NBR_TRACE("k_neighbours2<true, MGL_NBR_FULL>");
 	}
@@ -551,7 +538,7 @@
 		dfree(bt.bk_ipos); dfree(bt.bk_rpos); dfree(bt.bk_ibit); dfree(bt.bk_icl); dfree(bt.bk_rcl);
 	}
 	for (hipEvent_t e : sa->ev_sim_pool) if (e) (void)hipEventDestroy(e);
-	dfree(sa->d_todo2); dfree(sa->d_todo3); dfree(sa->d_counts); dfree(sa->big.sim_hdr2); dfree(sa->big.sim_slot2); dfree(sa->d_pickrec); dfree(sa->d_pickstate);
+	dfree(sa->d_todo2); dfree(sa->d_todo3); dfree(sa->d_counts); dfree(sa->d_pickrec); dfree(sa->d_pickstate);
 	dfree(sa->lim.why); dfree(sa->ab.hdr); dfree(sa->ab.ins_key); dfree(sa->ab.rem_key); dfree(sa->ab.ins_pos); dfree(sa->ab.rem_pos);
 	dfree(sa->ab.tctx); dfree(sa->ab.scratch_pos); dfree(sa->ab.scratch_ev);
 	dfree(sa->ab.span_pos); dfree(sa->ab.span_ev); dfree(sa->ab.jobs_b); dfree(sa->ab.jobs_c);
@@ -914,7 +901,7 @@
 		HIPCHK(hipFuncSetAttribute((const void*)k_neighbours2<false, MGL_NBR_FULL>, hipFuncAttributeMaxDynamicSharedMemorySize, (int)sa->nbr2_lds));
 		HIPCHK(hipFuncSetAttribute((const void*)k_neighbours2<false, MGL_NBR_PICK>, hipFuncAttributeMaxDynamicSharedMemorySize, 160 * 1024));
 		HIPCHK(hipFuncSetAttribute((const void*)k_neighbours2<false, MGL_NBR_REST>, hipFuncAttributeMaxDynamicSharedMemorySize, (int)sa->nbr2_lds));
-		HIPCHK(hipFuncSetAttribute((const void*)k_neighbours2<true, MGL_NBR_FULL>, hipFuncAttributeMaxDynamicSharedMemorySize, (int)(sa->nbr2_lds + 12u * MGL_BIG_CAP)));
+		HIPCHK(hipFuncSetAttribute((const void*)k_neighbours2<true, MGL_NBR_FULL>, hipFuncAttributeMaxDynamicSharedMemorySize, (int)(4096u + sa->per_wave2 + 12u * MGL_BIG_CAP + MGL_COOP_BYTES)));
 		HIPCHK(hipMalloc(&sa->d_pickrec, sizeof(uint4) * K));
 		HIPCHK(hipMalloc(&sa->d_pickstate, sizeof(uint4) * 2 * K));
 		sa->split_nbr = getenv("MGL_NO_SPLIT") == nullptr;
@@ -924,9 +911,6 @@
 			HIPCHK(hipMalloc(&g.sim_keys, sizeof(uint16_t) * 2u * sa->chg_cap * (size_t)K));
 			HIPCHK(hipMalloc(&g.sim_pos, sizeof(uint32_t) * 2u * sa->chg_cap * (size_t)K));
 			HIPCHK(hipMemset(g.sim_hdr, 0xFF, sizeof(uint4) * (size_t)K));
-			HIPCHK(hipMalloc(&g.sim_hdr2, sizeof(uint4) * (size_t)K));
-			HIPCHK(hipMalloc(&g.sim_slot2, sizeof(uint32_t) * (size_t)K));
-			HIPCHK(hipMemset(g.sim_hdr2, 0xFF, sizeof(uint4) * (size_t)K));
 			if (getenv("MGL_NO_CONT") == nullptr) {
 				HIPCHK(hipMalloc(&g.cont, sizeof(uint32_t) * MGL_CONT_WORDS * (size_t)g.slots));
 				HIPCHK(hipMemset(g.cont, 0, sizeof(uint32_t) * MGL_CONT_WORDS * (size_t)g.slots));
@@ -1972,9 +1956,8 @@
 		stats->neighbour_launches = timed_steps;
 		for (uint64_t s = 0; s < timed_steps && s < sim_timed.size(); s++) {
 			if (!sim_timed[s]) continue;
-			for (uint32_t h = 0; h < 3; h++) {
-				if (h < 2 && h >= sim_timed[s]) continue;
-				HIPCHK(hipEventElapsedTime(&ms, sa->ev_sim_pool[6 * s + 2 * h], sa->ev_sim_pool[6 * s + 2 * h + 1]));
+			for (uint32_t h = 0; h < sim_timed[s]; h++) {
+				HIPCHK(hipEventElapsedTime(&ms, sa->ev_sim_pool[4 * s + 2 * h], sa->ev_sim_pool[4 * s + 2 * h + 1]));
 				stats->gpu_ms_sim += ms;
 				stats->sim_launches++;
 			}
@@ -2314,6 +2297,11 @@
 		sa->big.chg_cap = (uint32_t)value;
 		return MGL_OK;
 	}
+	if (key == 7) {
+		if (value != 1 && value != 2 && value != MGL_BIG_WAVES) return fail(MGL_EINVAL, "mgl_debug_set: 1, 2 or MGL_BIG_WAVES wavefronts");
+		sa->big_waves = (uint32_t)value;
+		return MGL_OK;
+	}
 	if (key == 3) { sa->force_rollbacks = (uint32_t)value; return MGL_OK; }
 	return fail(MGL_EINVAL, "mgl_debug_set: unknown key");
 }
diff --git a/megalania_amd/csrc/mgl_kernels2.hip b/megalania_amd/csrc/mgl_kernels2.hip
--- a/megalania_amd/csrc/mgl_kernels2.hip
+++ b/megalania_amd/csrc/mgl_kernels2.hip
@@ -593,9 +593,6 @@
 	uint32_t* spill_ctr;
 	uint32_t chg_cap;
 	uint4* sim_hdr;
-	uint4* sim_hdr2;
-	uint32_t* sim_slot2;
-	uint32_t lds_cache;
 	uint16_t* sim_keys;
 	uint32_t* sim_pos;
 	uint32_t* cont;
@@ -608,10 +605,83 @@
 #ifndef MGL_REST_WAVES_PER_SIMD
 #define MGL_REST_WAVES_PER_SIMD 4
 #endif
-#define MGL_SIM2_CAP 4096u
 #define MGL_NBR_FULL 0
 #define MGL_NBR_PICK 1
 #define MGL_NBR_REST 2
+#ifndef MGL_BIG_WAVES
+#define MGL_BIG_WAVES 4u
+#endif
+#define MGL_COOP_SIM 1u
+#define MGL_COOP_EXIT 2u
+#define MGL_COOP_BYTES 128u
+struct CoopCmd {
+	uint32_t gen;
+	uint32_t op;
+	uint32_t slot;
+	uint32_t n_ins, n_rem, nu, limit;
+	uint32_t overlay;
+	unsigned long long sum[MGL_BIG_WAVES];
+};
+static_assert(sizeof(CoopCmd) <= MGL_COOP_BYTES, "CoopCmd outgrew its LDS");
+__device__ __forceinline__ CoopCmd* coop_cmd(unsigned char* smem, uint32_t per_wave_bytes)
+{
+	return (CoopCmd*)(smem + 4096u + per_wave_bytes + 12u * MGL_BIG_CAP);
+}
+__device__ __forceinline__ void coop_share(const DevCtx& c, const Base2& b, const BigScratch& big, unsigned long long* dbg, unsigned char* smem,
+                                           uint32_t per_wave_bytes, const uint16_t* T, CoopCmd* cmd, uint32_t lane, uint32_t wid)
+{
+	const uint32_t slot = uni(cmd->slot), overlay = uni(cmd->overlay);
+	Changes cl;
+	cl.n_ins = uni(cmd->n_ins); cl.n_rem = uni(cmd->n_rem);
+	uint32_t* cp = (uint32_t*)(smem + 4096u + per_wave_bytes);
+	cl.ins_pos = cp; cl.rem_pos = cp + MGL_BIG_CAP;
+	cl.ins_key = (uint16_t*)(cp + 2u * MGL_BIG_CAP); cl.rem_key = cl.ins_key + MGL_BIG_CAP;
+	cl.uctx = big.uctx + (size_t)slot * big.uctx_cap; cl.ctxbits = nullptr;
+	cl.cap = MGL_BIG_CAP; cl.uctx_cap = big.uctx_cap; cl.nbitwords = 0;
+	cl.direct = 0; cl.dbg = dbg; cl.diag = c.diag_stop; cl.overflow = false; cl.list_full = false;
+	const uint16_t* gik = big.ins_key + (size_t)slot * big.cap; const uint32_t* gip = big.ins_pos + (size_t)slot * big.cap;
+	const uint16_t* grk = big.rem_key + (size_t)slot * big.cap; const uint32_t* grp = big.rem_pos + (size_t)slot * big.cap;
+	for (uint32_t e = threadIdx.x; e < cl.n_ins; e += blockDim.x) { cl.ins_pos[e] = gip[e]; cl.ins_key[e] = gik[e]; }
+	for (uint32_t e = threadIdx.x; e < cl.n_rem; e += blockDim.x) { cl.rem_pos[e] = grp[e]; cl.rem_key[e] = grk[e]; }
+	__syncthreads();
+	const int64_t mine = chain_sim_contexts(b, cl, T, uni(cmd->limit), overlay ? (uint16_t*)(smem + overlay) : nullptr, lane, wid * 64u, blockDim.x, uni(cmd->nu));
+	const uint64_t u = wave_sum64((uint64_t)mine);
+	if (lane == 0) cmd->sum[wid] = u;
+	__syncthreads();
+}
+__device__ __forceinline__ int64_t coop_sim(const DevCtx& c, const Base2& b, const BigScratch& big, unsigned long long* dbg, unsigned char* smem,
+                                            uint32_t per_wave_bytes, const uint16_t* T, Changes& ch, uint32_t slot, uint32_t limit, uint16_t* overlay,
+                                            uint32_t lane, bool* too_many)
+{
+	const uint32_t nu = chain_list(ch, lane, too_many);
+	if (*too_many) return 0;
+	if (ch.diag == 41) return (int64_t)nu;
+	CoopCmd* cmd = coop_cmd(smem, per_wave_bytes);
+	if (lane == 0) {
+		cmd->op = MGL_COOP_SIM; cmd->slot = slot; cmd->n_ins = ch.n_ins; cmd->n_rem = ch.n_rem; cmd->nu = nu; cmd->limit = limit;
+		cmd->overlay = overlay ? (uint32_t)((unsigned char*)overlay - smem) : 0u;
+		cmd->gen = cmd->gen + 1u;
+	}
+	__syncthreads();
+	coop_share(c, b, big, dbg, smem, per_wave_bytes, T, cmd, lane, 0u);
+	uint64_t d = 0;
+	for (uint32_t w = 0; w < (blockDim.x >> 6); w++) d += cmd->sum[w];
+	wave_sync();
+	return (int64_t)d;
+}
+__device__ __forceinline__ void coop_helpers(const DevCtx& c, const Base2& b, const BigScratch& big, unsigned long long* dbg, unsigned char* smem,
+                                             uint32_t per_wave_bytes, const uint16_t* T, uint32_t lane, uint32_t wid)
+{
+	CoopCmd* cmd = coop_cmd(smem, per_wave_bytes);
+	uint32_t seen = 0;
+	for (;;) {
+		__syncthreads();
+		const uint32_t gen = uni(cmd->gen);
+		if (uni(cmd->op) == MGL_COOP_EXIT || gen == seen) return;
+		seen = gen;
+		coop_share(c, b, big, dbg, smem, per_wave_bytes, T, cmd, lane, wid);
+	}
+}
 template <bool BIG, int MODE>
 __device__ __forceinline__ void nbr2_one(const DevCtx& c, const Base2& b, Control* ctl, uint64_t seed,
                                          uint64_t step_override, uint32_t K, const NbrOut& out, uint32_t per_wave_bytes,
@@ -661,7 +731,6 @@
 	ch.n_ins = ch.n_rem = 0; ch.direct = 0; ch.overflow = false; ch.list_full = false;
 	bool too_many = false;
 	bool spilled = BIG;
-	const bool spilled_lds = false;
 
 	const uint64_t gstep = step_override != ~0ull ? step_override : ctl->gstep;
 	NbrRng rng; rng.key = mgl_rng_key(seed, gstep, j); rng.n = 0;
@@ -672,7 +741,6 @@
 	uint32_t target;
 	mgl_wstate nb;
 	if (MODE == MGL_NBR_REST && lane == 0) big.sim_hdr[j] = make_uint4(0xFFFFFFFFu, 0u, 0u, 0u);
-	if (BIG && big.sim_hdr2 != nullptr && lane == 0) big.sim_hdr2[j] = make_uint4(0xFFFFFFFFu, 0u, 0u, 0u);
 	if (MODE == MGL_NBR_REST) {
 		const uint4 s0 = pickstate[2u * j], s1 = pickstate[2u * j + 1u];
 		target = s0.x; rng.n = s0.y;
@@ -828,15 +896,6 @@
 			if ((ch.n_ins + ch.n_rem) != 0) { sim_limit = pick_pos; sim_overlay = true; phase = P_SIM; }
 			else phase = P_TOPK;
 		}
-		if (BIG && big.sim_hdr2 != nullptr && !sim_overlay && !spilled_lds && ch.n_ins <= MGL_SIM2_CAP && ch.n_rem <= MGL_SIM2_CAP && phase == P_SIM) {
-			if (lane == 0) {
-				big.sim_slot2[j] = slot;
-				big.sim_hdr2[j] = make_uint4(ch.n_ins, ch.n_rem, (uint32_t)(uint64_t)ch.direct, (uint32_t)((uint64_t)ch.direct >> 32));
-			}
-			sim_deferred = true;
-			phase = P_OUT;
-			continue;
-		}
 		if (MODE == MGL_NBR_REST && phase == P_SIM) {
 			uint16_t* gk = big.sim_keys + (size_t)j * (2u * big.chg_cap);
 			uint32_t* gp = big.sim_pos + (size_t)j * (2u * big.chg_cap);
@@ -849,18 +908,8 @@
 		}
 		if (MODE == MGL_NBR_FULL && phase == P_SIM) {
 			int64_t r;
-			if (BIG && big.lds_cache && ch.n_ins <= MGL_BIG_CAP && ch.n_rem <= MGL_BIG_CAP) {
-				uint32_t* cp = (uint32_t*)(mine + per_wave_bytes);
-				Changes cl = ch;
-				cl.ins_pos = cp; cl.rem_pos = cp + MGL_BIG_CAP;
-				cl.ins_key = (uint16_t*)(cp + 2u * MGL_BIG_CAP); cl.rem_key = cl.ins_key + MGL_BIG_CAP;
-				for (uint32_t e = lane; e < ch.n_ins; e += 64) { cl.ins_pos[e] = ch.ins_pos[e]; cl.ins_key[e] = ch.ins_key[e]; }
-				for (uint32_t e = lane; e < ch.n_rem; e += 64) { cl.rem_pos[e] = ch.rem_pos[e]; cl.rem_key[e] = ch.rem_key[e]; }
-				wave_sync();
-				r = chain_sim(b, cl, T, sim_limit, sim_overlay ? probs : nullptr, lane, &too_many);
-			} else {
-				r = chain_sim(b, ch, T, sim_limit, (MODE != MGL_NBR_REST && sim_overlay) ? probs : nullptr, lane, &too_many);
-			}
+			if (BIG) r = coop_sim(c, b, big, prof_acc, smem, per_wave_bytes, T, ch, slot, sim_limit, sim_overlay ? probs : nullptr, lane, &too_many);
+			else r = chain_sim(b, ch, T, sim_limit, sim_overlay ? probs : nullptr, lane, &too_many);
 			wave_sync();
 			if (too_many) { phase = P_OUT; continue; }
 			if (sim_overlay) { prof_mark(prof, 6, lane); phase = P_TOPK; }
@@ -1095,15 +1144,16 @@
 }
 
 template <bool BIG, int MODE>
-__global__ void __launch_bounds__((MODE == MGL_NBR_PICK ? 512 : 64), (MODE == MGL_NBR_FULL ? (BIG ? 1 : MGL_NBR_WAVES_PER_SIMD) : (MODE == MGL_NBR_REST ? MGL_REST_WAVES_PER_SIMD : 4))) k_neighbours2(DevCtx c, Base2 b, Control* ctl, uint64_t seed,
+__global__ void __launch_bounds__((MODE == MGL_NBR_PICK ? 512 : (BIG ? 64 * MGL_BIG_WAVES : 64)), (MODE == MGL_NBR_FULL ? (BIG ? 1 : MGL_NBR_WAVES_PER_SIMD) : (MODE == MGL_NBR_REST ? MGL_REST_WAVES_PER_SIMD : 4))) k_neighbours2(DevCtx c, Base2 b, Control* ctl, uint64_t seed,
                                                      uint64_t step_override, uint32_t K, NbrOut out, uint32_t per_wave_bytes,
                                                      uint32_t* todo, uint32_t* todo_count, unsigned long long* prof_acc,
                                                      BigScratch big, uint4* pickrec, uint32_t j_base, uint32_t j_end, uint4* pickstate)
 {
 	const uint32_t waves = blockDim.x >> 6;
-	if (BIG && blockIdx.x * waves >= *big.todo_in_count) return;
+	if (BIG && blockIdx.x >= *big.todo_in_count) return;
 	extern __shared__ __attribute__((aligned(16))) unsigned char smem[];
 	uint16_t* T = (uint16_t*)smem;
+	if (BIG && threadIdx.x == 0) { CoopCmd* cmd = coop_cmd(smem, per_wave_bytes); cmd->gen = 0; cmd->op = MGL_COOP_SIM; }
 	if (MODE == MGL_NBR_PICK && MGL_PICK_T_GLOBAL) {
 		T = const_cast<uint16_t*>(c.cost_tbl);
 	} else if (MODE != MGL_NBR_REST) {
@@ -1112,9 +1162,12 @@
 	}
 	const uint32_t lane = threadIdx.x & 63u, wid = threadIdx.x >> 6;
 	if (BIG) {
+		if (wid != 0) { coop_helpers(c, b, big, prof_acc, smem, per_wave_bytes, T, lane, wid); return; }
 		const uint32_t n = *big.todo_in_count;
-		for (uint32_t unit = blockIdx.x * waves + wid; unit < n; unit += gridDim.x * waves)
-			nbr2_one<BIG, MODE>(c, b, ctl, seed, step_override, K, out, per_wave_bytes, todo, todo_count, prof_acc, big, pickrec, j_base, j_end, pickstate, smem, T, unit, lane, wid);
+		for (uint32_t unit = blockIdx.x; unit < n; unit += gridDim.x)
+			nbr2_one<BIG, MODE>(c, b, ctl, seed, step_override, K, out, per_wave_bytes, todo, todo_count, prof_acc, big, pickrec, j_base, j_end, pickstate, smem, T, unit, lane, 0u);
+		if (lane == 0) { CoopCmd* cmd = coop_cmd(smem, per_wave_bytes); cmd->op = MGL_COOP_EXIT; cmd->gen = cmd->gen + 1u; }
+		__syncthreads();
 	} else {
 		nbr2_one<BIG, MODE>(c, b, ctl, seed, step_override, K, out, per_wave_bytes, todo, todo_count, prof_acc, big, pickrec, j_base, j_end, pickstate, smem, T,
 		                    blockIdx.x * waves + wid, lane, wid);
@@ -1124,9 +1177,6 @@
 
 #ifndef MGL_SIM_WAVES
 #define MGL_SIM_WAVES 2u
-#endif
-#ifndef MGL_SIM_WAVES_LIST
-#define MGL_SIM_WAVES_LIST 8u
 #endif
 #define MGL_SIM_WAVES_MAX 8u
 struct SimShared {
@@ -1135,14 +1185,13 @@
 	unsigned long long* sum;
 	uint32_t* nu_many;
 };
-template <bool FROM_BIG, bool COUNT>
+template <bool COUNT>
 __device__ __forceinline__ void sim_one(const DevCtx& c, const Base2& b, Control* ctl, const NbrOut& out, const BigScratch& big, const uint4* hdrs,
                                         uint32_t j, uint32_t* todo, uint32_t* todo_count, const SimShared& sh, unsigned long long* traffic_ctr)
 {
 	const uint4 hdr = hdrs[j];
 	if (hdr.x == 0xFFFFFFFFu) return;
-	const uint32_t cap = FROM_BIG ? MGL_SIM2_CAP : big.chg_cap;
-	const uint32_t slot = FROM_BIG ? big.sim_slot2[j] : 0u;
+	const uint32_t cap = big.chg_cap;
 	uint32_t* s_bits = sh.dyn;
 	uint32_t* s_pos = sh.dyn + ((((c.L.total + 31u) >> 5) + 3u) & ~3u);
 	uint16_t* s_key = (uint16_t*)(s_pos + 2u * cap);
@@ -1156,18 +1205,10 @@
 	ch.cap = cap; ch.uctx_cap = 2 * cap;
 	ch.nbitwords = (c.L.total + 31u) >> 5;
 	ch.direct = 0; ch.dbg = nullptr; ch.diag = c.diag_stop; ch.overflow = false; ch.list_full = false;
-	__syncthreads();
-	if (FROM_BIG) {
-		const uint16_t* ik = big.ins_key + (size_t)slot * big.cap; const uint32_t* ip = big.ins_pos + (size_t)slot * big.cap;
-		const uint16_t* rk = big.rem_key + (size_t)slot * big.cap; const uint32_t* rp = big.rem_pos + (size_t)slot * big.cap;
-		for (uint32_t e = threadIdx.x; e < ch.n_ins; e += blockDim.x) { s_key[e] = ik[e]; s_pos[e] = ip[e]; }
-		for (uint32_t e = threadIdx.x; e < ch.n_rem; e += blockDim.x) { s_key[cap + e] = rk[e]; s_pos[cap + e] = rp[e]; }
-	} else {
-		const uint16_t* gk = big.sim_keys + (size_t)j * (2u * cap);
-		const uint32_t* gp = big.sim_pos + (size_t)j * (2u * cap);
-		for (uint32_t e = threadIdx.x; e < ch.n_ins; e += blockDim.x) { s_key[e] = gk[e]; s_pos[e] = gp[e]; }
-		for (uint32_t e = threadIdx.x; e < ch.n_rem; e += blockDim.x) { s_key[cap + e] = gk[cap + e]; s_pos[cap + e] = gp[cap + e]; }
-	}
+	const uint16_t* gk = big.sim_keys + (size_t)j * (2u * cap);
+	const uint32_t* gp = big.sim_pos + (size_t)j * (2u * cap);
+	for (uint32_t e = threadIdx.x; e < ch.n_ins; e += blockDim.x) { s_key[e] = gk[e]; s_pos[e] = gp[e]; }
+	for (uint32_t e = threadIdx.x; e < ch.n_rem; e += blockDim.x) { s_key[cap + e] = gk[cap + e]; s_pos[cap + e] = gp[cap + e]; }
 	__syncthreads();
 	if (wid == 0) {
 		bool too_many = false;
@@ -1202,25 +1243,18 @@
 }
 template <bool COUNT>
 __global__ void __launch_bounds__(64 * MGL_SIM_WAVES_MAX, 8) k_sim(DevCtx c, Base2 b, Control* ctl, NbrOut out, BigScratch big, uint32_t j_base, uint32_t j_end,
-                                                           uint32_t* todo, uint32_t* todo_count, const uint32_t* list, const uint32_t* list_count,
-                                                           unsigned long long* traffic_ctr)
-{
-	if (list ? blockIdx.x >= *list_count : j_base + blockIdx.x >= j_end) return;
+                                                           uint32_t* todo, uint32_t* todo_count, unsigned long long* traffic_ctr)
+{
+	if (j_base + blockIdx.x >= j_end) return;
 	__shared__ __attribute__((aligned(16))) uint16_t T[2048];
 	extern __shared__ __attribute__((aligned(16))) uint32_t s_dyn[];
 	__shared__ unsigned long long s_sum[MGL_SIM_WAVES_MAX];
 	__shared__ uint32_t s_nm[2];
-	if (!list && big.sim_hdr[j_base + blockIdx.x].x == 0xFFFFFFFFu) return;
+	if (big.sim_hdr[j_base + blockIdx.x].x == 0xFFFFFFFFu) return;
 	for (uint32_t i = threadIdx.x; i < 256; i += blockDim.x) reinterpret_cast<uint4*>(T)[i] = reinterpret_cast<const uint4*>(c.cost_tbl)[i];
 	SimShared sh;
 	sh.T = T; sh.dyn = s_dyn; sh.sum = s_sum; sh.nu_many = s_nm;
-	if (list) {
-		const uint32_t n = *list_count;
-		for (uint32_t i = blockIdx.x; i < n; i += gridDim.x)
-			sim_one<true, COUNT>(c, b, ctl, out, big, big.sim_hdr2, list[i], todo, todo_count, sh, traffic_ctr);
-	} else {
-		sim_one<false, COUNT>(c, b, ctl, out, big, big.sim_hdr, j_base + blockIdx.x, todo, todo_count, sh, traffic_ctr);
-	}
+	sim_one<COUNT>(c, b, ctl, out, big, big.sim_hdr, j_base + blockIdx.x, todo, todo_count, sh, traffic_ctr);
 }
 
 
```

New measurement: 14.45 million, median of 6. 1.05x the previous value.
